# Zehong-Ma/MagCache

Measured on AMD Instinct MI355X. Metric: denoising steps/sec (MagCache on), Wan2.1-T2V-1.3B 480p 81f, higher is better.
Workload: dtype bf16

## Files before the change

include/magcache_hip.h:

```cpp
#ifndef MAGCACHE_HIP_H
#define MAGCACHE_HIP_H

#include <stddef.h>
#include <stdint.h>

#ifdef __cplusplus
extern "C" {
#endif

typedef struct mc_engine mc_engine;
typedef void* mc_stream;

typedef enum {
  MC_OK = 0,
  MC_EINVAL = 1,
  MC_ENOMEM = 2,
  MC_EHIP = 3,
  MC_ESTATE = 4
} mc_status;

typedef enum { MC_F32 = 0, MC_BF16 = 1 } mc_dtype;

typedef enum {
  MC_MODE_FULL = 0,
  MC_MODE_SKIP = 1,
  MC_MODE_CALIB = 2
} mc_mode;

typedef struct {
  int dim, ffn_dim, num_heads, num_layers;
  int in_dim, out_dim, freq_dim, text_dim, text_len;
  int latent_f, latent_h, latent_w;
  float eps;
  int sp_rank, sp_size;
  int n_branches;
  int calibration;
  int clip_dim;
  int vace_layers;
  int vace_stride;
  int vace_in_dim;
  int fp8_linear;
  int no_context_cache;
  int no_token_timesteps;
  int sp_phases;
} mc_config;

const char* mc_last_error(void);
const char* mc_version(void);
mc_status mc_set_option(const char* key, int value);

mc_status mc_create(const mc_config* cfg, mc_engine** out);
mc_status mc_create_sized(const mc_config* cfg, size_t cfg_bytes, mc_engine** out);
void mc_destroy(mc_engine* e);
size_t mc_workspace_bytes(const mc_engine* e);
mc_status mc_set_workspace(mc_engine* e, void* ws_dev, size_t bytes);
mc_status mc_buffer_info(const mc_engine* e, const char* name, size_t* offset, size_t* bytes);

mc_status mc_set_weight(mc_engine* e, const char* name, const void* src_dev, mc_dtype dtype, const int64_t* shape,
                        int ndim, mc_stream stream);
int mc_weights_missing(const mc_engine* e, char* buf, size_t buflen);

mc_status mc_forward(mc_engine* e, const float* latent_dev, const float* t_dev, double t_host,
                     const void* context_dev, mc_dtype ctx_dtype, int ctx_len, int branch, mc_mode mode,
                     float* out_dev, mc_stream stream);

mc_status mc_set_context(mc_engine* e, int slot, const void* context_dev, mc_dtype ctx_dtype, int ctx_len,
                         mc_stream stream);
mc_status mc_use_context(mc_engine* e, int slot);

mc_status mc_set_clip_fea(mc_engine* e, const void* clip_dev, mc_dtype dtype, int n_tokens, mc_stream stream);

mc_status mc_set_vace_context(mc_engine* e, const float* vace_dev, float context_scale, mc_stream stream);

mc_status mc_set_token_timesteps(mc_engine* e, const float* t_tokens_dev, mc_stream stream);

typedef enum {
  MC_PROF_ATTN_SELF = 0,
  MC_PROF_ATTN_CROSS = 1,
  MC_PROF_GEMM_QKV = 2,
  MC_PROF_GEMM_O = 3,
  MC_PROF_GEMM_CROSS_Q = 4,
  MC_PROF_GEMM_CROSS_O = 5,
  MC_PROF_GEMM_FFN1 = 6,
  MC_PROF_GEMM_FFN2 = 7,
  MC_PROF_LN_MODULATE = 8,
  MC_PROF_RMSNORM_ROPE = 9,
  MC_PROF_EMBED = 10,
  MC_PROF_HEAD = 11,
  MC_PROF_OTHER = 12,
  MC_PROF_SP_WAIT = 13,
  MC_PROF_NCLASS = 14
} mc_prof_class;
mc_status mc_profile_enable(mc_engine* e, int level);
mc_status mc_profile_read(mc_engine* e, double* attn_ms_total, int* attn_launches);
mc_status mc_profile_read_classes(mc_engine* e, double ms_total[MC_PROF_NCLASS], int launches[MC_PROF_NCLASS]);

mc_status mc_embed(mc_engine* e, const float* latent_dev, const float* t_dev, double t_host,
                   const void* context_dev, mc_dtype ctx_dtype, int ctx_len, mc_stream stream);
mc_status mc_block_pre_attn(mc_engine* e, int layer, mc_stream stream);
mc_status mc_block_pre_kv(mc_engine* e, int layer, mc_stream stream);
mc_status mc_block_pre_q(mc_engine* e, int layer, mc_stream stream);
mc_status mc_sp_set_chunks(mc_engine* e, int chunks);
mc_status mc_sp_round_info(const mc_engine* e, int round, int* n_rounds, int* chunk_rows, int* valid);
mc_status mc_block_attn_local(mc_engine* e, int layer, mc_stream stream);
mc_status mc_block_attn_round(mc_engine* e, int layer, int round, mc_stream stream);
mc_status mc_block_post_attn(mc_engine* e, int layer, int branch, mc_mode mode, mc_stream stream);
typedef int (*mc_sp_gather_fn)(void* user, int layer, int phase, mc_stream stream);
mc_status mc_blocks_sp(mc_engine* e, int layer_begin, int layer_end, int branch, mc_mode mode, int overlap,
                       mc_sp_gather_fn gather, void* user, mc_stream stream);
mc_status mc_sp_geometry(const mc_engine* e, int* num_layers, int* seq_len, int* rows_per_rank, int* head_stride, int* dim,
                         int* sp_size);
void* mc_workspace_base(const mc_engine* e);

#define MC_SP_ID_BYTES 128
typedef struct mc_sp_comm mc_sp_comm;
int mc_sp_rccl_available(void);
mc_status mc_sp_comm_id(void* id_out);
mc_status mc_sp_comm_create(const void* id, int nranks, int rank, mc_sp_comm** out);
void mc_sp_comm_destroy(mc_sp_comm* c);
const char* mc_sp_comm_info(const mc_sp_comm* c);
mc_status mc_blocks_sp_rccl(mc_engine* e, mc_sp_comm* c, int layer_begin, int layer_end, int branch, mc_mode mode,
                            int overlap, mc_stream stream);
mc_status mc_forward_sp_rccl(mc_engine* e, mc_sp_comm* c, const float* latent_dev, const float* t_dev, double t_host,
                             const void* context_dev, mc_dtype ctx_dtype, int ctx_len, int branch, mc_mode mode,
                             int overlap, float* tokens_full_dev, float* out_dev, mc_stream stream);
mc_status mc_vace_block_pre(mc_engine* e, int i, mc_stream stream);
mc_status mc_vace_block_post(mc_engine* e, int i, int branch, mc_mode mode, mc_stream stream);
mc_status mc_head(mc_engine* e, int branch, mc_mode mode, mc_stream stream);
mc_status mc_unpatchify(mc_engine* e, const float* tokens_dev, int tok0, int n_tok, float* out_dev,
                        mc_stream stream);

mc_status mc_calib_ready(const mc_engine* e, int branch, int* has_stats);
mc_status mc_calib_finalize(mc_engine* e, int branch, mc_stream stream);
mc_status mc_state_reset(mc_engine* e);
mc_status mc_import_residual(mc_engine* e, int branch, const float* src_dev, mc_stream stream);

typedef struct mc_rule mc_rule;
enum {
  MC_RULE_WAN21 = 0,
  MC_RULE_HUNYUAN = 1,
  MC_RULE_FLUX = 2,
  MC_RULE_WAN22_T2V = 3,
  MC_RULE_WAN22_I2V = 4,
  MC_RULE_WAN22_TI2V = 5,
  MC_RULE_FRAMEPACK = 6,
  MC_RULE_OMNIGEN2 = 7,
  MC_RULE_QWEN = 8,
  MC_RULE_EVAL_WAN = 9,
  MC_RULE_EVAL_OPENSORA = 10
};
mc_rule* mc_rule_create(int variant, int num_steps, double thresh, int K, double retention_ratio,
                        const double* mag_ratios, int n_ratios, int split_step);
void mc_rule_destroy(mc_rule* r);
int mc_rule_step(mc_rule* r, int* branch);
int mc_rule_cnt(const mc_rule* r);
void mc_rule_state(const mc_rule* r, double acc_err[2], int acc_steps[2], double acc_ratio[2]);
void mc_nearest_interp(const double* src, int src_len, double* dst, int target_length);

mc_status mc_op_gemm_bf16(const void* A_dev, long lda, const void* W_dev, long ldw, const float* bias_dev, int M,
                          int N, int K, int epi, void* Cb_dev, long ldc, float* X_dev, long ldx,
                          const float* gate_dev, const void* X0_dev, long ldx0, float* R_dev, long ldr,
                          void* X0out_dev, long ldx0out, int m_valid, mc_stream stream);
mc_status mc_op_gemm_bf16_resid_sel(const void* A_dev, long lda, const void* W_dev, long ldw, const float* bias_dev, int M,
                                    int N, int K, int capture, float* X_dev, long ldx, const float* gate_dev,
                                    const float* gate2_dev, const unsigned char* gate_sel_dev, const void* X0_dev, long ldx0,
                                    float* R_dev, long ldr, mc_stream stream);
mc_status mc_op_gemm_bf16_rowsplit(const void* A_dev, long lda, const void* W_dev, const void* W_b_dev, long ldw,
                                   const float* bias_dev, const float* bias_b_dev, int M, int N, int K, int m_split, int epi,
                                   void* Cb_dev, long ldc, float* X_dev, long ldx, const float* gate_dev, const float* gate_b_dev,
                                   mc_stream stream);
mc_status mc_op_gemm_bf16_gelu_split(const void* A_dev, long lda, const void* W_dev, long ldw, const float* bias_dev, int M,
                                     int N, int K, int n_split, void* Cb_dev, long ldc, void* Cb2_dev, long ldc2,
                                     mc_stream stream);
int mc_op_gemm_bf16_kernel(int M, int N, int K, int epi);
mc_status mc_op_set_splitk_workspace(void* ws_dev, size_t bytes);
int mc_op_gemm_bf16_splitk(int M, int N, int K, int epi);
size_t mc_op_gemm_splitk_need(int M, int N, int K, int epi);
mc_status mc_op_quantize_rows_fp8(const void* x_dev, mc_dtype dtype, long ldx, int M, int K, void* q_dev, long ldq,
                                  float* scale_dev, mc_stream stream);
mc_status mc_op_gemm_fp8(const void* A_q_dev, long lda, const float* a_scale_dev, const void* W_q_dev, long ldw,
                         const float* w_scale_dev, const float* bias_dev, int M, int N, int K, int epi, void* Cb_dev,
                         long ldc, float* X_dev, long ldx, const float* gate_dev, mc_stream stream);
mc_status mc_op_quantize_rows_mx(const void* x_dev, mc_dtype dtype, long ldx, int M, int K, void* q_dev, long ldq,
                                 void* scales_dev, long rows_pad, mc_stream stream);
mc_status mc_op_gemm_mxfp8(const void* A_q_dev, long lda, const void* a_scales_dev, long rows_pad_a, const void* W_q_dev,
                           long ldw, const void* w_scales_dev, long rows_pad_w, const float* bias_dev, int M, int N, int K,
                           int epi, void* Cb_dev, long ldc, float* X_dev, long ldx, const float* gate_dev,
                           mc_stream stream);
mc_status mc_op_attention(const void* Q_dev, long ldq, const void* K_dev, long ldk, long k_shard_stride,
                          const void* V_dev, long ldv, long v_shard_stride, void* O_dev, long ldo, int Lq_pad,
                          int n_heads, int shard_rows, int shard_valid, int n_shards, float scale,
                          mc_stream stream);
mc_status mc_op_attention_partial(const void* Q_dev, long ldq, const void* K_dev, long ldk, long k_shard_stride,
                                  const void* V_dev, long ldv, long v_shard_stride, void* O_dev, long ldo,
                                  int Lq_pad, int n_heads, int shard_rows, int shard_valid, int n_shards,
                                  float scale, int skip_shard, float* lse_out_dev, const float* lse_in_dev,
                                  mc_stream stream);
mc_status mc_op_attn_merge(const void* const* o_parts, const float* const* lse_parts, int n, void* out_bf16_dev, long ldo,
                           int rows, int rows_pad, int d, mc_stream stream);
mc_status mc_op_ln_modulate(const float* x_dev, long ldx, const void* x0_dev, long ldx0, const float* sc_dev,
                            const float* sh_dev, int mode, float eps, void* out_bf16_dev, long ldo,
                            float* out_f32_dev, long ldof, int M, int D, mc_stream stream);
mc_status mc_op_rmsnorm_rope(void* x_bf16_dev, long ldx, const float* w_dev, float eps, const float* cs_dev,
                             int cs_row0, int M, int D, mc_stream stream);
mc_status mc_op_skip_add(const void* x0_bf16_dev, long ldx0, const float* r_dev, long ldr, float* out_dev, long ldo,
                         int M, int D, mc_stream stream);
mc_status mc_op_residual_sub(const float* x_dev, long ldx, const void* x0_bf16_dev, long ldx0, float* r_dev,
                             long ldr, int M, int D, mc_stream stream);
mc_status mc_op_add_rows(float* x_dev, long ldx, const void* s_dev, mc_dtype s_dtype, float* r_dev, long ldr,
                         const void* x0_bf16_dev, long ldx0, int rows, int D, mc_stream stream);
mc_status mc_op_calib_stats(const float* r_dev, long ldr, const float* rp_dev, long ldrp, int M, int D,
                            double* partial_dev, int n_blocks, double* sums_dev, float* stats_dev,
                            mc_stream stream);
mc_status mc_op_cfg_euler(const float* cond_dev, const float* uncond_dev, float guide, float dt, float* x_dev,
                          float* eps_out_dev, size_t n, mc_stream stream);
mc_status mc_op_cfg_norm_euler(const float* cond_dev, const float* uncond_dev, long ld_pred, float guide, float dt,
                               float* x_dev, long ldx, int n_rows, int C, mc_stream stream);
mc_status mc_op_rmsnorm_rows_bf16(const float* x_dev, long ldx, const float* w_dev, float eps, void* out_bf16_dev, long ldo,
                                  int rows_valid, int rows, int D, mc_stream stream);
mc_status mc_op_lincomb(const float* const* xs_dev, const float* coef, int k, float* out_dev, size_t n,
                        mc_stream stream);
mc_status mc_op_cast_bf16(const float* src_dev, void* dst_bf16_dev, size_t n, mc_stream stream);
mc_status mc_op_rope_table(int F, int Hp, int Wp, int tok0, int n_tok, float* cs_host);

#ifdef __cplusplus
}
#endif
#endif
```

magcache_amd/_lib.py:

```python
import ctypes as C
import os

_HERE = os.path.dirname(os.path.abspath(__file__))
LIB_PATH = os.path.join(_HERE, "libmagcache_hip.so")
LIB_PATH = os.environ.get("MAGCACHE_HIP_LIB", LIB_PATH)

MC_OK, MC_EINVAL, MC_ENOMEM, MC_EHIP, MC_ESTATE = 0, 1, 2, 3, 4
MC_F32, MC_BF16 = 0, 1
MC_MODE_FULL, MC_MODE_SKIP, MC_MODE_CALIB = 0, 1, 2
PROF_CLASSES = ("attn_self", "attn_cross", "gemm_qkv", "gemm_o", "gemm_cross_q", "gemm_cross_o", "gemm_ffn1", "gemm_ffn2",
                "ln_modulate", "rmsnorm_rope", "embed", "head", "other", "sp_wait")
RULE_VARIANTS = {"wan21": 0, "hunyuan": 1, "flux": 2, "wan22_t2v": 3, "wan22_i2v": 4, "wan22_ti2v": 5, "framepack": 6,
                 "omnigen2": 7, "qwen": 8, "eval_wan": 9, "eval_opensora": 10}


class McConfig(C.Structure):
    _fields_ = [(n, C.c_int) for n in ("dim", "ffn_dim", "num_heads", "num_layers", "in_dim", "out_dim", "freq_dim",
                                       "text_dim", "text_len", "latent_f", "latent_h", "latent_w")] + \
               [("eps", C.c_float)] + \
               [(n, C.c_int) for n in ("sp_rank", "sp_size", "n_branches", "calibration", "clip_dim", "vace_layers",
                                         "vace_stride", "vace_in_dim", "fp8_linear", "no_context_cache",
                                         "no_token_timesteps", "sp_phases")]


class MagCacheHipError(RuntimeError):
    def __init__(self, status, msg):
        super().__init__(f"magcache_hip status {status}: {msg}")
        self.status = status


_vp, _i, _l, _f, _d, _sz = C.c_void_p, C.c_int, C.c_long, C.c_float, C.c_double, C.c_size_t
SP_GATHER_FN = C.CFUNCTYPE(C.c_int, C.c_void_p, C.c_int, C.c_int, C.c_void_p)

SIGNATURES = {
    "mc_last_error": (C.c_char_p, []),
    "mc_version": (C.c_char_p, []),
    "mc_set_option": (_i, [C.c_char_p, _i]),
    "mc_create": (_i, [C.POINTER(McConfig), C.POINTER(_vp)]),
    "mc_create_sized": (_i, [C.POINTER(McConfig), _sz, C.POINTER(_vp)]),
    "mc_destroy": (None, [_vp]),
    "mc_workspace_bytes": (_sz, [_vp]),
    "mc_set_workspace": (_i, [_vp, _vp, _sz]),
    "mc_buffer_info": (_i, [_vp, C.c_char_p, C.POINTER(_sz), C.POINTER(_sz)]),
    "mc_set_weight": (_i, [_vp, C.c_char_p, _vp, _i, C.POINTER(C.c_int64), _i, _vp]),
    "mc_weights_missing": (_i, [_vp, C.c_char_p, _sz]),
    "mc_forward": (_i, [_vp, _vp, _vp, _d, _vp, _i, _i, _i, _i, _vp, _vp]),
    "mc_set_clip_fea": (_i, [_vp, _vp, _i, _i, _vp]),
    "mc_set_vace_context": (_i, [_vp, _vp, _f, _vp]),
    "mc_set_token_timesteps": (_i, [_vp, _vp, _vp]),
    "mc_set_context": (_i, [_vp, _i, _vp, _i, _i, _vp]),
    "mc_use_context": (_i, [_vp, _i]),
    "mc_profile_enable": (_i, [_vp, _i]),
    "mc_profile_read": (_i, [_vp, C.POINTER(_d), C.POINTER(_i)]),
    "mc_profile_read_classes": (_i, [_vp, C.POINTER(_d), C.POINTER(_i)]),
    "mc_embed": (_i, [_vp, _vp, _vp, _d, _vp, _i, _i, _vp]),
    "mc_block_pre_attn": (_i, [_vp, _i, _vp]),
    "mc_block_pre_kv": (_i, [_vp, _i, _vp]),
    "mc_block_pre_q": (_i, [_vp, _i, _vp]),
    "mc_sp_set_chunks": (_i, [_vp, _i]),
    "mc_sp_round_info": (_i, [_vp, _i, C.POINTER(_i), C.POINTER(_i), C.POINTER(_i)]),
    "mc_sp_geometry": (_i, [_vp] + [C.POINTER(_i)] * 6),
    "mc_workspace_base": (_vp, [_vp]),
    "mc_block_attn_local": (_i, [_vp, _i, _vp]),
    "mc_block_attn_round": (_i, [_vp, _i, _i, _vp]),
    "mc_sp_rccl_available": (_i, []),
    "mc_sp_comm_id": (_i, [_vp]),
    "mc_sp_comm_create": (_i, [_vp, _i, _i, C.POINTER(_vp)]),
    "mc_sp_comm_destroy": (None, [_vp]),
    "mc_sp_comm_info": (C.c_char_p, [_vp]),
    "mc_blocks_sp_rccl": (_i, [_vp, _vp, _i, _i, _i, _i, _i, _vp]),
    "mc_forward_sp_rccl": (_i, [_vp, _vp, _vp, _vp, _d, _vp, _i, _i, _i, _i, _i, _vp, _vp, _vp]),
    "mc_block_post_attn": (_i, [_vp, _i, _i, _i, _vp]),
    "mc_blocks_sp": (_i, [_vp, _i, _i, _i, _i, _i, _vp, _vp, _vp]),
    "mc_vace_block_pre": (_i, [_vp, _i, _vp]),
    "mc_vace_block_post": (_i, [_vp, _i, _i, _i, _vp]),
    "mc_head": (_i, [_vp, _i, _i, _vp]),
    "mc_unpatchify": (_i, [_vp, _vp, _i, _i, _vp, _vp]),
    "mc_calib_ready": (_i, [_vp, _i, C.POINTER(_i)]),
    "mc_calib_finalize": (_i, [_vp, _i, _vp]),
    "mc_state_reset": (_i, [_vp]),
    "mc_import_residual": (_i, [_vp, _i, _vp, _vp]),
    "mc_rule_create": (_vp, [_i, _i, _d, _i, _d, C.POINTER(_d), _i, _i]),
    "mc_rule_destroy": (None, [_vp]),
    "mc_rule_step": (_i, [_vp, C.POINTER(_i)]),
    "mc_rule_cnt": (_i, [_vp]),
    "mc_rule_state": (None, [_vp, C.POINTER(_d), C.POINTER(_i), C.POINTER(_d)]),
    "mc_nearest_interp": (None, [C.POINTER(_d), _i, C.POINTER(_d), _i]),
    "mc_op_gemm_bf16": (_i, [_vp, _l, _vp, _l, _vp, _i, _i, _i, _i, _vp, _l, _vp, _l, _vp, _vp, _l, _vp, _l, _vp, _l,
                             _i, _vp]),
    "mc_op_gemm_bf16_resid_sel": (_i, [_vp, _l, _vp, _l, _vp, _i, _i, _i, _i, _vp, _l, _vp, _vp, _vp, _vp, _l, _vp, _l, _vp]),
    "mc_op_gemm_bf16_rowsplit": (_i, [_vp, _l, _vp, _vp, _l, _vp, _vp, _i, _i, _i, _i, _i, _vp, _l, _vp, _l, _vp, _vp, _vp]),
    "mc_op_gemm_bf16_gelu_split": (_i, [_vp, _l, _vp, _l, _vp, _i, _i, _i, _i, _vp, _l, _vp, _l, _vp]),
    "mc_op_gemm_bf16_kernel": (_i, [_i, _i, _i, _i]),
    "mc_op_gemm_bf16_splitk": (_i, [_i, _i, _i, _i]),
    "mc_op_gemm_splitk_need": (_sz, [_i, _i, _i, _i]),
    "mc_op_set_splitk_workspace": (_i, [_vp, _sz]),
    "mc_op_attention": (_i, [_vp, _l, _vp, _l, _l, _vp, _l, _l, _vp, _l, _i, _i, _i, _i, _i, _f, _vp]),
    "mc_op_quantize_rows_fp8": (_i, [_vp, _i, _l, _i, _i, _vp, _l, _vp, _vp]),
    "mc_op_gemm_fp8": (_i, [_vp, _l, _vp, _vp, _l, _vp, _vp, _i, _i, _i, _i, _vp, _l, _vp, _l, _vp, _vp]),
    "mc_op_quantize_rows_mx": (_i, [_vp, _i, _l, _i, _i, _vp, _l, _vp, _l, _vp]),
    "mc_op_gemm_mxfp8": (_i, [_vp, _l, _vp, _l, _vp, _l, _vp, _l, _vp, _i, _i, _i, _i, _vp, _l, _vp, _l, _vp, _vp]),
    "mc_op_attention_partial": (_i, [_vp, _l, _vp, _l, _l, _vp, _l, _l, _vp, _l, _i, _i, _i, _i, _i, _f, _i, _vp, _vp, _vp]),
    "mc_op_attn_merge": (_i, [_vp, _vp, _i, _vp, _l, _i, _i, _i, _vp]),
    "mc_op_ln_modulate": (_i, [_vp, _l, _vp, _l, _vp, _vp, _i, _f, _vp, _l, _vp, _l, _i, _i, _vp]),
    "mc_op_rmsnorm_rope": (_i, [_vp, _l, _vp, _f, _vp, _i, _i, _i, _vp]),
    "mc_op_skip_add": (_i, [_vp, _l, _vp, _l, _vp, _l, _i, _i, _vp]),
    "mc_op_residual_sub": (_i, [_vp, _l, _vp, _l, _vp, _l, _i, _i, _vp]),
    "mc_op_calib_stats": (_i, [_vp, _l, _vp, _l, _i, _i, _vp, _i, _vp, _vp, _vp]),
    "mc_op_cfg_euler": (_i, [_vp, _vp, _f, _f, _vp, _vp, _sz, _vp]),
    "mc_op_cast_bf16": (_i, [_vp, _vp, _sz, _vp]),
    "mc_op_cfg_norm_euler": (_i, [_vp, _vp, _l, _f, _f, _vp, _l, _i, _i, _vp]),
    "mc_op_rmsnorm_rows_bf16": (_i, [_vp, _l, _vp, _f, _vp, _l, _i, _i, _i, _vp]),
    "mc_op_lincomb": (_i, [_vp, _vp, _i, _vp, _sz, _vp]),
    "mc_op_add_rows": (_i, [_vp, _l, _vp, _i, _vp, _l, _vp, _l, _i, _i, _vp]),
    "mc_op_rope_table": (_i, [_i, _i, _i, _i, _i, _vp]),
    "mc_mmdit_create": (_i, [_vp, C.POINTER(_vp)]),
    "mc_mmdit_destroy": (None, [_vp]),
    "mc_mmdit_workspace_bytes": (_sz, [_vp]),
    "mc_mmdit_set_workspace": (_i, [_vp, _vp, _sz]),
    "mc_mmdit_buffer_info": (_i, [_vp, C.c_char_p, C.POINTER(_sz), C.POINTER(_sz)]),
    "mc_mmdit_geometry_bytes": (_i, [_vp, _i, _i, _i, _i, _i, C.POINTER(_sz)]),
    "mc_mmdit_set_geometry": (_i, [_vp, _i, _i, _i, _i, _i]),
    "mc_mmdit_set_weight": (_i, [_vp, C.c_char_p, _vp, _i, C.POINTER(C.c_int64), _i, _vp]),
    "mc_mmdit_weights_missing": (_i, [_vp, C.c_char_p, _sz]),
    "mc_mmdit_set_rope": (_i, [_vp, _vp, _vp, _i, _vp]),
    "mc_mmdit_set_controlnet": (_i, [_vp, _vp, _i, _vp, _i, _i, _i]),
    "mc_mmdit_controlnet_index": (_i, [_i, _i, _i, _i]),
    "mc_mmdit_forward": (_i, [_vp, _vp, _d, _d, _vp, _i, _vp, _i, _vp, _vp]),
    "mc_mmdit_forward2": (_i, [_vp, _vp, _d, _d, _vp, _i, _vp, _i, _i, _vp, _vp]),
    "mc_mmdit_begin": (_i, [_vp, _vp, _d, _d, _vp, _i, _vp, _i, _vp]),
    "mc_mmdit_block_pre": (_i, [_vp, _i, _vp]),
    "mc_mmdit_block_attn_local": (_i, [_vp, _i, _vp]),
    "mc_mmdit_block_post": (_i, [_vp, _i, _vp]),
    "mc_mmdit_end": (_i, [_vp, _vp, _vp]),
    "mc_mmdit_unpatchify": (_i, [_vp, _vp, _vp, _vp]),
    "mc_mmdit_calib_stats": (_i, [_vp, C.POINTER(C.c_float), _vp]),
    "mc_mmdit_state_reset": (_i, [_vp]),
}


class McMmditConfig(C.Structure):
    _fields_ = [(n, C.c_int) for n in ("family", "dim", "num_heads", "n_double", "n_single", "in_channels", "out_channels",
                                       "txt_dim", "txt_len", "vec_dim", "img_tokens", "latent_f", "latent_h", "latent_w",
                                       "refiner_depth", "calibration", "sp_rank", "sp_size")]


MC_FAMILY_FLUX, MC_FAMILY_HUNYUAN, MC_FAMILY_QWEN = 0, 1, 2

_lib = None


def load():
    global _lib
    if _lib is not None:
        return _lib
    if not os.path.exists(LIB_PATH):
        raise ImportError(f"{LIB_PATH} not found: the HIP engine is not built (python -m magcache_amd.build). "
                          "magcache_amd has no CPU fallback by design.")
    import torch
    lib = C.CDLL(LIB_PATH)
    for name, (res, args) in SIGNATURES.items():
        fn = getattr(lib, name)
        fn.restype = res
        fn.argtypes = args
    _lib = lib
    for kv in filter(None, os.environ.get("MAGCACHE_HIP_OPTIONS", "").split(",")):
        key, _, val = kv.partition("=")
        check(lib.mc_set_option(key.strip().encode(), int(val)))
    return lib


def check(status):
    if status != MC_OK:
        raise MagCacheHipError(status, load().mc_last_error().decode())
```

magcache_amd/csrc/engine.cpp:

```cpp
#include <cmath>
#include <cstddef>
#include <memory>

#include "host.h"

using mc::align_up;
using mc::bf16_t;
using mc::fail;
using mc::gp;
using mc::Linear;
using mc::RowRange;
using mc::whole;

namespace {

struct Layer {
  Linear qkv, o, cq, ckv, co, ffn1, ffn2;
  float *nq, *nk, *cnq, *cnk, *n3w, *n3b, *mod;
  Linear ckv_img;
  float* cnk_img = nullptr;
};

}

constexpr int kSpMaxParts = 9;

struct mc_engine {
  mc_config cfg;
  int d, ffn, H, NL, L, Lr, Lp, P, rank, tok0, Kp;
  int ctx_rows;
  std::vector<Layer> layers;
  bf16_t *w_patch, *w_text0, *w_text1;
  float *b_patch, *b_text0, *b_text1;
  float *w_time0, *b_time0, *w_time1, *b_time1, *w_tproj, *b_tproj;
  float *w_head, *b_head, *head_mod;
  bf16_t *w_img1 = nullptr, *w_img3 = nullptr;
  float *ln_img0_w = nullptr, *ln_img0_b = nullptr, *b_img1 = nullptr, *b_img3 = nullptr, *ln_img4_w = nullptr,
        *ln_img4_b = nullptr;
  int img_rows = 0;
  bool have_clip = false;
  bool sp = false;
  int sp_chunks = 1;
  int attn_layer = -2;
  int attn_launches = 0;
  bool attn_local_done = false;
  int attn_rounds_done = 0;
  hipStream_t side = nullptr;
  hipEvent_t ev_fork = nullptr, ev_join = nullptr;
  size_t splitk_bytes = 0;
  bool ctx_valid[2] = {false, false};
  int ctx_active = -1;
  const float* tok_t = nullptr;
  int HT = 64;
  int profile = 0;
  std::vector<hipEvent_t> prof_ev;
  std::vector<uint8_t> prof_cls;
  size_t prof_n = 0;
  std::vector<Layer> vlayers;
  std::vector<bf16_t*> w_after;
  std::vector<float*> b_after;
  bf16_t *w_vpatch = nullptr, *w_before = nullptr;
  float *b_vpatch = nullptr, *b_before = nullptr, *vscale = nullptr;
  int NV = 0, Kvp = 0;
  bool have_vace = false;
  float* cs_table = nullptr;
  mc::WeightStore weights;
  mc::Workspace work;
  int res_slot[2] = {0, 1};
  int res_scratch = 2;
  bool have_res[2] = {false, false};
  bool have_stats[2] = {false, false};
  bool embedded = false;

  template <class T>
  T* buf(const char* name) const { return work.get<T>(name); }
  float* residual(int idx) const {
    static const char* names[3] = {"residual0", "residual1", "residual2"};
    return buf<float>(names[idx]);
  }
};

namespace {

struct Prof {
  mc_engine* e;
  hipStream_t s;
  size_t idx = 0;
  bool on = false;
  Prof(mc_engine* e_, int cls, hipStream_t s_) : e(e_), s(s_) {
    if (!e->profile || (e->profile < 2 && cls != MC_PROF_ATTN_SELF) || e->prof_n + 2 > e->prof_ev.size()) return;
    idx = e->prof_n;
    if (hipEventRecord(e->prof_ev[idx], s) != hipSuccess) return;
    e->prof_cls[idx / 2] = (uint8_t)cls;
    e->prof_n += 2;
    on = true;
  }
  ~Prof() {
    if (on && hipEventRecord(e->prof_ev[idx + 1], s) != hipSuccess) e->prof_cls[idx / 2] = 0xff;
  }
  Prof(const Prof&) = delete;
  Prof& operator=(const Prof&) = delete;
};

void rope_table_host(int F, int Hp, int Wp, int tok0, int n_tok, float* cs) {
  const int d = 128, c = d / 2;
  const int n_hw = c / 3, n_t = c - 2 * n_hw;
  const double dim_t = (double)(d - 4 * (d / 6)), dim_hw = (double)(2 * (d / 6));
  for (int r = 0; r < n_tok; ++r) {
    const int tok = tok0 + r;
    float* row = cs + (size_t)r * 2 * c;
    if (tok >= F * Hp * Wp) {
      for (int i = 0; i < c; ++i) { row[2 * i] = 1.f; row[2 * i + 1] = 0.f; }
      continue;
    }
    const int f = tok / (Hp * Wp), rem = tok % (Hp * Wp), h = rem / Wp, w = rem % Wp;
    for (int i = 0; i < c; ++i) {
      double pos, fr;
      if (i < n_t) { pos = f; fr = 1.0 / std::pow(10000.0, (2.0 * i) / dim_t); }
      else if (i < n_t + n_hw) { pos = h; fr = 1.0 / std::pow(10000.0, (2.0 * (i - n_t)) / dim_hw); }
      else { pos = w; fr = 1.0 / std::pow(10000.0, (2.0 * (i - n_t - n_hw)) / dim_hw); }
      const double a = pos * fr;
      row[2 * i] = (float)std::cos(a);
      row[2 * i + 1] = (float)std::sin(a);
    }
  }
}

mc_status check_ready(const mc_engine* e) {
  if (!e) return fail(MC_EINVAL, "null engine");
  return mc::check_ready(e->work, e->weights, "mc_set_workspace");
}

}

namespace mc {
int g_fp8_fused_quant = 1;
int g_sp_attn_partials = 1;
}
static int g_n_cu = 0;

extern "C" {

mc_status mc_create_sized(const mc_config* cfg, size_t cfg_bytes, mc_engine** out) {
  if (!cfg || !out) return fail(MC_EINVAL, "null argument");
  if (cfg_bytes < offsetof(mc_config, fp8_linear) || cfg_bytes > sizeof(mc_config) || (cfg_bytes % sizeof(int)) != 0)
    return fail(MC_EINVAL, "mc_config of %zu bytes: this library knows %zu (0.1 layout) .. %zu", cfg_bytes,
                offsetof(mc_config, fp8_linear), sizeof(mc_config));
  mc_config full;
  memset(&full, 0, sizeof(full));
  memcpy(&full, cfg, cfg_bytes);
  return mc_create(&full, out);
}

mc_status mc_create(const mc_config* cfg, mc_engine** out) {
  if (!cfg || !out) return fail(MC_EINVAL, "null argument");
  const mc_config& c = *cfg;
  if (c.dim <= 0 || c.num_heads <= 0 || c.dim != c.num_heads * 128)
    return fail(MC_EINVAL, "dim (%d) must be num_heads (%d) * 128", c.dim, c.num_heads);
  if ((c.dim % 256) || (c.ffn_dim % 64) || (c.text_dim % 64) || (c.freq_dim % 4) || c.num_layers <= 0)
    return fail(MC_EINVAL, "unsupported geometry dim=%d ffn=%d text_dim=%d", c.dim, c.ffn_dim, c.text_dim);
  if ((c.latent_h & 1) || (c.latent_w & 1) || c.latent_f <= 0)
    return fail(MC_EINVAL, "latent grid %dx%dx%d not divisible by patch (1,2,2)", c.latent_f, c.latent_h, c.latent_w);
  if (c.sp_size < 1 || c.sp_rank < 0 || c.sp_rank >= c.sp_size) return fail(MC_EINVAL, "bad sp rank/size");
  if (c.n_branches != 1 && c.n_branches != 2) return fail(MC_EINVAL, "n_branches must be 1 or 2");
  if (c.out_dim * 4 > 256) return fail(MC_EINVAL, "out_dim*4 > 256 unsupported by the head kernel");
  if (c.clip_dim < 0 || (c.clip_dim % 256) != 0) return fail(MC_EINVAL, "clip_dim %d must be 0 or a multiple of 256", c.clip_dim);
  if (c.vace_layers < 0 || (c.vace_layers > 0 && (c.vace_stride <= 0 || c.vace_in_dim <= 0 ||
                                                   (c.vace_layers - 1) * c.vace_stride >= c.num_layers)))
    return fail(MC_EINVAL, "bad VACE geometry: %d blocks, stride %d, in_dim %d", c.vace_layers, c.vace_stride, c.vace_in_dim);
  if ((c.no_context_cache | c.no_token_timesteps) & ~1) return fail(MC_EINVAL, "no_context_cache / no_token_timesteps must be 0 or 1");
  if (c.fp8_linear < 0 || c.fp8_linear > 3)
    return fail(MC_EINVAL, "fp8_linear must be 0, 1 (per-row scales), 2 (MX block scales: QKV, FFN-1, FFN-2) or 3 (MX, the d x d Linears too)");
  if (c.fp8_linear && ((c.dim % 256) || (c.ffn_dim % 256) || c.dim < 512 || c.ffn_dim < 512))
    return fail(MC_EINVAL, "fp8_linear needs dim and ffn_dim to be multiples of 256 and >= 512");
  if (c.vace_layers > 0 && c.sp_size > 1 && (c.vace_layers - 1) * c.vace_stride == c.num_layers - 1)
    return fail(MC_EINVAL, "VACE with a hint on the last layer is single-GPU in this engine");

  std::unique_ptr<mc_engine, void (*)(mc_engine*)> own(new mc_engine(), mc_destroy);
  mc_engine* e = own.get();
  e->cfg = c;
  e->d = c.dim; e->ffn = c.ffn_dim; e->H = c.num_heads; e->NL = c.num_layers;
  e->L = c.latent_f * (c.latent_h / 2) * (c.latent_w / 2);
  e->P = c.sp_size; e->rank = c.sp_rank;
  e->sp = c.sp_size > 1 || c.sp_phases != 0;
  if (e->L % e->P) return fail(MC_EINVAL, "seq_len %d not divisible by sp_size %d", e->L, c.sp_size);
  e->Lr = e->L / e->P;
  e->Lp = (int)align_up(e->Lr, 256);
  e->tok0 = e->rank * e->Lr;
  e->Kp = (int)align_up((size_t)c.in_dim * 4, 64);
  e->HT = (int)align_up((size_t)c.out_dim * 4, 64);
  e->ctx_rows = (int)align_up(c.text_len, 64);
  const size_t d = e->d, ffn = e->ffn;
  mc::WeightStore& W = e->weights;

#define ALLOC(ptr, n) MC_TRY(W.alloc(&(ptr), (n)))
  const mc::Quant q_big = c.fp8_linear >= 2 ? mc::QUANT_MX : c.fp8_linear == 1 ? mc::QUANT_ROW : mc::QUANT_NONE;
  const mc::Quant q_dd = c.fp8_linear == 3 ? mc::QUANT_MX : mc::QUANT_NONE;
  e->layers.resize(e->NL);
  e->NV = c.vace_layers;
  e->vlayers.resize(e->NV);
  for (int i = 0; i < e->NL + e->NV; ++i) {
    const bool is_vace = i >= e->NL;
    Layer& l = is_vace ? e->vlayers[i - e->NL] : e->layers[i];
    const std::string p = (is_vace ? "vace_blocks." + std::to_string(i - e->NL) : "blocks." + std::to_string(i)) + ".";
    MC_TRY(W.add_linear(l.qkv, p + "self_attn.", {{"q", d}, {"k", d}, {"v", d}}, d, q_big));
    MC_TRY(W.add_linear(l.o, p + "self_attn.", {{"o", d}}, d, q_dd));
    MC_TRY(W.add_linear(l.cq, p + "cross_attn.", {{"q", d}}, d, q_dd));
    MC_TRY(W.add_linear(l.ckv, p + "cross_attn.", {{"k", d}, {"v", d}}, d));
    MC_TRY(W.add_linear(l.co, p + "cross_attn.", {{"o", d}}, d, q_dd));
    MC_TRY(W.add_linear(l.ffn1, p + "ffn.", {{"0", ffn}}, d, q_big));
    MC_TRY(W.add_linear(l.ffn2, p + "ffn.", {{"2", d}}, ffn, q_big));
    ALLOC(l.nq, d); ALLOC(l.nk, d); ALLOC(l.n3w, d); ALLOC(l.n3b, d); ALLOC(l.cnq, d); ALLOC(l.cnk, d); ALLOC(l.mod, 6 * d);
    W.add(p + "self_attn.norm_q.weight", l.nq, MC_F32, d);
    W.add(p + "self_attn.norm_k.weight", l.nk, MC_F32, d);
    W.add(p + "norm3.weight", l.n3w, MC_F32, d);
    W.add(p + "norm3.bias", l.n3b, MC_F32, d);
    W.add(p + "cross_attn.norm_q.weight", l.cnq, MC_F32, d);
    W.add(p + "cross_attn.norm_k.weight", l.cnk, MC_F32, d);
    W.add(p + "modulation", l.mod, MC_F32, 6 * d);
    if (c.clip_dim > 0) {
      MC_TRY(W.add_linear(l.ckv_img, p + "cross_attn.", {{"k_img", d}, {"v_img", d}}, d));
      ALLOC(l.cnk_img, d);
      W.add(p + "cross_attn.norm_k_img.weight", l.cnk_img, MC_F32, d);
    }
  }
  if (e->NV > 0) {
    e->Kvp = (int)align_up((size_t)c.vace_in_dim * 4, 64);
    const size_t kv = (size_t)c.vace_in_dim * 4;
    if (kv != (size_t)e->Kvp) { return fail(MC_EINVAL, "vace_in_dim*4 must be a multiple of 64"); }
    ALLOC(e->w_vpatch, d * kv); ALLOC(e->b_vpatch, d); ALLOC(e->w_before, d * d); ALLOC(e->b_before, d);
    ALLOC(e->vscale, d);
    W.add("vace_patch_embedding.weight", e->w_vpatch, MC_BF16, d * kv);
    W.add("vace_patch_embedding.bias", e->b_vpatch, MC_F32, d);
    W.add("vace_blocks.0.before_proj.weight", e->w_before, MC_BF16, d * d);
    W.add("vace_blocks.0.before_proj.bias", e->b_before, MC_F32, d);
    e->w_after.resize(e->NV); e->b_after.resize(e->NV);
    for (int i = 0; i < e->NV; ++i) {
      ALLOC(e->w_after[i], d * d); ALLOC(e->b_after[i], d);
      const std::string p = "vace_blocks." + std::to_string(i) + ".after_proj.";
      W.add(p + "weight", e->w_after[i], MC_BF16, d * d);
      W.add(p + "bias", e->b_after[i], MC_F32, d);
    }
  }
  if (c.clip_dim > 0) {
    const size_t cd = c.clip_dim;
    e->img_rows = (int)align_up(257, 64);
    ALLOC(e->ln_img0_w, cd); ALLOC(e->ln_img0_b, cd); ALLOC(e->w_img1, cd * cd); ALLOC(e->b_img1, cd);
    ALLOC(e->w_img3, d * cd); ALLOC(e->b_img3, d); ALLOC(e->ln_img4_w, d); ALLOC(e->ln_img4_b, d);
    W.add("img_emb.proj.0.weight", e->ln_img0_w, MC_F32, cd);
    W.add("img_emb.proj.0.bias", e->ln_img0_b, MC_F32, cd);
    W.add("img_emb.proj.1.weight", e->w_img1, MC_BF16, cd * cd);
    W.add("img_emb.proj.1.bias", e->b_img1, MC_F32, cd);
    W.add("img_emb.proj.3.weight", e->w_img3, MC_BF16, d * cd);
    W.add("img_emb.proj.3.bias", e->b_img3, MC_F32, d);
    W.add("img_emb.proj.4.weight", e->ln_img4_w, MC_F32, d);
    W.add("img_emb.proj.4.bias", e->ln_img4_b, MC_F32, d);
  }
  const size_t kin = (size_t)c.in_dim * 4;
  ALLOC(e->w_patch, d * e->Kp); ALLOC(e->b_patch, d);
  HIP_TRY(hipMemset(e->w_patch, 0, d * e->Kp * sizeof(bf16_t)));
  ALLOC(e->w_text0, d * c.text_dim); ALLOC(e->b_text0, d); ALLOC(e->w_text1, d * d); ALLOC(e->b_text1, d);
  ALLOC(e->w_time0, d * c.freq_dim); ALLOC(e->b_time0, d); ALLOC(e->w_time1, d * d); ALLOC(e->b_time1, d);
  ALLOC(e->w_tproj, 6 * d * d); ALLOC(e->b_tproj, 6 * d);
  ALLOC(e->w_head, (size_t)c.out_dim * 4 * d); ALLOC(e->b_head, (size_t)c.out_dim * 4); ALLOC(e->head_mod, 2 * d);
  mc::Slot& patch = W.add("patch_embedding.weight", e->w_patch, MC_BF16, d * kin);
  if (kin != (size_t)e->Kp) patch.pad = {d, kin, (size_t)e->Kp};
  W.add("patch_embedding.bias", e->b_patch, MC_F32, d);
  W.add("text_embedding.0.weight", e->w_text0, MC_BF16, d * c.text_dim);
  W.add("text_embedding.0.bias", e->b_text0, MC_F32, d);
  W.add("text_embedding.2.weight", e->w_text1, MC_BF16, d * d);
  W.add("text_embedding.2.bias", e->b_text1, MC_F32, d);
  W.add("time_embedding.0.weight", e->w_time0, MC_F32, d * c.freq_dim);
  W.add("time_embedding.0.bias", e->b_time0, MC_F32, d);
  W.add("time_embedding.2.weight", e->w_time1, MC_F32, d * d);
  W.add("time_embedding.2.bias", e->b_time1, MC_F32, d);
  W.add("time_projection.1.weight", e->w_tproj, MC_F32, 6 * d * d);
  W.add("time_projection.1.bias", e->b_tproj, MC_F32, 6 * d);
  W.add("head.head.weight", e->w_head, MC_F32, (size_t)c.out_dim * 4 * d);
  W.add("head.head.bias", e->b_head, MC_F32, (size_t)c.out_dim * 4);
  W.add("head.modulation", e->head_mod, MC_F32, 2 * d);

  ALLOC(e->cs_table, (size_t)e->Lp * 128);
  {
    std::vector<float> cs((size_t)e->Lp * 128);
    rope_table_host(c.latent_f, c.latent_h / 2, c.latent_w / 2, e->tok0, e->Lr, cs.data());
    for (size_t r = e->Lr; r < (size_t)e->Lp; ++r)
      for (int i = 0; i < 64; ++i) { cs[r * 128 + 2 * i] = 1.f; cs[r * 128 + 2 * i + 1] = 0.f; }
    HIP_TRY(hipMemcpy(e->cs_table, cs.data(), cs.size() * sizeof(float), hipMemcpyHostToDevice));
  }
#undef ALLOC

  mc::Workspace& ws = e->work;
  const size_t Lp = e->Lp;
  ws.add("x", Lp * d * 4);
  ws.add("x0", Lp * d * 2);
  ws.add("xn", Lp * d * 2);
  ws.add("qkv", Lp * 3 * d * 2);
  ws.add("ao", Lp * d * 2);
  ws.add("h", std::max(Lp * ffn * 2, Lp * d * 4));
  ws.add("tokens", Lp * e->Kp * 2);
  ws.add("ctx_in", (size_t)e->ctx_rows * c.text_dim * 2);
  ws.add("ctx_h", (size_t)e->ctx_rows * d * 2);
  ws.add("ctx", (size_t)e->ctx_rows * d * 2);
  ws.add("ckv", (size_t)e->ctx_rows * 2 * d * 2);
  ws.add("ctx_cache", (size_t)2 * e->ctx_rows * d * 2);
  if (!c.no_context_cache)
    ws.add("ckv_cache", (size_t)2 * (e->NL + e->NV) * e->ctx_rows * 2 * d * 2);
  const size_t tsets = c.no_token_timesteps ? 1 : 2;
  ws.add("temb", tsets * (c.freq_dim + 2 * d + 6 * d) * 4);
  ws.add("emod", tsets * (e->NL + e->NV) * 6 * d * 4);
  ws.add("tok_sel", c.no_token_timesteps ? 256 : (size_t)Lp + 256);
  ws.add("tok_t2", 64);
  if (c.fp8_linear) {
    ws.add("aq", Lp * std::max(d, ffn));
    ws.add("a_scale", Lp * 4);
    if (c.fp8_linear >= 2) ws.add("a_mx", (std::max(d, ffn) / 32) * Lp);
  }
  if (e->NV > 0) {
    ws.add("xc", Lp * d * 4);
    ws.add("c0", Lp * d * 2);
    ws.add("vtokens", Lp * (size_t)e->Kvp * 2);
  }
  ws.add("ehead", 2 * 2 * d * 4);
  ws.add("head_tokens", (size_t)Lp * e->HT * 4);
  ws.add("kv_local", e->sp ? Lp * 2 * d * 2 : 256);
  ws.add("kv_gather", e->sp ? (size_t)e->P * Lp * 2 * d * 2 : 256);
  ws.add("residual0", Lp * d * 4);
  ws.add("residual1", c.n_branches > 1 ? Lp * d * 4 : 256);
  ws.add("residual2", c.calibration ? Lp * d * 4 : 256);
  if (c.clip_dim > 0) {
    const size_t ir = e->img_rows, cd = c.clip_dim;
    ws.add("clip_in", ir * cd * 4);
    ws.add("clip_n", ir * cd * 2);
    ws.add("clip_h", ir * cd * 2);
    ws.add("clip_o", ir * d * 4);
    ws.add("clip_h2", ir * d * 2);
    ws.add("ctx_img", ir * d * 2);
    ws.add("ckv_img", ir * 2 * d * 2);
    ws.add("ao2", Lp * d * 2);
  }
  if (e->sp) ws.add("attn_lse", (size_t)e->H * Lp * 4);
  e->splitk_bytes = e->sp ? mc::gemm_splitk_ws_need((int)Lp, (int)d, (int)ffn, mc::EPI_RESID_GATE) : 0;
  ws.add("splitk", e->splitk_bytes ? e->splitk_bytes : 256);
  ws.add("ao_part", e->P > 1 ? (size_t)kSpMaxParts * Lp * d * 2 : 256);
  ws.add("lse_part", e->P > 1 ? (size_t)kSpMaxParts * e->H * Lp * 4 : 256);
  ws.add("calib_partial", (2048 * 4 + 2) * 8);
  ws.add("calib_sums", 4 * 8);
  ws.add("calib_stats", 2 * 3 * 4);
  *out = own.release();
  return MC_OK;
}

void mc_destroy(mc_engine* e) {
  if (!e) return;
  e->weights.free_all();
  for (hipEvent_t ev : e->prof_ev) (void)hipEventDestroy(ev);
  if (e->ev_fork) (void)hipEventDestroy(e->ev_fork);
  if (e->ev_join) (void)hipEventDestroy(e->ev_join);
  if (e->side) (void)hipStreamDestroy(e->side);
  delete e;
}

size_t mc_workspace_bytes(const mc_engine* e) { return e ? e->work.need : 0; }

mc_status mc_set_workspace(mc_engine* e, void* ws_dev, size_t bytes) {
  if (!e) return fail(MC_EINVAL, "null argument");
  MC_TRY(e->work.bind(ws_dev, bytes));
  e->have_res[0] = e->have_res[1] = false;
  HIP_TRY(hipMemset(e->buf<double>("calib_partial") + 2048 * 4, 0, 16));
  return MC_OK;
}

mc_status mc_buffer_info(const mc_engine* e, const char* name, size_t* offset, size_t* bytes) {
  if (!e || !name) return fail(MC_EINVAL, "null argument");
  std::string n(name);
  if (n == "residual_branch0" || n == "residual_branch1") {
    static const char* names[3] = {"residual0", "residual1", "residual2"};
    n = names[e->res_slot[n.back() - '0']];
  }
  return e->work.info(n, offset, bytes);
}

mc_status mc_set_weight(mc_engine* e, const char* name, const void* src_dev, mc_dtype dtype, const int64_t* shape,
                        int ndim, mc_stream stream) {
  if (e) {
    e->ctx_valid[0] = e->ctx_valid[1] = false;
    e->ctx_active = -1;
  }
  if (!e || !name || !src_dev || !shape) return fail(MC_EINVAL, "null argument");
  return e->weights.set(name, src_dev, dtype, shape, ndim, (hipStream_t)stream);
}

int mc_weights_missing(const mc_engine* e, char* buf, size_t buflen) { return e ? e->weights.missing(buf, buflen) : -1; }

mc_status mc_set_clip_fea(mc_engine* e, const void* clip_dev, mc_dtype dtype, int n_tokens, mc_stream stream_) {
  hipStream_t s = (hipStream_t)stream_;
  mc_status st = check_ready(e);
  if (st != MC_OK) return st;
  const mc_config& c = e->cfg;
  if (c.clip_dim <= 0) return fail(MC_EINVAL, "engine was created without clip_dim (t2v model)");
  if (!clip_dev || n_tokens != 257) return fail(MC_EINVAL, "clip_fea must be [257, %d]", c.clip_dim);
  const int cd = c.clip_dim, ir = e->img_rows, d = e->d;
  float* in = e->buf<float>("clip_in");
  HIP_TRY(hipMemsetAsync(in, 0, (size_t)ir * cd * 4, s));
  if (dtype == MC_F32) {
    HIP_TRY(hipMemcpyAsync(in, clip_dev, (size_t)n_tokens * cd * 4, hipMemcpyDeviceToDevice, s));
  } else {
    return fail(MC_EINVAL, "clip_fea must be given as fp32");
  }
  bf16_t* n0 = e->buf<bf16_t>("clip_n");
  HIP_TRY(mc::launch_ln_modulate(in, cd, nullptr, 0, e->ln_img0_w, e->ln_img0_b, 1, 1e-5f, n0, cd, nullptr, 0, ir, cd, s));
  {
    mc::GemmParams p = gp(n0, cd, e->w_img1, cd, e->b_img1, ir, cd, cd);
    p.Cb = e->buf<bf16_t>("clip_h"); p.ldc = cd;
    HIP_TRY(mc::launch_gemm_bf16(p, mc::EPI_GELU_ERF_BF16, s));
    mc::GemmParams q = gp(e->buf<bf16_t>("clip_h"), cd, e->w_img3, cd, e->b_img3, ir, d, cd);
    q.Cb = e->buf<bf16_t>("clip_h2"); q.ldc = d;
    HIP_TRY(mc::launch_gemm_bf16(q, mc::EPI_BF16, s));
  }
  HIP_TRY(hipMemsetAsync(e->buf<float>("clip_o"), 0, (size_t)ir * d * 4, s));
  HIP_TRY(mc::launch_ln_modulate(e->buf<float>("clip_o"), d, e->buf<bf16_t>("clip_h2"), d, e->ln_img4_w,
                                 e->ln_img4_b, 1, 1e-5f, e->buf<bf16_t>("ctx_img"), d, nullptr, 0, ir, d, s));
  e->have_clip = true;
  return MC_OK;
}

mc_status mc_set_vace_context(mc_engine* e, const float* vace_dev, float context_scale, mc_stream stream_) {
  hipStream_t s = (hipStream_t)stream_;
  mc_status st = check_ready(e);
  if (st != MC_OK) return st;
  if (e->NV <= 0) return fail(MC_EINVAL, "engine was created without VACE blocks");
  const mc_config& c = e->cfg;
  const int d = e->d;
  if (vace_dev) {
    bf16_t* vt = e->buf<bf16_t>("vtokens");
    HIP_TRY(mc::launch_patchify(vace_dev, c.vace_in_dim, c.latent_f, c.latent_h, c.latent_w, e->tok0, e->Lr, e->Lp, vt,
                                e->Kvp, s));
    mc::GemmParams p = gp(vt, e->Kvp, e->w_vpatch, e->Kvp, e->b_vpatch, e->Lp, d, e->Kvp);
    p.X = e->buf<float>("xc"); p.ldx = d;
    p.X0out = e->buf<bf16_t>("c0"); p.ldx0out = d;
    p.m_valid = e->Lr;
    HIP_TRY(mc::launch_gemm_bf16(p, mc::EPI_EMBED, s));
    e->have_vace = true;
  } else if (!e->have_vace) {
    return fail(MC_EINVAL, "null vace_context and none set before");
  }
  std::vector<float> sc(d, context_scale);
  HIP_TRY(hipMemcpyAsync(e->vscale, sc.data(), (size_t)d * 4, hipMemcpyHostToDevice, s));
  HIP_TRY(hipStreamSynchronize(s));
  return MC_OK;
}

static mc_status embed_context(mc_engine* e, const void* context_dev, mc_dtype ctx_dtype, int ctx_len, bf16_t* dst,
                               hipStream_t s) {
  const mc_config& c = e->cfg;
  const int d = e->d;
  if (ctx_len <= 0 || ctx_len > c.text_len)
    return fail(MC_EINVAL, "context length %d exceeds text_len %d", ctx_len, c.text_len);
  bf16_t* ctx_in = e->buf<bf16_t>("ctx_in");
  if (ctx_dtype == MC_F32) {
    HIP_TRY(mc::launch_cast_pad_bf16((const float*)context_dev, c.text_dim, ctx_len, e->ctx_rows, c.text_dim, ctx_in,
                                     c.text_dim, s));
  } else {
    HIP_TRY(hipMemsetAsync(ctx_in, 0, (size_t)e->ctx_rows * c.text_dim * 2, s));
    HIP_TRY(hipMemcpyAsync(ctx_in, context_dev, (size_t)ctx_len * c.text_dim * 2, hipMemcpyDeviceToDevice, s));
  }
  mc::GemmParams p = gp(ctx_in, c.text_dim, e->w_text0, c.text_dim, e->b_text0, e->ctx_rows, d, c.text_dim);
  p.Cb = e->buf<bf16_t>("ctx_h"); p.ldc = d;
  HIP_TRY(mc::launch_gemm_bf16(p, mc::EPI_GELU_BF16, s));
  mc::GemmParams q = gp(e->buf<bf16_t>("ctx_h"), d, e->w_text1, d, e->b_text1, e->ctx_rows, d, d);
  q.Cb = dst; q.ldc = d;
  HIP_TRY(mc::launch_gemm_bf16(q, mc::EPI_BF16, s));
  return MC_OK;
}

static mc_status context_kv(mc_engine* e, const Layer& l, const bf16_t* ctx, bf16_t* ckv, hipStream_t s) {
  const int d = e->d;
  mc::GemmParams q = gp(ctx, d, l.ckv.w, d, l.ckv.b, e->ctx_rows, 2 * d, d);
  q.Cb = ckv; q.ldc = 2 * d;
  HIP_TRY(mc::launch_gemm_bf16(q, mc::EPI_BF16, s));
  HIP_TRY(mc::launch_rmsnorm_rope(ckv, 2 * d, l.cnk, e->cfg.eps, nullptr, 0, e->ctx_rows, d, s));
  return MC_OK;
}

mc_status mc_embed(mc_engine* e, const float* latent_dev, const float* t_dev, double t_host,
                   const void* context_dev, mc_dtype ctx_dtype, int ctx_len, mc_stream stream_) {
  hipStream_t s = (hipStream_t)stream_;
  mc_status st = check_ready(e);
  if (st != MC_OK) return st;
  if (!latent_dev) return fail(MC_EINVAL, "null input");
  const mc_config& c = e->cfg;
  if (c.clip_dim > 0 && !e->have_clip)
    return fail(MC_ESTATE, "i2v model: mc_set_clip_fea must run before the forward (reference assert :226-227)");
  const int d = e->d;
  Prof pr(e, MC_PROF_EMBED, s);
  bf16_t* tokens = e->buf<bf16_t>("tokens");
  if (e->Kp != c.in_dim * 4) HIP_TRY(hipMemsetAsync(tokens, 0, (size_t)e->Lp * e->Kp * 2, s));
  HIP_TRY(mc::launch_patchify(latent_dev, c.in_dim, c.latent_f, c.latent_h, c.latent_w, e->tok0, e->Lr, e->Lp,
                              tokens, e->Kp, s));
  {
    mc::GemmParams p = gp(tokens, e->Kp, e->w_patch, e->Kp, e->b_patch, e->Lp, d, e->Kp);
    p.X = e->buf<float>("x"); p.ldx = d;
    p.X0out = e->buf<bf16_t>("x0"); p.ldx0out = d;
    p.m_valid = e->Lr;
    HIP_TRY(mc::launch_gemm_bf16(p, mc::EPI_EMBED, s));
  }
  const int n_sets = e->tok_t ? 2 : 1;
  float* t2 = e->buf<float>("tok_t2");
  if (e->tok_t)
    HIP_TRY(mc::launch_token_t_prepare(e->tok_t, e->L, e->tok0, e->Lr, e->Lp, t2, e->buf<uint8_t>("tok_sel"), s));
  const size_t temb_set = (size_t)c.freq_dim + 2 * d + 6 * d, emod_set = (size_t)(e->NL + e->NV) * 6 * d;
  for (int set = 0; set < n_sets; ++set) {
    float* temb = e->buf<float>("temb") + set * temb_set;
    float* sinus = temb;
    float* h1 = temb + c.freq_dim;
    float* ev = h1 + d;
    float* e0 = ev + d;
    HIP_TRY(mc::launch_sinusoid(e->tok_t ? t2 + set : t_dev, t_host, c.freq_dim, sinus, s));
    HIP_TRY(mc::launch_gemv_f32(e->w_time0, sinus, e->b_time0, h1, d, c.freq_dim, 0, 1, s));
    HIP_TRY(mc::launch_gemv_f32(e->w_time1, h1, e->b_time1, ev, d, d, 0, 0, s));
    HIP_TRY(mc::launch_gemv_f32(e->w_tproj, ev, e->b_tproj, e0, 6 * d, d, 1, 0, s));
    float* emod = e->buf<float>("emod") + set * emod_set;
    for (int l = 0; l < e->NL + e->NV; ++l)
      HIP_TRY(mc::launch_add_bcast(e0, 6 * d, (l < e->NL ? e->layers[l] : e->vlayers[l - e->NL]).mod,
                                   emod + (size_t)l * 6 * d, 6 * d, s));
    HIP_TRY(mc::launch_add_bcast(ev, d, e->head_mod, e->buf<float>("ehead") + set * 2 * d, 2 * d, s));
  }
  if (context_dev) {
    e->ctx_active = -1;
    mc_status cst = embed_context(e, context_dev, ctx_dtype, ctx_len, e->buf<bf16_t>("ctx"), s);
    if (cst != MC_OK) return cst;
  } else if (e->ctx_active < 0 || !e->ctx_valid[e->ctx_active]) {
    return fail(MC_ESTATE, "context_dev is NULL but no cached context is selected (mc_set_context)");
  }
  e->embedded = true;
  return MC_OK;
}

struct ActSrc {
  const bf16_t* rows = nullptr; long ld = 0;
  bool quantised = false;
  uint8_t *q = nullptr, *mx = nullptr;
};

static mc_status linear(mc_engine* e, const Linear& l, RowRange out, ActSrc a, mc::GemmParams p, int epi, hipStream_t s) {
  const int Lp = e->Lp, K = l.k_in;
  if (!l.q) {
    HIP_TRY(mc::launch_linear_bf16(l, out, a.rows, a.ld, Lp, p, epi, s));
    return MC_OK;
  }
  p.M = Lp; p.N = out.count; p.K = K; p.bias = l.b + out.first;
  uint8_t* aq = a.q ? a.q : e->buf<uint8_t>("aq");
  p.A = (const bf16_t*)aq; p.lda = K; p.W = (const bf16_t*)(l.q + (size_t)out.first * K); p.ldw = K;
  if (l.mx) {
    uint8_t* am = a.mx ? a.mx : e->buf<uint8_t>("a_mx");
    if (!a.quantised) HIP_TRY(mc::launch_quantize_rows_mx(a.rows, nullptr, a.ld, Lp, K, aq, K, am, (long)Lp, s));
    p.a_mx = am; p.mx_rows_a = (long)Lp; p.w_mx = l.mx + out.first; p.mx_rows_w = l.n_out;
    HIP_TRY(mc::launch_gemm_mxfp8(p, epi, s));
    return MC_OK;
  }
  float* as = e->buf<float>("a_scale");
  if (!a.quantised) HIP_TRY(mc::launch_quantize_rows_fp8(a.rows, nullptr, a.ld, Lp, K, aq, K, as, s));
  p.a_scale = as; p.w_scale = l.q_scale + out.first;
  HIP_TRY(mc::launch_gemm_fp8(p, epi, s));
  return MC_OK;
}

static mc_status ln_for_gemm(mc_engine* e, const Linear& l, const float* x, const float* sc, const float* sh, int mode,
                             const float* sc2, const float* sh2, const uint8_t* sel, hipStream_t s, ActSrc* a) {
  const int d = e->d, Lp = e->Lp;
  bf16_t* xn = e->buf<bf16_t>("xn");
  *a = ActSrc{xn, d, l.q && mc::g_fp8_fused_quant};
  if (a->quantised) {
    HIP_TRY(mc::launch_ln_modulate_fp8(x, d, sc, sh, mode, e->cfg.eps, e->buf<uint8_t>("aq"), d,
                                       l.mx ? nullptr : e->buf<float>("a_scale"), l.mx ? e->buf<uint8_t>("a_mx") : nullptr,
                                       (long)Lp, Lp, d, s, sc2, sh2, sel));
  } else {
    HIP_TRY(mc::launch_ln_modulate(x, d, nullptr, 0, sc, sh, mode, e->cfg.eps, xn, d, nullptr, 0, Lp, d, s, sc2, sh2, sel));
  }
  return MC_OK;
}

static const float* second_set(const mc_engine* e, const float* em) {
  return e->tok_t ? em + (size_t)(e->NL + e->NV) * 6 * e->d : nullptr;
}
static const uint8_t* tok_sel(const mc_engine* e) { return e->tok_t ? e->buf<uint8_t>("tok_sel") : nullptr; }

static int sp_chunk_rows(const mc_engine* e) { return e->Lp / e->sp_chunks; }
static int sp_round_valid(const mc_engine* e, int c) {
  const int lc = sp_chunk_rows(e);
  return std::max(0, std::min(lc, e->Lr - c * lc));
}
static int sp_rounds(const mc_engine* e) {
  const int lc = sp_chunk_rows(e);
  return (e->Lr + lc - 1) / lc;
}

static mc_status block_pre_kv(mc_engine* e, const Layer& l, const float* em, float* x, hipStream_t s) {
  const int d = e->d, Lp = e->Lp;
  const float* em2 = second_set(e, em);
  ActSrc a;
  {
    Prof pr(e, MC_PROF_LN_MODULATE, s);
    MC_TRY(ln_for_gemm(e, l.qkv, x, em + d, em, 0, em2 ? em2 + d : nullptr, em2, tok_sel(e), s, &a));
  }
  mc::GemmParams p = {};
  if (!e->sp) {
    bf16_t* qkv = e->buf<bf16_t>("qkv");
    p.Cb = qkv; p.ldc = 3 * d;
    {
      Prof pr(e, MC_PROF_GEMM_QKV, s);
      MC_TRY(linear(e, l.qkv, whole(l.qkv), a, p, mc::EPI_BF16, s));
    }
    Prof pr(e, MC_PROF_RMSNORM_ROPE, s);
    HIP_TRY(mc::launch_rmsnorm_rope(qkv, 3 * d, l.nq, e->cfg.eps, e->cs_table, 0, Lp, d, s));
    HIP_TRY(mc::launch_rmsnorm_rope(qkv + d, 3 * d, l.nk, e->cfg.eps, e->cs_table, 0, Lp, d, s));
  } else {
    bf16_t* kvl = e->buf<bf16_t>("kv_local");
    p.Cb = kvl; p.ldc = 2 * d;
    {
      Prof pr(e, MC_PROF_GEMM_QKV, s);
      MC_TRY(linear(e, l.qkv, RowRange{d, 2 * d}, a, p, mc::EPI_BF16, s));
    }
    Prof pr(e, MC_PROF_RMSNORM_ROPE, s);
    HIP_TRY(mc::launch_rmsnorm_rope(kvl, 2 * d, l.nk, e->cfg.eps, e->cs_table, 0, Lp, d, s));
  }
  e->attn_layer = -2;
  return MC_OK;
}

static mc_status block_pre_q(mc_engine* e, const Layer& l, hipStream_t s) {
  const int d = e->d, Lp = e->Lp;
  if (!e->sp) return MC_OK;
  bf16_t* qkv = e->buf<bf16_t>("qkv");
  {
    Prof pr(e, MC_PROF_GEMM_QKV, s);
    mc::GemmParams p = {};
    p.Cb = qkv; p.ldc = d;
    MC_TRY(linear(e, l.qkv, RowRange{0, d}, ActSrc{e->buf<bf16_t>("xn"), d, true}, p, mc::EPI_BF16, s));
  }
  Prof pr(e, MC_PROF_RMSNORM_ROPE, s);
  HIP_TRY(mc::launch_rmsnorm_rope(qkv, d, l.nq, e->cfg.eps, e->cs_table, 0, Lp, d, s));
  return MC_OK;
}

static mc_status block_pre(mc_engine* e, const Layer& l, const float* em, float* x, hipStream_t s) {
  mc_status st = block_pre_kv(e, l, em, x, s);
  return st != MC_OK ? st : block_pre_q(e, l, s);
}

static mc_status check_layer_call(mc_engine* e, int layer) {
  if (!e || !e->embedded) return fail(MC_ESTATE, "mc_embed must run first");
  if (layer < 0 || layer >= e->NL) return fail(MC_EINVAL, "layer %d out of range", layer);
  return MC_OK;
}

mc_status mc_block_pre_attn(mc_engine* e, int layer, mc_stream stream_) {
  if (mc_status st = check_layer_call(e, layer); st != MC_OK) return st;
  return block_pre(e, e->layers[layer], e->buf<float>("emod") + (size_t)layer * 6 * e->d, e->buf<float>("x"),
                   (hipStream_t)stream_);
}

mc_status mc_block_pre_kv(mc_engine* e, int layer, mc_stream stream_) {
  if (mc_status st = check_layer_call(e, layer); st != MC_OK) return st;
  if (!e->sp) return fail(MC_ESTATE, "mc_block_pre_kv needs a sequence-parallel engine (sp_size > 1 or sp_phases) (one GPU: mc_block_pre_attn / mc_forward)");
  return block_pre_kv(e, e->layers[layer], e->buf<float>("emod") + (size_t)layer * 6 * e->d, e->buf<float>("x"),
                      (hipStream_t)stream_);
}

mc_status mc_block_pre_q(mc_engine* e, int layer, mc_stream stream_) {
  if (mc_status st = check_layer_call(e, layer); st != MC_OK) return st;
  if (!e->sp) return fail(MC_ESTATE, "mc_block_pre_q needs a sequence-parallel engine (sp_size > 1 or sp_phases)");
  return block_pre_q(e, e->layers[layer], (hipStream_t)stream_);
}

static mc_status sp_attn_launch(mc_engine* e, int layer, int round, hipStream_t s) {
  const int d = e->d, Lp = e->Lp;
  if (e->attn_layer != layer) {
    e->attn_layer = layer; e->attn_launches = 0; e->attn_local_done = false; e->attn_rounds_done = 0;
  }
  const int n_rounds = sp_rounds(e);
  mc::AttnParams a;
  memset(&a, 0, sizeof(a));
  a.O = e->buf<bf16_t>("ao"); a.ldo = d; a.Lq_pad = Lp; a.n_heads = e->H; a.scale = 1.0f / std::sqrt(128.0f);
  a.Q = e->buf<bf16_t>("qkv"); a.ldq = d;
  bool more;
  if (round < 0) {
    if (e->attn_launches) return fail(MC_ESTATE, "the local-shard attention must be the first launch of a layer's chain");
    bf16_t* kvl = e->buf<bf16_t>("kv_local");
    a.K = kvl; a.ldk = 2 * d; a.V = kvl + d; a.ldv = 2 * d;
    a.shard_rows = Lp; a.shard_valid = e->Lr; a.n_shards = 1;
    more = true;
  } else {
    if (round != e->attn_rounds_done || round >= n_rounds)
      return fail(MC_ESTATE, "attention round %d out of order (rounds done %d of %d)", round, e->attn_rounds_done, n_rounds);
    const int lc = sp_chunk_rows(e);
    bf16_t* kvg = e->buf<bf16_t>("kv_gather") + (size_t)round * e->P * lc * 2 * d;
    a.K = kvg; a.ldk = 2 * d; a.k_shard_stride = (long)lc * 2 * d;
    a.V = kvg + d; a.ldv = 2 * d; a.v_shard_stride = (long)lc * 2 * d;
    a.shard_rows = lc; a.shard_valid = sp_round_valid(e, round); a.n_shards = e->P;
    if (e->attn_local_done) a.skip_shard_p1 = e->rank + 1;
    more = round + 1 < n_rounds;
    if (e->attn_local_done && e->P == 1) {
      e->attn_rounds_done++;
      return MC_OK;
    }
  }
  if (e->attn_launches) a.lse_in = e->buf<float>("attn_lse");
  if (more) a.lse_out = e->buf<float>("attn_lse");
  {
    Prof pr(e, MC_PROF_ATTN_SELF, s);
    HIP_TRY(mc::launch_attention(a, s));
  }
  e->attn_launches++;
  if (round < 0) e->attn_local_done = true; else e->attn_rounds_done++;
  return MC_OK;
}

static mc_status sp_attn_partial(mc_engine* e, int round, hipStream_t s) {
  const int d = e->d, Lp = e->Lp;
  const int slot = round < 0 ? 0 : 1 + round;
  mc::AttnParams a;
  memset(&a, 0, sizeof(a));
  a.O = e->buf<bf16_t>("ao_part") + (size_t)slot * Lp * d; a.ldo = d; a.Lq_pad = Lp; a.n_heads = e->H;
  a.scale = 1.0f / std::sqrt(128.0f);
  a.Q = e->buf<bf16_t>("qkv"); a.ldq = d;
  a.lse_out = e->buf<float>("lse_part") + (size_t)slot * e->H * Lp;
  if (round < 0) {
    bf16_t* kvl = e->buf<bf16_t>("kv_local");
    a.K = kvl; a.ldk = 2 * d; a.V = kvl + d; a.ldv = 2 * d;
    a.shard_rows = Lp; a.shard_valid = e->Lr; a.n_shards = 1;
  } else {
    const int lc = sp_chunk_rows(e);
    bf16_t* kvg = e->buf<bf16_t>("kv_gather") + (size_t)round * e->P * lc * 2 * d;
    a.K = kvg; a.ldk = 2 * d; a.k_shard_stride = (long)lc * 2 * d;
    a.V = kvg + d; a.ldv = 2 * d; a.v_shard_stride = (long)lc * 2 * d;
    a.shard_rows = lc; a.shard_valid = sp_round_valid(e, round); a.n_shards = e->P;
    a.skip_shard_p1 = e->rank + 1;
  }
  HIP_TRY(mc::launch_attention(a, s));
  return MC_OK;
}

static mc_status sp_side_stream(mc_engine* e) {
  if (e->side) return MC_OK;
  HIP_TRY(hipStreamCreateWithFlags(&e->side, hipStreamNonBlocking));
  HIP_TRY(hipEventCreateWithFlags(&e->ev_fork, hipEventDisableTiming));
  HIP_TRY(hipEventCreateWithFlags(&e->ev_join, hipEventDisableTiming));
  return MC_OK;
}

mc_status mc_block_attn_local(mc_engine* e, int layer, mc_stream stream_) {
  if (mc_status st = check_layer_call(e, layer); st != MC_OK) return st;
  if (!e->sp) return fail(MC_ESTATE, "mc_block_attn_local needs a sequence-parallel engine (sp_size > 1 or sp_phases)");
  return sp_attn_launch(e, layer, -1, (hipStream_t)stream_);
}

mc_status mc_block_attn_round(mc_engine* e, int layer, int round, mc_stream stream_) {
  if (mc_status st = check_layer_call(e, layer); st != MC_OK) return st;
  if (!e->sp) return fail(MC_ESTATE, "mc_block_attn_round needs a sequence-parallel engine (sp_size > 1 or sp_phases)");
  if (round < 0) return fail(MC_EINVAL, "round %d", round);
  return sp_attn_launch(e, layer, round, (hipStream_t)stream_);
}

mc_status mc_sp_set_chunks(mc_engine* e, int chunks) {
  if (!e) return fail(MC_EINVAL, "null engine");
  if (!e->sp) return fail(MC_ESTATE, "mc_sp_set_chunks needs a sequence-parallel engine (sp_size > 1 or sp_phases)");
  if (chunks < 1 || chunks > 64 || e->Lp % chunks || (e->Lp / chunks) % 64)
    return fail(MC_EINVAL, "sp chunks %d: rows per shard %d / chunks must be a multiple of 64", chunks, e->Lp);
  e->sp_chunks = chunks;
  e->attn_layer = -2;
  return MC_OK;
}

mc_status mc_sp_geometry(const mc_engine* e, int* num_layers, int* seq_len, int* rows_per_rank, int* head_stride, int* dim,
                         int* sp_size) {
  if (!e) return fail(MC_EINVAL, "null engine");
  if (num_layers) *num_layers = e->NL;
  if (seq_len) *seq_len = e->L;
  if (rows_per_rank) *rows_per_rank = e->Lr;
  if (head_stride) *head_stride = e->HT;
  if (dim) *dim = e->d;
  if (sp_size) *sp_size = e->P;
  return MC_OK;
}

void* mc_workspace_base(const mc_engine* e) { return e ? (void*)e->work.ws : nullptr; }

mc_status mc_sp_round_info(const mc_engine* e, int round, int* n_rounds, int* chunk_rows, int* valid) {
  if (!e) return fail(MC_EINVAL, "null engine");
  if (round < 0 || round >= e->sp_chunks) return fail(MC_EINVAL, "round %d of %d", round, e->sp_chunks);
  if (n_rounds) *n_rounds = e->sp ? sp_rounds(e) : 0;
  if (chunk_rows) *chunk_rows = sp_chunk_rows(e);
  if (valid) *valid = sp_round_valid(e, round);
  return MC_OK;
}

static mc_status block_post(mc_engine* e, const Layer& l, const float* em, float* x, int layer, bool capture, int branch,
                            mc_mode mode, hipStream_t s) {
  const int d = e->d, Lp = e->Lp, ffn = e->ffn;
  bf16_t* qkv = e->buf<bf16_t>("qkv");
  bf16_t* ao = e->buf<bf16_t>("ao");
  const float scale = 1.0f / std::sqrt(128.0f);
  const float* em2 = second_set(e, em);
  const uint8_t* sel = tok_sel(e);

  if (!e->sp) {
    mc::AttnParams a;
    memset(&a, 0, sizeof(a));
    a.O = ao; a.ldo = d; a.Lq_pad = Lp; a.n_heads = e->H; a.scale = scale;
    a.Q = qkv; a.ldq = 3 * d;
    a.K = qkv + d; a.ldk = 3 * d; a.k_shard_stride = 0;
    a.V = qkv + 2 * d; a.ldv = 3 * d; a.v_shard_stride = 0;
    a.shard_rows = Lp; a.shard_valid = e->Lr; a.n_shards = 1;
    Prof pr(e, MC_PROF_ATTN_SELF, s);
    HIP_TRY(mc::launch_attention(a, s));
  } else {
    if (e->attn_layer != layer) { e->attn_layer = layer; e->attn_launches = 0; e->attn_local_done = false; e->attn_rounds_done = 0; }
    while (e->attn_rounds_done < sp_rounds(e)) {
      mc_status st = sp_attn_launch(e, layer, e->attn_rounds_done, s);
      if (st != MC_OK) return st;
    }
    e->attn_layer = -2;
  }
  {
    Prof pr(e, MC_PROF_GEMM_O, s);
    mc::GemmParams p = {};
    p.X = x; p.ldx = d; p.gate = em + 2 * d;
    if (em2) { p.gate2 = em2 + 2 * d; p.gate_sel = sel; }
    MC_TRY(linear(e, l.o, whole(l.o), ActSrc{ao, d}, p, mc::EPI_RESID_GATE, s));
  }
  ActSrc xn;
  {
    Prof pr(e, MC_PROF_LN_MODULATE, s);
    MC_TRY(ln_for_gemm(e, l.cq, x, l.n3w, l.n3b, 1, nullptr, nullptr, nullptr, s, &xn));
  }
  bf16_t* cq = qkv;
  bf16_t* ckv = e->buf<bf16_t>("ckv");
  {
    mc::GemmParams p = {};
    p.Cb = cq; p.ldc = d;
    {
      Prof pr(e, MC_PROF_GEMM_CROSS_Q, s);
      MC_TRY(linear(e, l.cq, whole(l.cq), xn, p, mc::EPI_BF16, s));
    }
    {
      Prof pr(e, MC_PROF_RMSNORM_ROPE, s);
      HIP_TRY(mc::launch_rmsnorm_rope(cq, d, l.cnq, e->cfg.eps, nullptr, 0, Lp, d, s));
    }
    if (e->ctx_active >= 0) {
      const size_t li = (size_t)(&l - (layer >= 0 ? e->layers.data() : e->vlayers.data())) + (layer >= 0 ? 0 : e->NL);
      ckv = e->buf<bf16_t>("ckv_cache") + ((size_t)e->ctx_active * (e->NL + e->NV) + li) * e->ctx_rows * 2 * d;
    } else {
      Prof pr(e, MC_PROF_OTHER, s);
      mc_status kst = context_kv(e, l, e->buf<bf16_t>("ctx"), ckv, s);
      if (kst != MC_OK) return kst;
    }
    mc::AttnParams a;
    memset(&a, 0, sizeof(a));
    a.Q = cq; a.ldq = d; a.K = ckv; a.ldk = 2 * d; a.V = ckv + d; a.ldv = 2 * d;
    a.O = ao; a.ldo = d; a.Lq_pad = Lp; a.n_heads = e->H; a.scale = scale;
    a.shard_rows = e->ctx_rows; a.shard_valid = e->cfg.text_len; a.n_shards = 1;
    {
      Prof pr(e, MC_PROF_ATTN_CROSS, s);
      HIP_TRY(mc::launch_attention(a, s));
    }
    if (e->cfg.clip_dim > 0) {
      Prof pr(e, MC_PROF_OTHER, s);
      bf16_t* ckvi = e->buf<bf16_t>("ckv_img");
      bf16_t* ao2 = e->buf<bf16_t>("ao2");
      mc::GemmParams qi = gp(e->buf<bf16_t>("ctx_img"), d, l.ckv_img.w, d, l.ckv_img.b, e->img_rows, 2 * d, d);
      qi.Cb = ckvi; qi.ldc = 2 * d;
      HIP_TRY(mc::launch_gemm_bf16(qi, mc::EPI_BF16, s));
      HIP_TRY(mc::launch_rmsnorm_rope(ckvi, 2 * d, l.cnk_img, e->cfg.eps, nullptr, 0, e->img_rows, d, s));
      mc::AttnParams ai = a;
      ai.K = ckvi; ai.V = ckvi + d; ai.O = ao2;
      ai.shard_rows = e->img_rows; ai.shard_valid = 257;
      HIP_TRY(mc::launch_attention(ai, s));
      HIP_TRY(mc::launch_add_bf16(ao, ao2, (size_t)Lp * d, s));
    }
    Prof pr(e, MC_PROF_GEMM_CROSS_O, s);
    mc::GemmParams o = {};
    o.X = x; o.ldx = d; o.gate = nullptr;
    MC_TRY(linear(e, l.co, whole(l.co), ActSrc{ao, d}, o, mc::EPI_RESID_GATE, s));
  }
  {
    Prof pr(e, MC_PROF_LN_MODULATE, s);
    MC_TRY(ln_for_gemm(e, l.ffn1, x, em + 4 * d, em + 3 * d, 0, em2 ? em2 + 4 * d : nullptr, em2 ? em2 + 3 * d : nullptr, sel,
                       s, &xn));
  }
  bf16_t* h = e->buf<bf16_t>("h");
  {
    mc::GemmParams p = {};
    p.Cb = h; p.ldc = ffn;
    const bool h_fp8 = l.ffn1.mx && l.ffn2.mx && mc::g_fp8_fused_quant;
    ActSrc hidden{h, ffn};
    if (h_fp8) {
      hidden.quantised = true; hidden.q = (uint8_t*)h; hidden.mx = hidden.q + (size_t)Lp * ffn;
      p.Cq = hidden.q; p.ldcq = ffn; p.c_mx = hidden.mx; p.mx_rows_c = Lp;
    }
    {
      Prof pr(e, MC_PROF_GEMM_FFN1, s);
      MC_TRY(linear(e, l.ffn1, whole(l.ffn1), xn, p, h_fp8 ? mc::EPI_GELU_MXFP8 : mc::EPI_GELU_BF16, s));
    }
    mc::GemmParams q = {};
    q.X = x; q.ldx = d; q.gate = em + 5 * d;
    if (e->splitk_bytes) { q.splitk_ws = e->buf<float>("splitk"); q.splitk_ws_bytes = e->splitk_bytes; }
    if (em2) { q.gate2 = em2 + 5 * d; q.gate_sel = sel; }
    auto ffn2 = [&](int epi) -> mc_status {
      Prof pr(e, MC_PROF_GEMM_FFN2, s);
      return linear(e, l.ffn2, whole(l.ffn2), hidden, q, epi, s);
    };
    if (capture) {
      const int dst = (mode == MC_MODE_CALIB) ? e->res_scratch : e->res_slot[branch];
      q.X0 = e->buf<bf16_t>("x0"); q.ldx0 = d;
      q.R = e->residual(dst); q.ldr = d;
      {
        mc_status st = ffn2(mc::EPI_RESID_CAPTURE);
        if (st != MC_OK) return st;
      }
      if (mode == MC_MODE_CALIB) {
        if (!e->cfg.calibration) return fail(MC_ESTATE, "engine was created without calibration=1");
        if (e->have_res[branch]) {
          Prof pr(e, MC_PROF_OTHER, s);
          HIP_TRY(mc::launch_calib_stats(e->residual(dst), d, e->residual(e->res_slot[branch]), d, e->Lr, d,
                                         e->buf<double>("calib_partial"), 2048, e->buf<double>("calib_sums"),
                                         e->buf<float>("calib_stats") + 3 * branch, s));
          e->have_stats[branch] = true;
        } else {
          e->have_stats[branch] = false;
        }
        std::swap(e->res_slot[branch], e->res_scratch);
      }
      e->have_res[branch] = true;
    } else {
      mc_status st = ffn2(mc::EPI_RESID_GATE);
      if (st != MC_OK) return st;
    }
  }
  return MC_OK;
}

static bool hint_on_last_layer(const mc_engine* e) {
  return e->NV > 0 && (e->NV - 1) * e->cfg.vace_stride == e->NL - 1;
}

mc_status mc_block_post_attn(mc_engine* e, int layer, int branch, mc_mode mode, mc_stream stream_) {
  if (!e || !e->embedded) return fail(MC_ESTATE, "mc_embed must run first");
  if (layer < 0 || layer >= e->NL) return fail(MC_EINVAL, "layer %d out of range", layer);
  if (branch < 0 || branch >= e->cfg.n_branches) return fail(MC_EINVAL, "branch %d out of range", branch);
  return block_post(e, e->layers[layer], e->buf<float>("emod") + (size_t)layer * 6 * e->d, e->buf<float>("x"), layer,
                    layer == e->NL - 1 && !hint_on_last_layer(e), branch, mode, (hipStream_t)stream_);
}

static mc_status vace_pre_kv(mc_engine* e, int i, hipStream_t s) {
  const int d = e->d, Lp = e->Lp;
  float* xc = e->buf<float>("xc");
  if (i == 0) {
    HIP_TRY(hipMemsetAsync(xc, 0, (size_t)Lp * d * 4, s));
    HIP_TRY(mc::launch_skip_add(e->buf<bf16_t>("x0"), d, xc, d, xc, d, Lp, d, s));
    mc::GemmParams p = gp(e->buf<bf16_t>("c0"), d, e->w_before, d, e->b_before, Lp, d, d);
    p.X = xc; p.ldx = d; p.gate = nullptr;
    HIP_TRY(mc::launch_gemm_bf16(p, mc::EPI_RESID_GATE, s));
  }
  return block_pre_kv(e, e->vlayers[i], e->buf<float>("emod") + (size_t)(e->NL + i) * 6 * d, xc, s);
}

static mc_status vace_pre(mc_engine* e, int i, hipStream_t s) {
  mc_status st = vace_pre_kv(e, i, s);
  return st != MC_OK ? st : block_pre_q(e, e->vlayers[i], s);
}

static mc_status vace_post(mc_engine* e, int i, int branch, mc_mode mode, hipStream_t s) {
  const int d = e->d, Lp = e->Lp;
  float* xc = e->buf<float>("xc");
  mc_status st = block_post(e, e->vlayers[i], e->buf<float>("emod") + (size_t)(e->NL + i) * 6 * d, xc, -1, false, branch,
                            mode, s);
  if (st != MC_OK) return st;
  bf16_t* xn = e->buf<bf16_t>("xn");
  HIP_TRY(mc::launch_cast_bf16(xc, xn, (size_t)Lp * d, s));
  mc::GemmParams h = gp(xn, d, e->w_after[i], d, e->b_after[i], Lp, d, d);
  h.X = e->buf<float>("x"); h.ldx = d; h.gate = e->vscale;
  HIP_TRY(mc::launch_gemm_bf16(h, mc::EPI_RESID_GATE, s));
  return MC_OK;
}

static mc_status vace_block(mc_engine* e, int i, int branch, mc_mode mode, hipStream_t s) {
  mc_status st = vace_pre(e, i, s);
  return st != MC_OK ? st : vace_post(e, i, branch, mode, s);
}

mc_status mc_vace_block_pre(mc_engine* e, int i, mc_stream stream) {
  if (!e || !e->embedded) return fail(MC_ESTATE, "mc_embed must run first");
  if (i < 0 || i >= e->NV) return fail(MC_EINVAL, "VACE block %d out of range", i);
  if (!e->have_vace) return fail(MC_ESTATE, "mc_set_vace_context must run first");
  return vace_pre(e, i, (hipStream_t)stream);
}

mc_status mc_vace_block_post(mc_engine* e, int i, int branch, mc_mode mode, mc_stream stream) {
  if (!e || !e->embedded) return fail(MC_ESTATE, "mc_embed must run first");
  if (i < 0 || i >= e->NV) return fail(MC_EINVAL, "VACE block %d out of range", i);
  if (branch < 0 || branch >= e->cfg.n_branches) return fail(MC_EINVAL, "branch %d out of range", branch);
  return vace_post(e, i, branch, mode, (hipStream_t)stream);
}

mc_status mc_blocks_sp(mc_engine* e, int layer_begin, int layer_end, int branch, mc_mode mode, int overlap,
                       mc_sp_gather_fn gather, void* user, mc_stream stream) {
  if (!e || !e->embedded) return fail(MC_ESTATE, "mc_embed must run first");
  if (!gather) return fail(MC_EINVAL, "null gather callback");
  if (!e->sp) return fail(MC_ESTATE, "mc_blocks_sp needs a sequence-parallel engine (sp_size > 1 or sp_phases) (one GPU: mc_forward)");
  if (layer_begin < 0 || layer_end > e->NL || layer_begin > layer_end)
    return fail(MC_EINVAL, "layers [%d, %d) out of range (num_layers %d)", layer_begin, layer_end, e->NL);
  if (mode == MC_MODE_SKIP) return fail(MC_EINVAL, "a skipped forward runs no blocks (mc_embed -> mc_head)");
  hipStream_t s = (hipStream_t)stream;
  const int R = sp_rounds(e);
  auto coll = [&](int layer, int phase) -> mc_status {
    const int rc = gather(user, layer, phase, stream);
    return rc == 0 ? MC_OK : fail(MC_ESTATE, "gather callback failed (layer %d, phase %d, code %d)", layer, phase, rc);
  };
  auto wait_round = [&](int layer, int c, hipStream_t on) -> mc_status {
    Prof pr(e, MC_PROF_SP_WAIT, on);
    const int rc = gather(user, layer, 2 * c + 1, (mc_stream)on);
    return rc == 0 ? MC_OK : fail(MC_ESTATE, "gather callback failed (layer %d, phase %d, code %d)", layer, 2 * c + 1, rc);
  };
  if (!g_n_cu) {
    int dev = 0, n = 0;
    if (hipGetDevice(&dev) == hipSuccess && hipDeviceGetAttribute(&n, hipDeviceAttributeMultiprocessorCount, dev) == hipSuccess && n > 0)
      g_n_cu = n;
    else
      g_n_cu = 256;
  }
  const long wg = (long)(e->Lp / 256) * e->H, waves = (wg + g_n_cu - 1) / g_n_cu;
  const bool underfilled = wg * 10 < waves * g_n_cu * 9;
  const bool partials = (mc::g_sp_attn_partials == 2 || (mc::g_sp_attn_partials == 1 && underfilled)) && e->P > 1 && 1 + R <= kSpMaxParts;
  if (partials)
    if (mc_status st = sp_side_stream(e); st != MC_OK) return st;
  auto attend = [&](int l, const Layer& ly, int chain) -> mc_status {
    mc_status st;
    for (int c = 0; c < R; ++c)
      if ((st = coll(l, 2 * c)) != MC_OK) return st;
    if (!overlap)
      for (int c = 0; c < R; ++c)
        if ((st = wait_round(l, c, s)) != MC_OK) return st;
    if ((st = block_pre_q(e, ly, s)) != MC_OK) return st;
    if (!partials) {
      if ((st = sp_attn_launch(e, chain, -1, s)) != MC_OK) return st;
      for (int c = 0; c < R; ++c) {
        if (overlap && (st = wait_round(l, c, s)) != MC_OK) return st;
        if ((st = sp_attn_launch(e, chain, c, s)) != MC_OK) return st;
      }
      return MC_OK;
    }
    Prof chain_pr(e, MC_PROF_ATTN_SELF, s);
    HIP_TRY(hipEventRecord(e->ev_fork, s));
    HIP_TRY(hipStreamWaitEvent(e->side, e->ev_fork, 0));
    if ((st = sp_attn_partial(e, -1, s)) != MC_OK) return st;
    for (int c = 0; c < R; ++c) {
      hipStream_t on = (c & 1) ? s : e->side;
      if (overlap && (st = wait_round(l, c, on)) != MC_OK) return st;
      if ((st = sp_attn_partial(e, c, on)) != MC_OK) return st;
    }
    HIP_TRY(hipEventRecord(e->ev_join, e->side));
    HIP_TRY(hipStreamWaitEvent(s, e->ev_join, 0));
    const bf16_t* op[kSpMaxParts];
    const float* lp[kSpMaxParts];
    for (int i = 0; i <= R; ++i) {
      op[i] = e->buf<bf16_t>("ao_part") + (size_t)i * e->Lp * e->d;
      lp[i] = e->buf<float>("lse_part") + (size_t)i * e->H * e->Lp;
    }
    HIP_TRY(mc::launch_attn_merge(op, lp, 1 + R, e->buf<bf16_t>("ao"), e->d, e->Lp, e->Lp, e->d, s));
    e->attn_layer = chain; e->attn_launches = 1 + R; e->attn_local_done = true; e->attn_rounds_done = R;
    return MC_OK;
  };
  const int d = e->d;
  for (int l = layer_begin; l < layer_end; ++l) {
    mc_status st = block_pre_kv(e, e->layers[l], e->buf<float>("emod") + (size_t)l * 6 * d, e->buf<float>("x"), s);
    if (st != MC_OK) return st;
    if ((st = attend(l, e->layers[l], l)) != MC_OK) return st;
    if ((st = mc_block_post_attn(e, l, branch, mode, stream)) != MC_OK) return st;
    if (e->NV > 0 && l % e->cfg.vace_stride == 0 && l / e->cfg.vace_stride < e->NV) {
      const int i = l / e->cfg.vace_stride;
      if (!e->have_vace) return fail(MC_ESTATE, "mc_set_vace_context must run first");
      if ((st = vace_pre_kv(e, i, s)) != MC_OK) return st;
      if ((st = attend(l, e->vlayers[i], -1)) != MC_OK) return st;
      if ((st = mc_vace_block_post(e, i, branch, mode, stream)) != MC_OK) return st;
    }
  }
  return MC_OK;
}

static mc_status capture_unfused(mc_engine* e, int branch, mc_mode mode, hipStream_t s) {
  const int d = e->d;
  const int dst = (mode == MC_MODE_CALIB) ? e->res_scratch : e->res_slot[branch];
  HIP_TRY(mc::launch_residual_sub(e->buf<float>("x"), d, e->buf<bf16_t>("x0"), d, e->residual(dst), d, e->Lp, d, s));
  if (mode == MC_MODE_CALIB) {
    if (!e->cfg.calibration) return fail(MC_ESTATE, "engine was created without calibration=1");
    if (e->have_res[branch]) {
      HIP_TRY(mc::launch_calib_stats(e->residual(dst), d, e->residual(e->res_slot[branch]), d, e->Lr, d,
                                     e->buf<double>("calib_partial"), 2048, e->buf<double>("calib_sums"),
                                     e->buf<float>("calib_stats") + 3 * branch, s));
      e->have_stats[branch] = true;
    } else {
      e->have_stats[branch] = false;
    }
    std::swap(e->res_slot[branch], e->res_scratch);
  }
  e->have_res[branch] = true;
  return MC_OK;
}

mc_status mc_head(mc_engine* e, int branch, mc_mode mode, mc_stream stream_) {
  hipStream_t s = (hipStream_t)stream_;
  if (!e || !e->embedded) return fail(MC_ESTATE, "mc_embed must run first");
  if (branch < 0 || branch >= e->cfg.n_branches) return fail(MC_EINVAL, "branch %d out of range", branch);
  const int d = e->d;
  const float* eh = e->buf<float>("ehead");
  const float* eh2 = e->tok_t ? eh + 2 * d : nullptr;
  const uint8_t* sel = tok_sel(e);
  float* hn = e->buf<float>("h");
  Prof pr(e, MC_PROF_HEAD, s);
  if (mode == MC_MODE_SKIP) {
    if (!e->have_res[branch]) return fail(MC_ESTATE, "skip requested but residual_cache[%d] is empty", branch);
    HIP_TRY(mc::launch_ln_modulate(e->residual(e->res_slot[branch]), d, e->buf<bf16_t>("x0"), d, eh + d, eh, 0,
                                   e->cfg.eps, nullptr, 0, hn, d, e->Lr, d, s, eh2 ? eh2 + d : nullptr, eh2, sel));
  } else {
    HIP_TRY(mc::launch_ln_modulate(e->buf<float>("x"), d, nullptr, 0, eh + d, eh, 0, e->cfg.eps, nullptr, 0, hn, d,
                                   e->Lr, d, s, eh2 ? eh2 + d : nullptr, eh2, sel));
  }
  HIP_TRY(mc::launch_head_linear(hn, d, e->w_head, e->b_head, e->buf<float>("head_tokens"), e->HT, e->Lr,
                                 e->cfg.out_dim * 4, d, s));
  return MC_OK;
}

mc_status mc_unpatchify(mc_engine* e, const float* tokens_dev, int tok0, int n_tok, float* out_dev,
                        mc_stream stream_) {
  if (!e || !tokens_dev || !out_dev) return fail(MC_EINVAL, "null argument");
  if (tok0 < 0 || n_tok <= 0 || tok0 + n_tok > e->L) return fail(MC_EINVAL, "token range out of bounds");
  const mc_config& c = e->cfg;
  Prof pr(e, MC_PROF_HEAD, (hipStream_t)stream_);
  HIP_TRY(mc::launch_unpatchify(tokens_dev, e->HT, c.out_dim, c.latent_f, c.latent_h, c.latent_w, tok0, n_tok, out_dev,
                                (hipStream_t)stream_));
  return MC_OK;
}

mc_status mc_forward(mc_engine* e, const float* latent_dev, const float* t_dev, double t_host,
                     const void* context_dev, mc_dtype ctx_dtype, int ctx_len, int branch, mc_mode mode,
                     float* out_dev, mc_stream stream) {
  if (!e) return fail(MC_EINVAL, "null engine");
  if (e->sp) return fail(MC_ESTATE, "mc_forward is single-GPU; drive a sharded engine through the phase calls");
  if (!out_dev) return fail(MC_EINVAL, "null output");
  if (e->NV > 0 && mode != MC_MODE_SKIP && !e->have_vace)
    return fail(MC_ESTATE, "VACE model: mc_set_vace_context must run before a non-skipped forward");
  mc_status st = mc_embed(e, latent_dev, t_dev, t_host, context_dev, ctx_dtype, ctx_len, stream);
  if (st != MC_OK) return st;
  if (mode != MC_MODE_SKIP) {
    for (int l = 0; l < e->NL; ++l) {
      st = mc_block_pre_attn(e, l, stream);
      if (st != MC_OK) return st;
      st = mc_block_post_attn(e, l, branch, mode, stream);
      if (st != MC_OK) return st;
      if (e->NV > 0 && l % e->cfg.vace_stride == 0 && l / e->cfg.vace_stride < e->NV) {
        st = vace_block(e, l / e->cfg.vace_stride, branch, mode, (hipStream_t)stream);
        if (st != MC_OK) return st;
      }
    }
    if (hint_on_last_layer(e)) {
      st = capture_unfused(e, branch, mode, (hipStream_t)stream);
      if (st != MC_OK) return st;
    }
  }
  st = mc_head(e, branch, mode, stream);
  if (st != MC_OK) return st;
  return mc_unpatchify(e, e->buf<float>("head_tokens"), 0, e->L, out_dev, stream);
}

mc_status mc_calib_ready(const mc_engine* e, int branch, int* has_stats) {
  if (!e || !has_stats || branch < 0 || branch > 1) return fail(MC_EINVAL, "bad argument");
  *has_stats = e->have_stats[branch] ? 1 : 0;
  return MC_OK;
}

mc_status mc_calib_finalize(mc_engine* e, int branch, mc_stream stream) {
  if (!e || !e->work.ws) return fail(MC_ESTATE, "no workspace");
  if (branch < 0 || branch > 1) return fail(MC_EINVAL, "branch %d out of range", branch);
  HIP_TRY(mc::launch_calib_finalize(e->buf<double>("calib_sums"), e->buf<float>("calib_stats") + 3 * branch,
                                    (hipStream_t)stream));
  return MC_OK;
}

mc_status mc_import_residual(mc_engine* e, int branch, const float* src_dev, mc_stream stream) {
  if (!e || !e->work.ws || !src_dev) return fail(MC_EINVAL, "null argument / no workspace");
  if (branch < 0 || branch >= e->cfg.n_branches) return fail(MC_EINVAL, "branch %d out of range", branch);
  float* dst = e->residual(e->res_slot[branch]);
  if (dst != src_dev)
    HIP_TRY(hipMemcpyAsync(dst, src_dev, (size_t)e->Lr * e->d * sizeof(float), hipMemcpyDeviceToDevice,
                           (hipStream_t)stream));
  e->have_res[branch] = true;
  return MC_OK;
}

mc_status mc_set_context(mc_engine* e, int slot, const void* context_dev, mc_dtype ctx_dtype, int ctx_len,
                         mc_stream stream_) {
  hipStream_t s = (hipStream_t)stream_;
  mc_status st = check_ready(e);
  if (st != MC_OK) return st;
  if (slot < 0 || slot > 1) return fail(MC_EINVAL, "context slot %d out of range (0, 1)", slot);
  if (e->cfg.no_context_cache) return fail(MC_ESTATE, "the engine was created with no_context_cache: pass the context to every forward");
  if (!context_dev) return fail(MC_EINVAL, "null context");
  const int d = e->d;
  bf16_t* ctx = e->buf<bf16_t>("ctx_cache") + (size_t)slot * e->ctx_rows * d;
  e->ctx_valid[slot] = false;
  st = embed_context(e, context_dev, ctx_dtype, ctx_len, ctx, s);
  if (st != MC_OK) return st;
  bf16_t* base = e->buf<bf16_t>("ckv_cache") + (size_t)slot * (e->NL + e->NV) * e->ctx_rows * 2 * d;
  for (int l = 0; l < e->NL + e->NV; ++l) {
    st = context_kv(e, l < e->NL ? e->layers[l] : e->vlayers[l - e->NL], ctx, base + (size_t)l * e->ctx_rows * 2 * d, s);
    if (st != MC_OK) return st;
  }
  e->ctx_valid[slot] = true;
  e->ctx_active = slot;
  return MC_OK;
}

mc_status mc_use_context(mc_engine* e, int slot) {
  if (!e) return fail(MC_EINVAL, "null engine");
  if (slot < -1 || slot > 1) return fail(MC_EINVAL, "context slot %d out of range (-1, 0, 1)", slot);
  if (slot >= 0 && e->cfg.no_context_cache) return fail(MC_ESTATE, "the engine was created with no_context_cache");
  if (slot >= 0 && !e->ctx_valid[slot]) return fail(MC_ESTATE, "context slot %d was never set (mc_set_context)", slot);
  e->ctx_active = slot;
  return MC_OK;
}

mc_status mc_set_token_timesteps(mc_engine* e, const float* t_tokens_dev, mc_stream) {
  if (!e) return fail(MC_EINVAL, "null engine");
  if (t_tokens_dev && e->NV > 0) return fail(MC_EINVAL, "per-token timesteps are not defined for the VACE model");
  if (t_tokens_dev && e->cfg.no_token_timesteps) return fail(MC_ESTATE, "the engine was created with no_token_timesteps");
  e->tok_t = t_tokens_dev;
  return MC_OK;
}

mc_status mc_profile_enable(mc_engine* e, int on) {
  if (!e) return fail(MC_EINVAL, "null engine");
  if (on < 0 || on > 2) return fail(MC_EINVAL, "profile level %d (0 off, 1 self-attention, 2 every class)", on);
  if (on && e->prof_ev.empty()) {
    e->prof_ev.resize(2 * 8192);
    e->prof_cls.assign(8192, 0);
    for (auto& ev : e->prof_ev) HIP_TRY(hipEventCreate(&ev));
  }
  e->profile = on;
  e->prof_n = 0;
  return MC_OK;
}

mc_status mc_profile_read_classes(mc_engine* e, double ms_total[MC_PROF_NCLASS], int launches[MC_PROF_NCLASS]) {
  if (!e || !ms_total || !launches) return fail(MC_EINVAL, "null argument");
  for (int c = 0; c < MC_PROF_NCLASS; ++c) { ms_total[c] = 0.0; launches[c] = 0; }
  const size_t n = e->prof_n;
  e->prof_n = 0;
  for (size_t i = 0; i + 1 < n; i += 2) {
    const int c = e->prof_cls[i / 2];
    if (c >= MC_PROF_NCLASS) continue;
    HIP_TRY(hipEventSynchronize(e->prof_ev[i + 1]));
    float ms = 0.f;
    HIP_TRY(hipEventElapsedTime(&ms, e->prof_ev[i], e->prof_ev[i + 1]));
    ms_total[c] += ms;
    launches[c] += 1;
  }
  return MC_OK;
}

mc_status mc_profile_read(mc_engine* e, double* attn_ms_total, int* attn_launches) {
  if (!e || !attn_ms_total || !attn_launches) return fail(MC_EINVAL, "null argument");
  double ms[MC_PROF_NCLASS];
  int n[MC_PROF_NCLASS];
  mc_status st = mc_profile_read_classes(e, ms, n);
  if (st != MC_OK) return st;
  *attn_ms_total = ms[MC_PROF_ATTN_SELF];
  *attn_launches = n[MC_PROF_ATTN_SELF];
  return MC_OK;
}

mc_status mc_state_reset(mc_engine* e) {
  if (!e) return fail(MC_EINVAL, "null engine");
  e->have_res[0] = e->have_res[1] = false;
  e->have_stats[0] = e->have_stats[1] = false;
  return MC_OK;
}

mc_status mc_op_rope_table(int F, int Hp, int Wp, int tok0, int n_tok, float* cs_host) {
  if (!cs_host || n_tok <= 0) return fail(MC_EINVAL, "bad argument");
  rope_table_host(F, Hp, Wp, tok0, n_tok, cs_host);
  return MC_OK;
}

}
```

magcache_amd/csrc/ops_capi.cpp:

```cpp
#include <string>

#include "host.h"

using mc::bf16_t;
using mc::fail;
using mc::gp;

extern "C" {

const char* mc_last_error(void) { return mc::last_error(); }
const char* mc_version(void) { return "magcache_hip 0.5 (gfx950)"; }

static float* g_op_splitk_ws = nullptr;
static size_t g_op_splitk_bytes = 0;

mc_status mc_op_gemm_bf16(const void* A, long lda, const void* W, long ldw, const float* bias, int M, int N, int K,
                          int epi, void* Cb, long ldc, float* X, long ldx, const float* gate, const void* X0,
                          long ldx0, float* R, long ldr, void* X0out, long ldx0out, int m_valid, mc_stream s) {
  mc::GemmParams p = gp((const bf16_t*)A, lda, (const bf16_t*)W, ldw, bias, M, N, K);
  p.Cb = (bf16_t*)Cb; p.ldc = ldc; p.X = X; p.ldx = ldx; p.gate = gate;
  p.X0 = (const bf16_t*)X0; p.ldx0 = ldx0; p.R = R; p.ldr = ldr;
  p.X0out = (bf16_t*)X0out; p.ldx0out = ldx0out; p.m_valid = m_valid;
  p.splitk_ws = g_op_splitk_ws; p.splitk_ws_bytes = g_op_splitk_bytes;
  hipError_t err = mc::launch_gemm_bf16(p, epi, (hipStream_t)s);
  if (err == hipErrorInvalidValue) return fail(MC_EINVAL, "gemm: unsupported shape M=%d N=%d K=%d epi=%d", M, N, K, epi);
  HIP_TRY(err);
  return MC_OK;
}

mc_status mc_op_gemm_bf16_resid_sel(const void* A, long lda, const void* W, long ldw, const float* bias, int M, int N, int K,
                                    int capture, float* X, long ldx, const float* gate, const float* gate2,
                                    const unsigned char* gate_sel, const void* X0, long ldx0, float* R, long ldr, mc_stream s) {
  mc::GemmParams p = gp((const bf16_t*)A, lda, (const bf16_t*)W, ldw, bias, M, N, K);
  p.X = X; p.ldx = ldx; p.gate = gate; p.gate2 = gate2; p.gate_sel = gate_sel;
  p.X0 = (const bf16_t*)X0; p.ldx0 = ldx0; p.R = R; p.ldr = ldr;
  if (!gate || !gate2 || !gate_sel) return fail(MC_EINVAL, "gemm (per-token gates): gate, gate2 and gate_sel are required");
  hipError_t err = mc::launch_gemm_bf16(p, capture ? mc::EPI_RESID_CAPTURE : mc::EPI_RESID_GATE, (hipStream_t)s);
  if (err == hipErrorInvalidValue) return fail(MC_EINVAL, "gemm (per-token gates): unsupported shape M=%d N=%d K=%d", M, N, K);
  HIP_TRY(err);
  return MC_OK;
}

mc_status mc_op_gemm_bf16_rowsplit(const void* A, long lda, const void* W, const void* W_b, long ldw, const float* bias,
                                   const float* bias_b, int M, int N, int K, int m_split, int epi, void* Cb, long ldc, float* X,
                                   long ldx, const float* gate, const float* gate_b, mc_stream s) {
  mc::GemmParams p = gp((const bf16_t*)A, lda, (const bf16_t*)W, ldw, bias, M, N, K);
  p.Cb = (bf16_t*)Cb; p.ldc = ldc; p.X = X; p.ldx = ldx; p.gate = gate;
  p.m_split = m_split; p.W_b = (const bf16_t*)W_b; p.bias_b = bias_b; p.gate_b = gate_b;
  p.splitk_ws = g_op_splitk_ws; p.splitk_ws_bytes = g_op_splitk_bytes;
  if (epi != mc::EPI_BF16 && epi != mc::EPI_GELU_BF16 && epi != mc::EPI_RESID_GATE)
    return fail(MC_EINVAL, "gemm (row split): epi %d (0 bf16, 1 gelu, 2 gated residual)", epi);
  hipError_t err = mc::launch_gemm_bf16(p, epi, (hipStream_t)s);
  if (err == hipErrorInvalidValue)
    return fail(MC_EINVAL, "gemm (row split): unsupported shape M=%d N=%d K=%d m_split=%d epi=%d", M, N, K, m_split, epi);
  HIP_TRY(err);
  return MC_OK;
}

mc_status mc_op_gemm_bf16_gelu_split(const void* A, long lda, const void* W, long ldw, const float* bias, int M, int N, int K,
                                     int n_split, void* Cb, long ldc, void* Cb2, long ldc2, mc_stream s) {
  mc::GemmParams p = gp((const bf16_t*)A, lda, (const bf16_t*)W, ldw, bias, M, N, K);
  p.Cb = (bf16_t*)Cb; p.ldc = ldc; p.n_split = n_split; p.Cb2 = (bf16_t*)Cb2; p.ldc2 = ldc2;
  hipError_t err = mc::launch_gemm_bf16(p, mc::EPI_BF16_GELU_SPLIT, (hipStream_t)s);
  if (err == hipErrorInvalidValue)
    return fail(MC_EINVAL, "gemm (bf16 | gelu split): unsupported shape M=%d N=%d K=%d n_split=%d", M, N, K, n_split);
  HIP_TRY(err);
  return MC_OK;
}

int mc_op_gemm_bf16_kernel(int M, int N, int K, int epi) {
  mc::GemmParams p = gp(nullptr, K, nullptr, K, nullptr, M, N, K);
  p.ldc = N; p.ldx = N;
  if (M <= 0 || N <= 0 || K <= 0 || (K % 64) != 0 || (N % 4) != 0) return 0;
  static char dummy[16];
  if (epi == mc::EPI_RESID_CAPTURE) { p.X0 = (const bf16_t*)dummy; p.ldx0 = N; p.R = (float*)dummy; p.ldr = N; }
  if (epi == mc::EPI_BF16_GELU_SPLIT) { p.n_split = N > 256 ? (N / 2) / 256 * 256 : 0; p.Cb2 = (bf16_t*)dummy; p.ldc2 = N; }
  return mc::gemm_bf16_kernel_for(p, epi);
}

int mc_op_gemm_bf16_splitk(int M, int N, int K, int epi) {
  mc::GemmParams p = gp(nullptr, K, nullptr, K, nullptr, M, N, K);
  p.ldc = N; p.ldx = N;
  p.splitk_ws = g_op_splitk_ws; p.splitk_ws_bytes = g_op_splitk_bytes;
  if (M <= 0 || N <= 0 || K <= 0 || (mc::g_gemm_kernel != 0 && mc::g_gemm_kernel != 4)) return 1;
  return mc::gemm_splitk_slices(p, epi);
}

size_t mc_op_gemm_splitk_need(int M, int N, int K, int epi) { return mc::gemm_splitk_ws_need(M, N, K, epi); }

mc_status mc_op_set_splitk_workspace(void* ws_dev, size_t bytes) {
  g_op_splitk_ws = (float*)ws_dev;
  g_op_splitk_bytes = ws_dev ? bytes : 0;
  return MC_OK;
}

mc_status mc_op_attention(const void* Q, long ldq, const void* K, long ldk, long kss, const void* V, long ldv,
                          long vss, void* O, long ldo, int Lq_pad, int n_heads, int shard_rows, int shard_valid,
                          int n_shards, float scale, mc_stream s) {
  mc::AttnParams a;
  memset(&a, 0, sizeof(a));
  a.Q = (const bf16_t*)Q; a.ldq = ldq; a.K = (const bf16_t*)K; a.ldk = ldk; a.k_shard_stride = kss;
  a.V = (const bf16_t*)V; a.ldv = ldv; a.v_shard_stride = vss; a.O = (bf16_t*)O; a.ldo = ldo;
  a.Lq_pad = Lq_pad; a.n_heads = n_heads; a.shard_rows = shard_rows; a.shard_valid = shard_valid;
  a.n_shards = n_shards; a.scale = scale;
  hipError_t err = mc::launch_attention(a, (hipStream_t)s);
  if (err == hipErrorInvalidValue) return fail(MC_EINVAL, "attention: unsupported shape");
  HIP_TRY(err);
  return MC_OK;
}

mc_status mc_op_quantize_rows_fp8(const void* x, mc_dtype dtype, long ldx, int M, int K, void* q, long ldq, float* scale,
                                  mc_stream s) {
  hipError_t err = mc::launch_quantize_rows_fp8(dtype == MC_BF16 ? (const bf16_t*)x : nullptr,
                                                dtype == MC_F32 ? (const float*)x : nullptr, ldx, M, K, (uint8_t*)q, ldq,
                                                scale, (hipStream_t)s);
  if (err == hipErrorInvalidValue) return fail(MC_EINVAL, "quantize_rows_fp8: K, ldx, ldq must be multiples of 4");
  HIP_TRY(err);
  return MC_OK;
}

mc_status mc_op_gemm_fp8(const void* A, long lda, const float* a_scale, const void* W, long ldw, const float* w_scale,
                         const float* bias, int M, int N, int K, int epi, void* Cb, long ldc, float* X, long ldx,
                         const float* gate, mc_stream s) {
  mc::GemmParams p = gp((const bf16_t*)A, lda, (const bf16_t*)W, ldw, bias, M, N, K);
  p.a_scale = a_scale; p.w_scale = w_scale;
  p.Cb = (bf16_t*)Cb; p.ldc = ldc; p.X = X; p.ldx = ldx; p.gate = gate;
  hipError_t err = mc::launch_gemm_fp8(p, epi, (hipStream_t)s);
  if (err == hipErrorInvalidValue)
    return fail(MC_EINVAL, "gemm_fp8: needs N %% 256 == 0, K %% 256 == 0, K >= 512, lda/ldw %% 16 == 0, both scale vectors");
  HIP_TRY(err);
  return MC_OK;
}

mc_status mc_op_quantize_rows_mx(const void* x, mc_dtype dtype, long ldx, int M, int K, void* q, long ldq, void* scales,
                                 long rows_pad, mc_stream s) {
  hipError_t err = mc::launch_quantize_rows_mx(dtype == MC_BF16 ? (const bf16_t*)x : nullptr,
                                               dtype == MC_F32 ? (const float*)x : nullptr, ldx, M, K, (uint8_t*)q, ldq,
                                               (uint8_t*)scales, rows_pad, (hipStream_t)s);
  if (err == hipErrorInvalidValue)
    return fail(MC_EINVAL, "quantize_rows_mx: K %% 32 == 0, ldx %% 8 == 0, ldq %% 16 == 0, rows_pad >= M");
  HIP_TRY(err);
  return MC_OK;
}

mc_status mc_op_gemm_mxfp8(const void* A, long lda, const void* a_scales, long rows_pad_a, const void* W, long ldw,
                           const void* w_scales, long rows_pad_w, const float* bias, int M, int N, int K, int epi, void* Cb,
                           long ldc, float* X, long ldx, const float* gate, mc_stream s) {
  mc::GemmParams p = gp((const bf16_t*)A, lda, (const bf16_t*)W, ldw, bias, M, N, K);
  p.a_mx = (const uint8_t*)a_scales; p.mx_rows_a = rows_pad_a; p.w_mx = (const uint8_t*)w_scales; p.mx_rows_w = rows_pad_w;
  p.Cb = (bf16_t*)Cb; p.ldc = ldc; p.X = X; p.ldx = ldx; p.gate = gate;
  hipError_t err = mc::launch_gemm_mxfp8(p, epi, (hipStream_t)s);
  if (err == hipErrorInvalidValue)
    return fail(MC_EINVAL, "gemm_mxfp8: needs N %% 256 == 0, K %% 256 == 0, K >= 512, lda/ldw %% 16 == 0, block scales with "
                           "rows_pad_a >= M rounded up to 256, rows_pad_w >= N, both multiples of 4");
  HIP_TRY(err);
  return MC_OK;
}

mc_status mc_op_attention_partial(const void* Q, long ldq, const void* K, long ldk, long kss, const void* V, long ldv,
                                  long vss, void* O, long ldo, int Lq_pad, int n_heads, int shard_rows,
                                  int shard_valid, int n_shards, float scale, int skip_shard, float* lse_out,
                                  const float* lse_in, mc_stream s) {
  mc::AttnParams a;
  memset(&a, 0, sizeof(a));
  a.Q = (const bf16_t*)Q; a.ldq = ldq; a.K = (const bf16_t*)K; a.ldk = ldk; a.k_shard_stride = kss;
  a.V = (const bf16_t*)V; a.ldv = ldv; a.v_shard_stride = vss; a.O = (bf16_t*)O; a.ldo = ldo;
  a.Lq_pad = Lq_pad; a.n_heads = n_heads; a.shard_rows = shard_rows; a.shard_valid = shard_valid;
  a.n_shards = n_shards; a.scale = scale;
  a.skip_shard_p1 = skip_shard >= 0 ? skip_shard + 1 : 0; a.lse_out = lse_out; a.lse_in = lse_in;
  hipError_t err = mc::launch_attention(a, (hipStream_t)s);
  if (err == hipErrorInvalidValue) return fail(MC_EINVAL, "attention: unsupported shape / shard selection");
  HIP_TRY(err);
  return MC_OK;
}

mc_status mc_op_attn_merge(const void* const* o_parts, const float* const* lse_parts, int n, void* out, long ldo, int rows,
                           int rows_pad, int d, mc_stream s) {
  if (!o_parts || !lse_parts || !out) return fail(MC_EINVAL, "attn_merge: null argument");
  hipError_t err = mc::launch_attn_merge((const bf16_t* const*)o_parts, lse_parts, n, (bf16_t*)out, ldo, rows, rows_pad, d,
                                         (hipStream_t)s);
  if (err == hipErrorInvalidValue) return fail(MC_EINVAL, "attn_merge: 1..9 parts, d a multiple of 128, 16-byte rows");
  HIP_TRY(err);
  return MC_OK;
}

mc_status mc_op_ln_modulate(const float* x, long ldx, const void* x0, long ldx0, const float* sc, const float* sh,
                            int mode, float eps, void* out, long ldo, float* out_f32, long ldof, int M, int D,
                            mc_stream s) {
  hipError_t err = mc::launch_ln_modulate(x, ldx, (const bf16_t*)x0, ldx0, sc, sh, mode, eps, (bf16_t*)out, ldo,
                                          out_f32, ldof, M, D, (hipStream_t)s);
  if (err == hipErrorInvalidValue) return fail(MC_EINVAL, "ln_modulate: unsupported D=%d", D);
  HIP_TRY(err);
  return MC_OK;
}

mc_status mc_op_rmsnorm_rope(void* x, long ldx, const float* w, float eps, const float* cs, int cs_row0, int M, int D,
                             mc_stream s) {
  hipError_t err = mc::launch_rmsnorm_rope((bf16_t*)x, ldx, w, eps, cs, cs_row0, M, D, (hipStream_t)s);
  if (err == hipErrorInvalidValue) return fail(MC_EINVAL, "rmsnorm_rope: unsupported D=%d", D);
  HIP_TRY(err);
  return MC_OK;
}

mc_status mc_op_skip_add(const void* x0, long ldx0, const float* r, long ldr, float* out, long ldo, int M, int D,
                         mc_stream s) {
  hipError_t err = mc::launch_skip_add((const bf16_t*)x0, ldx0, r, ldr, out, ldo, M, D, (hipStream_t)s);
  if (err == hipErrorInvalidValue) return fail(MC_EINVAL, "skip_add: unsupported shape");
  HIP_TRY(err);
  return MC_OK;
}

mc_status mc_op_residual_sub(const float* x, long ldx, const void* x0, long ldx0, float* r, long ldr, int M, int D,
                             mc_stream s) {
  hipError_t err = mc::launch_residual_sub(x, ldx, (const bf16_t*)x0, ldx0, r, ldr, M, D, (hipStream_t)s);
  if (err == hipErrorInvalidValue) return fail(MC_EINVAL, "residual_sub: unsupported shape");
  HIP_TRY(err);
  return MC_OK;
}

mc_status mc_op_calib_stats(const float* r, long ldr, const float* rp, long ldrp, int M, int D, double* partial,
                            int n_blocks, double* sums, float* stats, mc_stream s) {
  hipError_t err = mc::launch_calib_stats(r, ldr, rp, ldrp, M, D, partial, n_blocks, sums, stats, (hipStream_t)s);
  if (err == hipErrorInvalidValue) return fail(MC_EINVAL, "calib_stats: unsupported shape");
  HIP_TRY(err);
  return MC_OK;
}

mc_status mc_op_cfg_euler(const float* cond, const float* uncond, float guide, float dt, float* x, float* eps_out,
                          size_t n, mc_stream s) {
  HIP_TRY(mc::launch_cfg_euler(cond, uncond, guide, dt, x, eps_out, n, (hipStream_t)s));
  return MC_OK;
}

mc_status mc_op_cfg_norm_euler(const float* cond, const float* uncond, long ld_pred, float guide, float dt, float* x, long ldx,
                               int n_rows, int C, mc_stream s) {
  if (!cond || !uncond || !x) return fail(MC_EINVAL, "null argument");
  hipError_t err = mc::launch_cfg_norm_euler(cond, uncond, ld_pred, guide, dt, x, ldx, n_rows, C, (hipStream_t)s);
  if (err == hipErrorInvalidValue) return fail(MC_EINVAL, "cfg_norm_euler: 0 < C <= 256, ld_pred / ldx >= C, n_rows >= 0");
  HIP_TRY(err);
  return MC_OK;
}

mc_status mc_op_rmsnorm_rows_bf16(const float* x, long ldx, const float* w, float eps, void* out, long ldo, int rows_valid,
                                  int rows, int D, mc_stream s) {
  if (!x || !w || !out) return fail(MC_EINVAL, "null argument");
  hipError_t err = mc::launch_rmsnorm_rows_bf16(x, ldx, w, eps, (bf16_t*)out, ldo, rows_valid, rows, D, (hipStream_t)s);
  if (err == hipErrorInvalidValue) return fail(MC_EINVAL, "rmsnorm_rows_bf16: D, ldx, ldo multiples of 4, 0 <= rows_valid <= rows");
  HIP_TRY(err);
  return MC_OK;
}

mc_status mc_op_lincomb(const float* const* xs_dev, const float* coef, int k, float* out_dev, size_t n, mc_stream s) {
  if (!xs_dev || !coef) return fail(MC_EINVAL, "null argument");
  hipError_t err = mc::launch_lincomb(xs_dev, coef, k, out_dev, n, (hipStream_t)s);
  if (err == hipErrorInvalidValue) return fail(MC_EINVAL, "lincomb: 1..6 operands, non-empty output");
  HIP_TRY(err);
  return MC_OK;
}

mc_status mc_op_add_rows(float* x, long ldx, const void* s, mc_dtype s_dtype, float* r, long ldr, const void* x0, long ldx0,
                         int rows, int D, mc_stream stream) {
  if (s_dtype != MC_F32 && s_dtype != MC_BF16) return fail(MC_EINVAL, "add_rows: the sample is fp32 or bf16");
  hipError_t err = mc::launch_add_rows(x, ldx, s, s_dtype == MC_BF16, r, ldr, (const bf16_t*)x0, ldx0, rows, D, (hipStream_t)stream);
  if (err == hipErrorInvalidValue)
    return fail(MC_EINVAL, "add_rows: D a multiple of 8, 16-byte aligned pointers, ldx / ldr >= D multiples of 4, ldx0 of 8, x0 needs r");
  HIP_TRY(err);
  return MC_OK;
}

mc_status mc_op_cast_bf16(const float* src, void* dst, size_t n, mc_stream s) {
  HIP_TRY(mc::launch_cast_bf16(src, (bf16_t*)dst, n, (hipStream_t)s));
  return MC_OK;
}

mc_status mc_set_option(const char* key, int value) {
  if (!key) return fail(MC_EINVAL, "null key");
  const std::string k(key);
  if (k == "gemm_kernel") {
    if ((value < 0 || value > 2) && value != 4)
      return fail(MC_EINVAL, "gemm_kernel must be 0 (by shape), 1 (128x128), 2 (256x256, 8 waves) or 4 (256x256, 4 waves, generated stream)");
    if (value == 2 && !mc::gemm_bf16_big_linked())
      return fail(MC_EINVAL, "gemm_kernel 2: the 8-wave reference kernel is not in this library (round 6: it lives in the "
                             "test-only libmagcache_hip_ref.so, magcache_amd.build.build_ref())");
    mc::g_gemm_kernel = value;
  } else if (k == "sp_attn_partials") {
    if (value < 0 || value > 2)
      return fail(MC_EINVAL, "sp_attn_partials must be 0 (chain on one stream), 1 (independent launches on two streams + merge where a launch "
                             "does not fill the chip in whole waves) or 2 (always)");
    mc::g_sp_attn_partials = value;
  } else if (k == "gemm_splitk") {
    if (value < 0 || value > 16) return fail(MC_EINVAL, "gemm_splitk must be 0 (never), 1 (by shape) or 2..16 (that many K slices wherever valid)");
    mc::g_gemm_splitk = value;
  } else if (k == "gemm_v2_max_grid") {
    if (value < 0 || value > 4096) return fail(MC_EINVAL, "gemm_v2_max_grid must be 0 (= the CUs) or a workgroup count");
    mc::g_gemm_v2_max_grid = value;
  } else if (k == "gemm_defer") {
    if (value != 0 && value != 1) return fail(MC_EINVAL, "gemm_defer must be 0 (residual epilogues in place) or 1 (deferred into the next tile's main loop)");
    mc::g_gemm_defer = value;
  } else if (k == "fp8_fused_quant") {
    if (value != 0 && value != 1) return fail(MC_EINVAL, "fp8_fused_quant must be 0 (separate quantise passes) or 1 (fused into the producers)");
    mc::g_fp8_fused_quant = value;
  } else if (k == "attn_kernel") {
    if (value != 0 && value != 3 && value != 5)
      return fail(MC_EINVAL, "attn_kernel must be 0 (default), 3 (8 waves x 32 rows) or 5 (4 waves x 64 rows, hand-scheduled)");
    mc::g_attn_kernel = value;
  } else if (k == "mmdit_two_streams") {
    if (value < -1 || value > 6) return fail(MC_EINVAL, "mmdit_two_streams must be -1 (by shape), 0, 1 or a diagnostic mode 2..6");
    mc::g_mmdit_two_streams = value;
  } else {
    return fail(MC_EINVAL, "unknown option '%s'", key);
  }
  return MC_OK;
}

}
```

magcache_amd/engine.py:

```python
import ctypes as C

import torch

from . import _lib
from ._lib import MC_BF16, MC_F32, MC_MODE_CALIB, MC_MODE_FULL, MC_MODE_SKIP, McConfig, check

WAN_T2V_1_3B = dict(dim=1536, ffn_dim=8960, freq_dim=256, num_heads=12, num_layers=30, text_len=512, in_dim=16,
                    out_dim=16, text_dim=4096, eps=1e-6)
WAN_T2V_14B = dict(dim=5120, ffn_dim=13824, freq_dim=256, num_heads=40, num_layers=40, text_len=512, in_dim=16,
                   out_dim=16, text_dim=4096, eps=1e-6)
WAN_I2V_14B = dict(WAN_T2V_14B, model_type="i2v", in_dim=36, clip_dim=1280)
N_CLIP_TOKENS = 257
WAN_VACE_1_3B = dict(WAN_T2V_1_3B, model_type="vace", vace_layers=list(range(0, 30, 2)), vace_in_dim=96)
WAN_VACE_14B = dict(WAN_T2V_14B, model_type="vace", vace_layers=list(range(0, 40, 5)), vace_in_dim=96)


def vace_geometry(cfg):
    if "vace_in_dim" not in cfg and "vace_layers" not in cfg:
        return 0, 0
    layers = cfg.get("vace_layers") or list(range(0, cfg["num_layers"], 2))
    stride = layers[1] - layers[0] if len(layers) > 1 else cfg["num_layers"]
    assert layers[0] == 0 and all(b - a == stride for a, b in zip(layers, layers[1:])), \
        f"vace_layers {layers}: the engine takes an arithmetic progression starting at 0 (upstream's configs are)"
    return len(layers), stride


def _stream():
    return C.c_void_p(torch.cuda.current_stream().cuda_stream)


def _ptr(t):
    return C.c_void_p(t.data_ptr()) if t is not None else C.c_void_p(0)


def weight_names(cfg):
    d, ffn = cfg["dim"], cfg["ffn_dim"]
    out = [("patch_embedding.weight", (d, cfg["in_dim"], 1, 2, 2)), ("patch_embedding.bias", (d,)),
           ("text_embedding.0.weight", (d, cfg["text_dim"])), ("text_embedding.0.bias", (d,)),
           ("text_embedding.2.weight", (d, d)), ("text_embedding.2.bias", (d,)),
           ("time_embedding.0.weight", (d, cfg["freq_dim"])), ("time_embedding.0.bias", (d,)),
           ("time_embedding.2.weight", (d, d)), ("time_embedding.2.bias", (d,)),
           ("time_projection.1.weight", (6 * d, d)), ("time_projection.1.bias", (6 * d,)),
           ("head.head.weight", (4 * cfg["out_dim"], d)), ("head.head.bias", (4 * cfg["out_dim"],)),
           ("head.modulation", (1, 2, d))]
    cd = cfg.get("clip_dim", 0)
    if cd:
        out += [("img_emb.proj.0.weight", (cd,)), ("img_emb.proj.0.bias", (cd,)),
                ("img_emb.proj.1.weight", (cd, cd)), ("img_emb.proj.1.bias", (cd,)),
                ("img_emb.proj.3.weight", (d, cd)), ("img_emb.proj.3.bias", (d,)),
                ("img_emb.proj.4.weight", (d,)), ("img_emb.proj.4.bias", (d,))]
    nv, _ = vace_geometry(cfg)
    if nv:
        out += [("vace_patch_embedding.weight", (d, cfg["vace_in_dim"], 1, 2, 2)), ("vace_patch_embedding.bias", (d,)),
                ("vace_blocks.0.before_proj.weight", (d, d)), ("vace_blocks.0.before_proj.bias", (d,))]
        out += [(f"vace_blocks.{i}.after_proj.{w}", (d, d) if w == "weight" else (d,)) for i in range(nv) for w in ("weight", "bias")]
    for p in [f"blocks.{i}." for i in range(cfg["num_layers"])] + [f"vace_blocks.{i}." for i in range(nv)]:
        for a in ("self_attn", "cross_attn"):
            for w in ("q", "k", "v", "o"):
                out += [(p + f"{a}.{w}.weight", (d, d)), (p + f"{a}.{w}.bias", (d,))]
            out += [(p + f"{a}.norm_q.weight", (d,)), (p + f"{a}.norm_k.weight", (d,))]
        if cd:
            out += [(p + "cross_attn.k_img.weight", (d, d)), (p + "cross_attn.k_img.bias", (d,)),
                    (p + "cross_attn.v_img.weight", (d, d)), (p + "cross_attn.v_img.bias", (d,)),
                    (p + "cross_attn.norm_k_img.weight", (d,))]
        out += [(p + "norm3.weight", (d,)), (p + "norm3.bias", (d,)),
                (p + "ffn.0.weight", (ffn, d)), (p + "ffn.0.bias", (ffn,)),
                (p + "ffn.2.weight", (d, ffn)), (p + "ffn.2.bias", (d,)),
                (p + "modulation", (1, 6, d))]
    return out


def synthetic_weights(cfg, seed=0, std=0.02, device="cuda"):
    g = torch.Generator(device=device).manual_seed(seed)
    for name, shape in weight_names(cfg):
        kind = name.replace("img_emb.proj.0.", "img_emb.norm0.").replace("img_emb.proj.4.", "img_emb.norm4.")
        if name.endswith("modulation"):
            t = torch.randn(shape, generator=g, device=device) / cfg["dim"] ** 0.5
        elif "norm" in kind and name.endswith("weight"):
            t = 1.0 + 0.1 * torch.randn(shape, generator=g, device=device)
        elif "norm" in kind and name.endswith("bias"):
            t = 0.1 * torch.randn(shape, generator=g, device=device)
        else:
            t = std * torch.randn(shape, generator=g, device=device)
        yield name, t


class Engine:

    def __init__(self, cfg, latent_grid, device="cuda:0", sp_rank=0, sp_size=1, n_branches=2, calibration=False,
                 sp_phases=False):
        if not torch.cuda.is_available():
            raise RuntimeError("magcache_amd.Engine needs a ROCm device; there is no CPU fallback")
        self.lib = _lib.load()
        self.cfg = dict(cfg)
        self.device = torch.device(device)
        torch.cuda.set_device(self.device)
        F_, H_, W_ = latent_grid
        self.grid = (F_, H_, W_)
        self.seq_len = F_ * (H_ // 2) * (W_ // 2)
        c = McConfig(dim=cfg["dim"], ffn_dim=cfg["ffn_dim"], num_heads=cfg["num_heads"], num_layers=cfg["num_layers"],
                     in_dim=cfg["in_dim"], out_dim=cfg["out_dim"], freq_dim=cfg["freq_dim"], text_dim=cfg["text_dim"],
                     text_len=cfg["text_len"], latent_f=F_, latent_h=H_, latent_w=W_, eps=cfg.get("eps", 1e-6),
                     sp_rank=sp_rank, sp_size=sp_size, n_branches=n_branches, calibration=int(calibration),
                     clip_dim=cfg.get("clip_dim", 0), vace_layers=vace_geometry(cfg)[0], vace_stride=vace_geometry(cfg)[1],
                     vace_in_dim=cfg.get("vace_in_dim", 0) if vace_geometry(cfg)[0] else 0,
                     fp8_linear=int(cfg.get("fp8_linear", 0) or 0),
                     no_context_cache=int(bool(cfg.get("no_context_cache", 0))),
                     no_token_timesteps=int(bool(cfg.get("no_token_timesteps", 0))), sp_phases=int(bool(sp_phases)))
        self.context_cache = not cfg.get("no_context_cache", 0)
        self.sp_rank, self.sp_size, self.n_branches = sp_rank, sp_size, n_branches
        self.sharded = sp_size > 1 or bool(sp_phases)
        self.vace_layers, self.vace_stride = vace_geometry(cfg)
        h = C.c_void_p()
        check(self.lib.mc_create_sized(C.byref(c), C.sizeof(c), C.byref(h)))
        self.h = h
        nbytes = self.lib.mc_workspace_bytes(self.h)
        self.workspace = torch.empty(nbytes + 256, dtype=torch.uint8, device=self.device)
        off = (-self.workspace.data_ptr()) % 256
        self.ws = self.workspace[off:off + nbytes]
        self.ws.zero_()
        check(self.lib.mc_set_workspace(self.h, _ptr(self.ws), nbytes))
        self.tokens_per_rank = self.seq_len // sp_size
        self.head_stride = (4 * cfg["out_dim"] + 63) // 64 * 64
        self._tok_t = None

    def __del__(self):
        try:
            if getattr(self, "h", None):
                torch.cuda.synchronize(self.device)
                for comm in getattr(self, "_rccl", []):
                    self.lib.mc_sp_comm_destroy(comm)
                self._rccl = []
                self.lib.mc_destroy(self.h)
                self.h = None
        except Exception:
            pass

    def set_weight(self, name, tensor):
        t = tensor.detach()
        if t.dtype not in (torch.float32, torch.bfloat16):
            t = t.float()
        t = t.to(self.device).contiguous()
        shape = (C.c_int64 * t.dim())(*t.shape)
        dt = MC_F32 if t.dtype == torch.float32 else MC_BF16
        st = self.lib.mc_set_weight(self.h, name.encode(), _ptr(t), dt, shape, t.dim(), _stream())
        if st != 0 and dt == MC_BF16 and b"must be given as fp32" in self.lib.mc_last_error():
            t = t.float()
            st = self.lib.mc_set_weight(self.h, name.encode(), _ptr(t), MC_F32, shape, t.dim(), _stream())
        check(st)
        torch.cuda.current_stream().synchronize()

    def load_weights(self, named_tensors):
        items = named_tensors.items() if hasattr(named_tensors, "items") else named_tensors
        for name, t in items:
            self.set_weight(name, t)
        buf = C.create_string_buffer(4096)
        n = self.lib.mc_weights_missing(self.h, buf, 4096)
        if n:
            raise KeyError(f"{n} weights missing, e.g.: {buf.value.decode().split()[:5]}")

    def buffer(self, name, dtype=torch.uint8):
        off, nb = C.c_size_t(), C.c_size_t()
        check(self.lib.mc_buffer_info(self.h, name.encode(), C.byref(off), C.byref(nb)))
        return self.ws[off.value:off.value + nb.value].view(dtype)

    def residual(self, branch):
        d = self.cfg["dim"]
        return self.buffer(f"residual_branch{branch}", torch.float32).view(-1, d)[:self.tokens_per_rank]

    def set_clip_fea(self, clip_fea):
        c = clip_fea.detach().to(self.device, torch.float32).reshape(-1, clip_fea.shape[-1]).contiguous()
        check(self.lib.mc_set_clip_fea(self.h, _ptr(c), MC_F32, c.shape[0], _stream()))
        torch.cuda.current_stream().synchronize()

    def set_token_timesteps(self, t_tokens):
        if t_tokens is None:
            if self._tok_t is not None:
                check(self.lib.mc_set_token_timesteps(self.h, C.c_void_p(0), _stream()))
                self._tok_t = None
            return
        t = t_tokens.detach().reshape(-1).to(self.device, torch.float32).contiguous()
        assert t.numel() >= self.seq_len, f"per-token timesteps: {t.numel()} < seq_len {self.seq_len}"
        check(self.lib.mc_set_token_timesteps(self.h, _ptr(t), _stream()))
        self._tok_t = t

    def token_timestep_record(self):
        r = self.buffer("tok_t2", torch.float32)[:3].cpu()
        return float(r[0]), float(r[1]), int(r[2])

    def profile(self, on=True):
        check(self.lib.mc_profile_enable(self.h, int(on)))

    def profile_read(self):
        ms, n = C.c_double(), C.c_int()
        check(self.lib.mc_profile_read(self.h, C.byref(ms), C.byref(n)))
        return ms.value, n.value

    def profile_read_classes(self):
        from ._lib import PROF_CLASSES
        ms, n = (C.c_double * len(PROF_CLASSES))(), (C.c_int * len(PROF_CLASSES))()
        check(self.lib.mc_profile_read_classes(self.h, ms, n))
        return {name: (ms[i], n[i]) for i, name in enumerate(PROF_CLASSES)}

    def set_vace_context(self, vace_context, scale=1.0):
        v = None if vace_context is None else vace_context.detach().to(self.device, torch.float32).contiguous()
        check(self.lib.mc_set_vace_context(self.h, _ptr(v), float(scale), _stream()))

    def _ctx(self, context):
        if context.dtype == torch.bfloat16:
            return context.contiguous(), MC_BF16
        return context.float().contiguous(), MC_F32

    def set_context(self, slot, context):
        ctx, cdt = self._ctx(context.to(self.device))
        check(self.lib.mc_set_context(self.h, int(slot), _ptr(ctx), cdt, ctx.shape[0], _stream()))
        self._keep_ctx = ctx

    def use_context(self, slot):
        check(self.lib.mc_use_context(self.h, int(slot)))

    def _ctx_args(self, context):
        if context is None:
            return None, MC_F32, 0
        ctx, cdt = self._ctx(context)
        return ctx, cdt, ctx.shape[0]

    def forward(self, latent, t, context, branch=0, mode=MC_MODE_FULL, out=None):
        assert not self.sharded, "use magcache_amd.parallel.SequenceParallelForward for a sharded engine"
        latent = latent.float().contiguous()
        ctx, cdt, clen = self._ctx_args(context)
        if out is None:
            out = torch.empty((self.cfg["out_dim"],) + self.grid, dtype=torch.float32, device=self.device)
        t_dev, t_host = self._t(t)
        check(self.lib.mc_forward(self.h, _ptr(latent), _ptr(t_dev), t_host, _ptr(ctx), cdt, clen, branch,
                                  mode, _ptr(out), _stream()))
        self._keep = (latent, ctx, t_dev)
        return out

    def _t(self, t):
        if torch.is_tensor(t):
            if t.is_cuda:
                return t.reshape(-1)[:1].to(torch.float32), 0.0
            return None, float(t.reshape(-1)[0])
        return None, float(t)

    def embed(self, latent, t, context):
        latent = latent.float().contiguous()
        ctx, cdt, clen = self._ctx_args(context)
        t_dev, t_host = self._t(t)
        check(self.lib.mc_embed(self.h, _ptr(latent), _ptr(t_dev), t_host, _ptr(ctx), cdt, clen, _stream()))
        self._keep = (latent, ctx, t_dev)

    def block_pre_attn(self, layer):
        check(self.lib.mc_block_pre_attn(self.h, layer, _stream()))

    def block_pre_kv(self, layer):
        check(self.lib.mc_block_pre_kv(self.h, layer, _stream()))

    def block_pre_q(self, layer):
        check(self.lib.mc_block_pre_q(self.h, layer, _stream()))

    def block_attn_local(self, layer):
        check(self.lib.mc_block_attn_local(self.h, layer, _stream()))

    def block_attn_round(self, layer, rnd):
        check(self.lib.mc_block_attn_round(self.h, layer, rnd, _stream()))

    def sp_set_chunks(self, chunks):
        check(self.lib.mc_sp_set_chunks(self.h, int(chunks)))

    def sp_round_info(self, rnd=0):
        n, rows, valid = C.c_int(), C.c_int(), C.c_int()
        check(self.lib.mc_sp_round_info(self.h, rnd, C.byref(n), C.byref(rows), C.byref(valid)))
        return n.value, rows.value, valid.value

    def rccl_attach(self, group=None):
        import torch.distributed as dist
        rank, n = dist.get_rank(group), dist.get_world_size(group)
        assert n == self.sp_size and rank == self.sp_rank, (n, rank, self.sp_size, self.sp_rank)
        have = torch.tensor([float(self.lib.mc_sp_rccl_available())], device=self.device)
        mine = have.item() > 0.5
        dist.all_reduce(have, op=dist.ReduceOp.MIN, group=group)
        if have.item() < 0.5:
            raise RuntimeError("librccl could not be bound on " + ("this rank: " + self.lib.mc_last_error().decode() if not mine
                                                                  else "another rank of the group"))
        box = [None]
        if rank == 0:
            buf = C.create_string_buffer(128)
            if self.lib.mc_sp_comm_id(buf) == 0:
                box[0] = buf.raw
        src = dist.get_global_rank(group, 0) if group is not None else 0
        dist.broadcast_object_list(box, src=src, group=group)
        if box[0] is None:
            raise RuntimeError("ncclGetUniqueId failed on the group's first rank")
        comm = C.c_void_p()
        check(self.lib.mc_sp_comm_create(C.c_char_p(box[0]), n, rank, C.byref(comm)))
        self._rccl = getattr(self, "_rccl", [])
        self._rccl.append(comm)
        return comm

    def rccl_detach(self, comm):
        torch.cuda.synchronize(self.device)
        self.lib.mc_sp_comm_destroy(comm)
        self._rccl = [c for c in getattr(self, "_rccl", []) if c is not comm]

    def rccl_info(self, comm):
        return self.lib.mc_sp_comm_info(comm).decode()

    def forward_sp_rccl(self, comm, latent, t, context, branch, mode, overlap, tokens_full, out):
        latent = latent.float().contiguous()
        ctx, cdt, clen = self._ctx_args(context)
        t_dev, t_host = self._t(t)
        check(self.lib.mc_forward_sp_rccl(self.h, comm, _ptr(latent), _ptr(t_dev), t_host, _ptr(ctx), cdt, clen, branch, mode,
                                          int(bool(overlap)), _ptr(tokens_full), _ptr(out), _stream()))
        self._keep = (latent, ctx, t_dev)

    def block_post_attn(self, layer, branch, mode):
        check(self.lib.mc_block_post_attn(self.h, layer, branch, mode, _stream()))

    def blocks_sp(self, layer_begin, layer_end, branch, mode, overlap, gather):
        from ._lib import SP_GATHER_FN
        err = []

        def cb(_user, layer, phase, stream_):
            try:
                gather(layer, phase, stream_)
                return 0
            except BaseException as ex:
                err.append(ex)
                return 1
        fn = SP_GATHER_FN(cb)
        st = self.lib.mc_blocks_sp(self.h, layer_begin, layer_end, branch, mode, int(bool(overlap)), fn, None, _stream())
        if err:
            raise err[0]
        check(st)

    def vace_block_pre(self, i):
        check(self.lib.mc_vace_block_pre(self.h, i, _stream()))

    def vace_block_post(self, i, branch, mode):
        check(self.lib.mc_vace_block_post(self.h, i, branch, mode, _stream()))

    def head(self, branch, mode):
        check(self.lib.mc_head(self.h, branch, mode, _stream()))

    def unpatchify(self, tokens, tok0, n_tok, out):
        check(self.lib.mc_unpatchify(self.h, _ptr(tokens), tok0, n_tok, _ptr(out), _stream()))

    def calib_has_stats(self, branch):
        has = C.c_int()
        check(self.lib.mc_calib_ready(self.h, branch, C.byref(has)))
        return bool(has.value)

    def calib_finalize(self, branch):
        check(self.lib.mc_calib_finalize(self.h, branch, _stream()))

    def calib_stats(self, branch):
        has = C.c_int()
        check(self.lib.mc_calib_ready(self.h, branch, C.byref(has)))
        if not has.value:
            return None
        s = self.buffer("calib_stats", torch.float32)[3 * branch:3 * branch + 3].cpu()
        return float(s[0]), float(s[1]), float(s[2])

    def import_residual(self, branch, tensor):
        t = tensor.float().contiguous()
        assert tuple(t.shape) == (self.tokens_per_rank, self.cfg["dim"]), tuple(t.shape)
        check(self.lib.mc_import_residual(self.h, branch, _ptr(t), _stream()))
        self._keep_res = t

    def reset(self):
        check(self.lib.mc_state_reset(self.h))


__all__ = ["Engine", "WAN_T2V_1_3B", "WAN_T2V_14B", "weight_names", "synthetic_weights", "MC_MODE_FULL",
           "MC_MODE_SKIP", "MC_MODE_CALIB"]
```

magcache_amd/model.py:

```python
import json
import os

import numpy as np
import torch

from .engine import MC_MODE_CALIB, MC_MODE_FULL, MC_MODE_SKIP, Engine
from .mag_ratios import TABLES


def nearest_interp(src_array, target_length):
    src_array = np.asarray(src_array)
    if target_length == 1:
        return np.array([src_array[-1]])
    pos = np.arange(target_length) * ((len(src_array) - 1) / (target_length - 1))
    return src_array[np.round(pos).astype(int)]


def resample_cfg_table(mag_ratios, sample_steps):
    mag_ratios = np.asarray(mag_ratios, dtype=np.float64)
    if len(mag_ratios) == sample_steps * 2:
        return mag_ratios
    pair = [nearest_interp(mag_ratios[i::2], sample_steps) for i in (0, 1)]
    return np.stack(pair, axis=1).reshape(-1)


def select_table(ckpt_dir, task="t2v"):
    s = str(ckpt_dir)
    if "vace" in task:
        return TABLES["wan2.1_vace_14B" if "14B" in s else "wan2.1_vace_1.3B"]
    if "i2v" in task:
        return TABLES["wan2.1_i2v_720P" if "720P" in s else "wan2.1_i2v_480P"]
    if "T2V-14B" in s:
        return TABLES["wan2.1_t2v_14B"]
    if "T2V-1.3B" in s:
        return TABLES["wan2.1_t2v_1.3B"]
    raise ValueError(f"no mag_ratios table for ckpt_dir={ckpt_dir!r}; run --magcache_calibration first")


def _version_of(t):
    try:
        return t._version
    except RuntimeError:
        return None


def _fingerprint(t):
    v = t.detach().contiguous()
    words = v.view(torch.int16 if v.element_size() == 2 else (torch.int32 if v.element_size() == 4 else torch.uint8))
    w = words.reshape(-1).to(torch.int64)
    idx = torch.arange(w.numel(), dtype=torch.int64, device=w.device) * 2654435761 + 1
    return torch.stack([w.sum(), (w * idx).sum()])


def _compare_conditioning():
    return os.environ.get("MAGCACHE_COMPARE_CONDITIONING") == "1"


def _tensor_key(t):
    return (t, _version_of(t), _fingerprint(t) if _compare_conditioning() else None)


def _same_tensor(key, t):
    k, ver, fp = key
    now = _version_of(t)
    if ver is None or now is None:
        return False
    same = k is t and ver == now or (k.data_ptr() == t.data_ptr() and k.shape == t.shape and k.dtype == t.dtype and
                                     k.device == t.device and ver == _version_of(k) == now)
    if same and _compare_conditioning():
        same = fp is not None and bool(torch.equal(fp, _fingerprint(t)))
    return same


class WanModelHIP:

    model_type = "t2v"
    patch_size = (1, 2, 2)

    def __init__(self, cfg, latent_grid, device="cuda:0", calibration=True, engine=None, sp_rank=0, sp_size=1,
                 sp_group=None, sp_phases=False):
        self.cfg = dict(cfg)
        for k in ("dim", "ffn_dim", "freq_dim", "text_len", "text_dim", "in_dim", "out_dim", "num_heads",
                  "num_layers"):
            setattr(self, k, cfg[k])
        self.latent_grid = tuple(latent_grid)
        if cfg.get("model_type", "t2v") != "t2v":
            self.model_type = cfg["model_type"]
        self._clip_key = None
        self._vace_key = None
        self._ctx_keys = [None, None]
        self._ctx_lru = 0
        self.engine = engine or Engine(cfg, latent_grid, device=device, n_branches=2, calibration=calibration,
                                       sp_rank=sp_rank, sp_size=sp_size, sp_phases=sp_phases)
        self.device = self.engine.device
        self.sp_group = sp_group

    def load_state_dict(self, state_dict):
        self.engine.load_weights(state_dict)
        self._ctx_keys = [None, None]
        return self

    def _cached_context(self, ctx):
        for slot, key in enumerate(self._ctx_keys):
            if key is not None and _same_tensor(key, ctx):
                try:
                    self.engine.use_context(slot)
                except Exception:
                    self._ctx_keys[slot] = None
                    break
                self._ctx_lru = 1 - slot
                return
        slot = self._ctx_lru
        self.engine.set_context(slot, ctx)
        self._ctx_keys[slot] = _tensor_key(ctx)
        self._ctx_lru = 1 - slot

    def _check_inputs(self, x, context, seq_len, clip_fea, y):
        if self.model_type == "i2v":
            assert clip_fea is not None and y is not None
        assert len(x) == 1 and len(context) == 1, "the engine evaluates one sample per call, as the Wan sampler does"
        u = x[0]
        c_in = u.shape[0] + (y[0].shape[0] if y is not None else 0)
        assert tuple(u.shape[1:]) == self.latent_grid and c_in == self.in_dim, \
            f"latent {tuple(u.shape)} (+y) does not match the engine grid {(self.in_dim,) + self.latent_grid}"
        if y is not None:
            assert len(y) == 1 and tuple(y[0].shape[1:]) == self.latent_grid
        assert self.engine.seq_len <= seq_len
        assert context[0].shape[0] <= self.text_len and context[0].shape[1] == self.text_dim

    def _run(self, x, t, context, branch, mode, clip_fea=None, y=None, vace=None):
        lat = x[0].to(self.device)
        if y is not None:
            lat = torch.cat([lat, y[0].to(self.device)], dim=0)
        if vace is not None:
            vc, scale = vace[0][0], float(vace[1])
            k = self._vace_key
            if k is None or not _same_tensor(k[0], vc):
                self.engine.set_vace_context(vc, scale)
                self._vace_key = (_tensor_key(vc), scale)
            elif k[1] != scale:
                self.engine.set_vace_context(None, scale)
                self._vace_key = (k[0], scale)
        if clip_fea is not None:
            if self._clip_key is None or not _same_tensor(self._clip_key, clip_fea):
                self.engine.set_clip_fea(clip_fea)
                self._clip_key = _tensor_key(clip_fea)
        if torch.is_tensor(t) and t.numel() > 1:
            assert t.shape[0] == 1 or t.dim() == 1, "one sample per call"
            tv = t.reshape(-1)
            assert tv.numel() >= self.engine.seq_len, f"t has {tv.numel()} entries, the sequence {self.engine.seq_len}"
            tv = tv[:self.engine.seq_len]
            k = getattr(self, "_tok_t_key", None)
            trusted = getattr(t, "_mc_two_valued", False) or os.environ.get("MAGCACHE_VALIDATE_TOKEN_T") == "0"
            if not trusted and (k is None or not _same_tensor(k, t)):
                n = int(torch.unique(tv).numel())
                if n > 2:
                    raise ValueError(f"per-token timesteps with {n} distinct values: the engine supports at most two "
                                     "per forward (Wan2.2 TI2V: conditioning frame + the step's t)")
                self._tok_t_key = _tensor_key(t)
            self.check_token_timesteps(block=False)
            self.engine.set_token_timesteps(tv)
            self._tok_trusted = trusted
            t = tv[-1:]
        elif hasattr(self.engine, "set_token_timesteps"):
            self.engine.set_token_timesteps(None)
        t = t if not torch.is_tensor(t) else t.to(self.device)
        if hasattr(self.engine, "set_context") and getattr(self.engine, "context_cache", True):
            self._cached_context(context[0])
            ctx = None
        else:
            ctx = context[0].to(self.device)
        if getattr(self.engine, "sharded", self.engine.sp_size > 1):
            if getattr(self, "_sp", None) is None:
                from .parallel import SequenceParallelForward
                self._sp = SequenceParallelForward(self.engine, group=self.sp_group)
            out = self._sp.forward(lat, t, ctx, branch, mode)
        else:
            out = self.engine.forward(lat, t, ctx, branch=branch, mode=mode)
        if getattr(self, "_tok_trusted", False):
            self._tok_trusted = False
            if getattr(self, "_tok_ring", None) is None:
                self._tok_ring = [[torch.zeros(3, dtype=torch.float32).pin_memory(), torch.cuda.Event(), False]
                                  for _ in range(16)]
                self._tok_next = 0
            slot = self._tok_ring[self._tok_next]
            if slot[2]:
                slot[1].synchronize()
                self._tok_examine(slot)
            slot[0].copy_(self.engine.buffer("tok_t2", torch.float32)[:3], non_blocking=True)
            slot[1].record()
            slot[2] = True
            self._tok_next = (self._tok_next + 1) % len(self._tok_ring)
        return [out.float()]

    @staticmethod
    def _tok_examine(slot):
        slot[2] = False
        tmax, tmin, neither = (float(v) for v in slot[0])
        if neither > 0:
            raise ValueError(f"per-token timesteps: {int(neither)} tokens carried neither t = {tmax:g} nor t = {tmin:g} in a "
                             "forward whose tensor was tagged two-valued (the engine supports at most two distinct values)")

    def check_token_timesteps(self, block=True):
        err = None
        for slot in getattr(self, "_tok_ring", None) or []:
            if not slot[2]:
                continue
            if block:
                slot[1].synchronize()
            elif not slot[1].query():
                continue
            try:
                self._tok_examine(slot)
            except ValueError as ex:
                err = err or ex
        if err is not None:
            raise err

    def __call__(self, *args, **kwargs):
        return type(self).forward(self, *args, **kwargs)


def _i2v_inputs(clip_fea, y):
    return {} if clip_fea is None and y is None else dict(clip_fea=clip_fea, y=y)


def plain_forward(self, x, t, context, seq_len, clip_fea=None, y=None):
    self._check_inputs(x, context, seq_len, clip_fea, y)
    return self._run(x, t, context, 0, MC_MODE_FULL, **_i2v_inputs(clip_fea, y))


WanModelHIP.forward = plain_forward


def _advance(self):
    self.cnt += 1
    if self.cnt >= self.num_steps:
        self.cnt = 0
        self.accumulated_ratio = [1.0, 1.0]
        self.accumulated_err = [0.0, 0.0]
        self.accumulated_steps = [0, 0]


def _decide(self):
    p = self.cnt % 2
    skip_forward = False
    if self.cnt >= int(self.num_steps * self.retention_ratio):
        self.accumulated_ratio[p] = self.accumulated_ratio[p] * self.mag_ratios[self.cnt]
        self.accumulated_steps[p] += 1
        self.accumulated_err[p] += np.abs(1 - self.accumulated_ratio[p])
        if self.accumulated_err[p] < self.magcache_thresh and self.accumulated_steps[p] <= self.K:
            skip_forward = True
        else:
            self.accumulated_err[p] = 0
            self.accumulated_steps[p] = 0
            self.accumulated_ratio[p] = 1.0
    if skip_forward and self.residual_cache[p] is None:
        raise RuntimeError("MagCache asked to skip before any residual was cached (retention_ratio too small?)")
    return p, skip_forward


def _cached_forward(self, x, t, context, **run_kw):
    p, skip_forward = _decide(self)
    out = self._run(x, t, context, p, MC_MODE_SKIP if skip_forward else MC_MODE_FULL, **run_kw)
    self.residual_cache[p] = self.engine.residual(p)
    _advance(self)
    return out


def _calibration_forward(self, x, t, context, **run_kw):
    p = self.cnt % 2
    out = self._run(x, t, context, p, MC_MODE_CALIB, **run_kw)
    if self.cnt >= 2:
        norm_ratio, norm_std, cos_dis = self.engine.calib_stats(p)
        self.norm_ratio.append(round(norm_ratio, 5))
        self.norm_std.append(round(norm_std, 5))
        self.cos_dis.append(round(cos_dis, 5))
        print(f"time: {self.cnt}, norm_ratio: {norm_ratio}, norm_std: {norm_std}, cos_dis: {cos_dis}")
    self.residual_cache[p] = self.engine.residual(p)
    self.cnt += 1
    if self.cnt >= self.num_steps:
        self.cnt = 0
        self.accumulated_ratio = [1.0, 1.0]
        self.accumulated_err = [0.0, 0.0]
        self.accumulated_steps = [0, 0]
        print("norm ratio")
        print(self.norm_ratio)
        print("norm std")
        print(self.norm_std)
        print("cos_dis")
        print(self.cos_dis)
        for fn, v in (("wan2_1_mag_ratio", self.norm_ratio), ("wan2_1_mag_std", self.norm_std),
                      ("wan2_1_cos_dis", self.cos_dis)):
            with open(fn + ".json", "w") as f:
                json.dump(v, f)
    return out


def magcache_forward(self, x, t, context, seq_len, clip_fea=None, y=None):
    self._check_inputs(x, context, seq_len, clip_fea, y)
    return _cached_forward(self, x, t, context, **_i2v_inputs(clip_fea, y))


def magcache_calibration(self, x, t, context, seq_len, clip_fea=None, y=None):
    self._check_inputs(x, context, seq_len, clip_fea, y)
    return _calibration_forward(self, x, t, context, **_i2v_inputs(clip_fea, y))


def _vace_checks(self, x, vace_context, context, seq_len):
    type(self)._check_inputs(self, x, context, seq_len, None, None)
    assert len(vace_context) == 1 and tuple(vace_context[0].shape[1:]) == self.latent_grid \
        and vace_context[0].shape[0] == self.cfg["vace_in_dim"], f"vace_context {tuple(vace_context[0].shape)}"


def magcache_vace_forward(self, x, t, vace_context, context, seq_len, vace_context_scale=1.0, clip_fea=None, y=None):
    _vace_checks(self, x, vace_context, context, seq_len)
    return _cached_forward(self, x, t, context, vace=(vace_context, vace_context_scale))


def magcache_vace_calibration(self, x, t, vace_context, context, seq_len, vace_context_scale=1.0, clip_fea=None, y=None):
    _vace_checks(self, x, vace_context, context, seq_len)
    return _calibration_forward(self, x, t, context, vace=(vace_context, vace_context_scale))


def vace_plain_forward(self, x, t, vace_context, context, seq_len, vace_context_scale=1.0, clip_fea=None, y=None):
    _vace_checks(self, x, vace_context, context, seq_len)
    return self._run(x, t, context, 0, MC_MODE_FULL, vace=(vace_context, vace_context_scale))


def call_branch(model, step, branch, x, t, context, seq_len, **kw):
    cls = type(model)
    has_state = getattr(cls, "forward", None) in (magcache_forward, magcache_calibration, magcache_vace_forward,
                                                  magcache_vace_calibration)
    if has_state:
        model.cnt = 2 * step + branch
    out = model(x, t=t, context=context, seq_len=seq_len, **kw)
    if has_state and branch == 0:
        _advance(model)
    return out


def init_magcache(model, sample_steps, magcache_thresh=0.12, magcache_K=2, retention_ratio=0.2, mag_ratios=None,
                  ckpt_dir="Wan2.1-T2V-1.3B"):
    cls = model.__class__
    cls.forward = magcache_forward
    cls.cnt = 0
    cls.num_steps = sample_steps * 2
    cls.magcache_thresh = magcache_thresh
    cls.K = magcache_K
    cls.accumulated_err = [0.0, 0.0]
    cls.accumulated_steps = [0, 0]
    cls.accumulated_ratio = [1.0, 1.0]
    cls.retention_ratio = retention_ratio
    cls.residual_cache = [None, None]
    table = select_table(ckpt_dir) if mag_ratios is None else np.asarray(mag_ratios, dtype=np.float64)
    cls.mag_ratios = resample_cfg_table(table, sample_steps)
    model.engine.reset()
    return model


def init_magcache_calibration(model, sample_steps):
    cls = model.__class__
    cls.forward = magcache_calibration
    cls.cnt = 0
    cls.num_steps = sample_steps * 2
    cls.norm_ratio, cls.norm_std, cls.cos_dis = [], [], []
    cls.residual_cache = [None, None]
    cls.accumulated_err, cls.accumulated_steps, cls.accumulated_ratio = [0.0, 0.0], [0, 0], [1.0, 1.0]
    model.engine.reset()
    return model


def disable_magcache(model):
    model.__class__.forward = plain_forward
    model.engine.reset()
    return model
```

magcache_amd/sampler.py:

```python
import math
import ctypes as C

import numpy as np
import torch

from . import _lib
from ._lib import check


def flow_timesteps(num_steps, shift=5.0, num_train_timesteps=1000, sigma_grid="reference"):
    if sigma_grid == "upstream":
        sig = np.linspace(1.0 - 1.0 / num_train_timesteps, 0.0, num_steps + 1)[:-1]
    else:
        assert sigma_grid == "reference", sigma_grid
        sig = np.linspace(1.0, 0.01, num_steps + 1)[:-1]
    sig = shift * sig / (1 + (shift - 1) * sig)
    sig = np.concatenate([sig, [0.0]]).astype(np.float32)
    return sig, (sig[:-1] * num_train_timesteps).astype(np.int64)


def cfg_euler_(latent, eps_cond, eps_uncond, guide_scale, dt, eps_out=None):
    lib = _lib.load()
    assert latent.is_contiguous() and eps_cond.is_contiguous() and eps_uncond.is_contiguous()
    check(lib.mc_op_cfg_euler(C.c_void_p(eps_cond.data_ptr()), C.c_void_p(eps_uncond.data_ptr()),
                              float(guide_scale), float(dt), C.c_void_p(latent.data_ptr()),
                              C.c_void_p(eps_out.data_ptr()) if eps_out is not None else C.c_void_p(0),
                              latent.numel(), C.c_void_p(torch.cuda.current_stream().cuda_stream)))
    return latent


def lincomb_hip(coefs, tensors, out=None):
    lib = _lib.load()
    k = len(tensors)
    out = torch.empty_like(tensors[0]) if out is None else out
    ptrs = (C.c_void_p * k)(*[t.data_ptr() for t in tensors])
    cf = (C.c_float * k)(*[float(c) for c in coefs])
    check(lib.mc_op_lincomb(ptrs, cf, k, C.c_void_p(out.data_ptr()), out.numel(),
                            C.c_void_p(torch.cuda.current_stream().cuda_stream)))
    return out


class FlowSolver:

    def __init__(self, sigmas, solver="unipc", order=2, lincomb=lincomb_hip):
        assert solver in ("euler", "unipc", "dpm++")
        self.sig = np.asarray(sigmas, dtype=np.float64)
        self.n = len(self.sig) - 1
        self.solver, self.order, self.lc = solver, order, lincomb
        with np.errstate(divide="ignore"):
            self.lam = np.log(1.0 - self.sig) - np.log(self.sig)
        self.x0_hist, self.idx_hist = [], []
        self.last_sample, self.lower_order_nums, self.this_order = None, 0, 1

    def _unipc_coeffs(self, i_s0, i_t, order, hist_idx, corrector):
        lam, sig = self.lam, self.sig
        h = lam[i_t] - lam[i_s0]
        rks = [(lam[j] - lam[i_s0]) / h for j in hist_idx[:order - 1]]
        rks.append(1.0)
        hh = -h
        h_phi_1 = math.expm1(hh)
        B_h = math.expm1(hh)
        h_phi_k = h_phi_1 / hh - 1.0
        fact = 1.0
        R, b = [], []
        for j in range(1, order + 1):
            R.append([rk ** (j - 1) for rk in rks])
            b.append(h_phi_k * fact / B_h)
            fact *= (j + 1)
            h_phi_k = h_phi_k / hh - 1.0 / fact
        R, b = np.array(R), np.array(b)
        if corrector:
            rhos = np.array([0.5]) if order == 1 else np.linalg.solve(R, b)
        else:
            rhos = np.array([0.5]) if order == 2 else (np.linalg.solve(R[:-1, :-1], b[:-1]) if order > 2 else np.array([]))
        alpha_t = 1.0 - sig[i_t]
        return sig[i_t] / sig[i_s0], -alpha_t * h_phi_1, -alpha_t * B_h, rks, rhos

    def _unipc_update(self, x, i_s0, i_t, order, model_t=None):
        m0 = self.x0_hist[-1]
        prev = list(zip(self.idx_hist[-2::-1], self.x0_hist[-2::-1]))[:order - 1]
        A, Bm, Cd, rks, rhos = self._unipc_coeffs(i_s0, i_t, order, [j for j, _ in prev], model_t is not None)
        coefs, tens = [A, Bm], [x, m0]
        for k, (_, mk) in enumerate(prev):
            w = Cd * rhos[k] / rks[k]
            coefs.append(w)
            tens.append(mk)
            coefs[1] -= w
        if model_t is not None:
            w = Cd * rhos[-1]
            coefs.append(w)
            tens.append(model_t)
            coefs[1] -= w
        return self.lc(coefs, tens)

    def step(self, i, x, v):
        sig = self.sig
        if self.solver == "euler":
            return self.lc([1.0, sig[i + 1] - sig[i]], [x, v])
        x0 = self.lc([1.0, -sig[i]], [x, v])
        if self.solver == "unipc":
            if i > 0 and self.last_sample is not None:
                x = self._unipc_update(self.last_sample, i - 1, i, self.this_order, model_t=x0)
            self.x0_hist.append(x0)
            self.idx_hist.append(i)
            self.x0_hist, self.idx_hist = self.x0_hist[-self.order:], self.idx_hist[-self.order:]
            this_order = min(self.order, self.n - i)
            self.this_order = min(this_order, self.lower_order_nums + 1)
            self.last_sample = x
            out = self._unipc_update(x, i, i + 1, self.this_order)
            if self.lower_order_nums < self.order:
                self.lower_order_nums += 1
            return out
        self.x0_hist.append(x0)
        self.idx_hist.append(i)
        self.x0_hist, self.idx_hist = self.x0_hist[-2:], self.idx_hist[-2:]
        lam = self.lam
        h = lam[i + 1] - lam[i]
        alpha_t = 1.0 - sig[i + 1]
        e = math.expm1(-h)
        if len(self.x0_hist) < 2 or i == self.n - 1:
            return self.lc([sig[i + 1] / sig[i], -alpha_t * e], [x, x0])
        r0 = (lam[i] - lam[self.idx_hist[0]]) / h
        w1 = -0.5 * alpha_t * e / r0
        return self.lc([sig[i + 1] / sig[i], -alpha_t * e + w1, -w1], [x, x0, self.x0_hist[0]])


def sample(model, noise, context, context_null, sampling_steps=50, shift=5.0, guide_scale=5.0, seq_len=None,
           callback=None, solver="euler", layout=None, lincomb=None, model_kwargs=None, sigma_grid="reference"):
    mk = model_kwargs or {}
    sig, ts = flow_timesteps(sampling_steps, shift, sigma_grid=sigma_grid)
    device = noise.device
    t_dev = torch.tensor(ts, dtype=torch.float32, device=device)
    latent = noise.clone().float().contiguous()
    seq_len = seq_len or model.engine.seq_len
    lc = lincomb or lincomb_hip
    fs = FlowSolver(sig, solver, lincomb=lc) if solver != "euler" else None
    cfg_par = layout is not None and layout.cfg_size == 2
    for i in range(sampling_steps):
        timestep = t_dev[i:i + 1]
        if cfg_par:
            from .model import call_branch
            mine = call_branch(model, i, layout.branch, [latent], timestep,
                               [context if layout.branch == 0 else context_null], seq_len, **mk)[0]
            eps_c, eps_u = layout.exchange(mine.contiguous())
        else:
            eps_c = model([latent], t=timestep, context=[context], seq_len=seq_len, **mk)[0]
            eps_u = model([latent], t=timestep, context=[context_null], seq_len=seq_len, **mk)[0]
        if fs is None and lincomb is None:
            cfg_euler_(latent, eps_c, eps_u, guide_scale, float(sig[i + 1] - sig[i]))
        elif fs is None:
            dt = float(sig[i + 1] - sig[i])
            latent = lc([1.0, dt * (1.0 - guide_scale), dt * guide_scale], [latent, eps_u, eps_c])
        else:
            v = lc([1.0 - guide_scale, guide_scale], [eps_u.contiguous(), eps_c.contiguous()])
            latent = fs.step(i, latent, v)
        if callback is not None:
            callback(i, latent)
    return latent


def qwen_image_sigmas(num_inference_steps, image_seq_len, base_image_seq_len=256, max_image_seq_len=8192, base_shift=0.5,
                      max_shift=0.9, shift_terminal=0.02, num_train_timesteps=1000):
    n = int(num_inference_steps)
    s = np.linspace(1.0, 1.0 / n, n).astype(np.float32)
    m = (max_shift - base_shift) / (max_image_seq_len - base_image_seq_len)
    mu = image_seq_len * m + (base_shift - m * base_image_seq_len)
    s = (math.exp(mu) / (math.exp(mu) + (1.0 / s.astype(np.float64) - 1.0) ** 1.0))
    if shift_terminal:
        one_minus = 1.0 - s
        s = 1.0 - one_minus / (one_minus[-1] / (1.0 - shift_terminal))
    s = s.astype(np.float32)
    return np.concatenate([s, [0.0]]).astype(np.float32), (s * num_train_timesteps).astype(np.float32)


def cfg_norm_euler_(latent, pred_cond, pred_uncond, true_cfg_scale, dt):
    lib = _lib.load()
    assert latent.dtype == pred_cond.dtype == pred_uncond.dtype == torch.float32
    assert latent.is_contiguous() and pred_cond.is_contiguous() and pred_uncond.is_contiguous()
    n, c = latent.shape[-2], latent.shape[-1]
    assert pred_cond.shape[-1] == c and pred_cond.shape[-2] >= n and pred_uncond.shape == pred_cond.shape
    check(lib.mc_op_cfg_norm_euler(C.c_void_p(pred_cond.data_ptr()), C.c_void_p(pred_uncond.data_ptr()), c,
                                   float(true_cfg_scale), float(dt), C.c_void_p(latent.data_ptr()), c, n, c,
                                   C.c_void_p(torch.cuda.current_stream().cuda_stream)))
    return latent


def sample_qwen_image(model, latents, prompt_embeds, negative_prompt_embeds, img_shapes, num_inference_steps=50,
                      true_cfg_scale=4.0, image_latents=None, sigmas=None, callback=None):
    x = latents.to(torch.float32).contiguous().clone()
    n = x.shape[1]
    if sigmas is None:
        sigmas, _ = qwen_image_sigmas(num_inference_steps, n)
    pe, ne = prompt_embeds, negative_prompt_embeds
    lens_c, lens_u = [int(pe.shape[1])], [int(ne.shape[1])]
    do_cfg = true_cfg_scale > 1 and ne is not None
    for i in range(num_inference_steps):
        t = torch.tensor([float(sigmas[i]) * 1000.0], device=x.device)
        inp = x if image_latents is None else torch.cat([x, image_latents.to(x)], dim=1)
        cond = model(hidden_states=inp, timestep=t / 1000, encoder_hidden_states=pe, img_shapes=img_shapes,
                     txt_seq_lens=lens_c, return_dict=False)[0]
        dt = float(sigmas[i + 1]) - float(sigmas[i])
        if do_cfg:
            unc = model(hidden_states=inp, timestep=t / 1000, encoder_hidden_states=ne, img_shapes=img_shapes,
                        txt_seq_lens=lens_u, return_dict=False)[0]
            cfg_norm_euler_(x[0], cond[0].contiguous(), unc[0].contiguous(), true_cfg_scale, dt)
        else:
            lincomb_hip([1.0, dt], [x[0], cond[0, :n].contiguous()], out=x[0])
        if callback is not None:
            callback(i, x)
    return x
```

Before: 5.509.

## Share block-0 self-attention between conditional and unconditional CFG forwards

Adds a pair mode where the first CFG branch saves the hidden state after block-0 self-attention and the cross-attention query. The second branch, given the same latent and timestep, reuses them and skips patch/time embedding and block-0 self-attention. This removes duplicated context-independent work in each step. In exchange it adds an extra device copy of the hidden state, extra workspace, and state-invalidation logic that must be dropped on any other API call.

```diff
diff --git a/include/magcache_hip.h b/include/magcache_hip.h
--- a/include/magcache_hip.h
+++ b/include/magcache_hip.h
@@ -63,6 +63,9 @@
 mc_status mc_forward(mc_engine* e, const float* latent_dev, const float* t_dev, double t_host,
                      const void* context_dev, mc_dtype ctx_dtype, int ctx_len, int branch, mc_mode mode,
                      float* out_dev, mc_stream stream);
+
+mc_status mc_pair_begin(mc_engine* e);
+mc_status mc_pair_end(mc_engine* e);
 
 mc_status mc_set_context(mc_engine* e, int slot, const void* context_dev, mc_dtype ctx_dtype, int ctx_len,
                          mc_stream stream);
diff --git a/magcache_amd/_lib.py b/magcache_amd/_lib.py
--- a/magcache_amd/_lib.py
+++ b/magcache_amd/_lib.py
@@ -45,6 +45,8 @@
     "mc_set_weight": (_i, [_vp, C.c_char_p, _vp, _i, C.POINTER(C.c_int64), _i, _vp]),
     "mc_weights_missing": (_i, [_vp, C.c_char_p, _sz]),
     "mc_forward": (_i, [_vp, _vp, _vp, _d, _vp, _i, _i, _i, _i, _vp, _vp]),
+    "mc_pair_begin": (_i, [_vp]),
+    "mc_pair_end": (_i, [_vp]),
     "mc_set_clip_fea": (_i, [_vp, _vp, _i, _i, _vp]),
     "mc_set_vace_context": (_i, [_vp, _vp, _f, _vp]),
     "mc_set_token_timesteps": (_i, [_vp, _vp, _vp]),
diff --git a/magcache_amd/csrc/engine.cpp b/magcache_amd/csrc/engine.cpp
--- a/magcache_amd/csrc/engine.cpp
+++ b/magcache_amd/csrc/engine.cpp
@@ -71,6 +71,12 @@
   bool have_res[2] = {false, false};
   bool have_stats[2] = {false, false};
   bool embedded = false;
+  enum { PAIR_NONE, PAIR_ARMED, PAIR_KEPT, PAIR_DEAD };
+  int pair = PAIR_NONE;
+  const float *pair_latent = nullptr, *pair_t_dev = nullptr;
+  double pair_t_host = 0.0;
+  bool pair_capable() const { return !sp && NV == 0 && cfg.clip_dim == 0 && cfg.fp8_linear == 0; }
+  void pair_drop() { if (pair != PAIR_NONE) pair = PAIR_DEAD; }
 
   template <class T>
   T* buf(const char* name) const { return work.get<T>(name); }
@@ -347,6 +353,8 @@
   ws.add("calib_partial", (2048 * 4 + 2) * 8);
   ws.add("calib_sums", 4 * 8);
   ws.add("calib_stats", 2 * 3 * 4);
+  ws.add("pair_x", e->pair_capable() ? Lp * d * 4 : 256);
+  ws.add("pair_cq", e->pair_capable() ? Lp * d * 2 : 256);
   *out = own.release();
   return MC_OK;
 }
@@ -367,6 +375,7 @@
   if (!e) return fail(MC_EINVAL, "null argument");
   MC_TRY(e->work.bind(ws_dev, bytes));
   e->have_res[0] = e->have_res[1] = false;
+  e->pair_drop();
   HIP_TRY(hipMemset(e->buf<double>("calib_partial") + 2048 * 4, 0, 16));
   return MC_OK;
 }
@@ -386,6 +395,7 @@
   if (e) {
     e->ctx_valid[0] = e->ctx_valid[1] = false;
     e->ctx_active = -1;
+    e->pair_drop();
   }
   if (!e || !name || !src_dev || !shape) return fail(MC_EINVAL, "null argument");
   return e->weights.set(name, src_dev, dtype, shape, ndim, (hipStream_t)stream);
@@ -397,6 +407,7 @@
   hipStream_t s = (hipStream_t)stream_;
   mc_status st = check_ready(e);
   if (st != MC_OK) return st;
+  e->pair_drop();
   const mc_config& c = e->cfg;
   if (c.clip_dim <= 0) return fail(MC_EINVAL, "engine was created without clip_dim (t2v model)");
   if (!clip_dev || n_tokens != 257) return fail(MC_EINVAL, "clip_fea must be [257, %d]", c.clip_dim);
@@ -429,6 +440,7 @@
   hipStream_t s = (hipStream_t)stream_;
   mc_status st = check_ready(e);
   if (st != MC_OK) return st;
+  e->pair_drop();
   if (e->NV <= 0) return fail(MC_EINVAL, "engine was created without VACE blocks");
   const mc_config& c = e->cfg;
   const int d = e->d;
@@ -483,24 +495,17 @@
   return MC_OK;
 }
 
-mc_status mc_embed(mc_engine* e, const float* latent_dev, const float* t_dev, double t_host,
-                   const void* context_dev, mc_dtype ctx_dtype, int ctx_len, mc_stream stream_) {
-  hipStream_t s = (hipStream_t)stream_;
-  mc_status st = check_ready(e);
-  if (st != MC_OK) return st;
-  if (!latent_dev) return fail(MC_EINVAL, "null input");
+static mc_status embed_latent_time(mc_engine* e, const float* latent_dev, const float* t_dev, double t_host, float* x,
+                                   hipStream_t s) {
   const mc_config& c = e->cfg;
-  if (c.clip_dim > 0 && !e->have_clip)
-    return fail(MC_ESTATE, "i2v model: mc_set_clip_fea must run before the forward (reference assert :226-227)");
   const int d = e->d;
-  Prof pr(e, MC_PROF_EMBED, s);
   bf16_t* tokens = e->buf<bf16_t>("tokens");
   if (e->Kp != c.in_dim * 4) HIP_TRY(hipMemsetAsync(tokens, 0, (size_t)e->Lp * e->Kp * 2, s));
   HIP_TRY(mc::launch_patchify(latent_dev, c.in_dim, c.latent_f, c.latent_h, c.latent_w, e->tok0, e->Lr, e->Lp,
                               tokens, e->Kp, s));
   {
     mc::GemmParams p = gp(tokens, e->Kp, e->w_patch, e->Kp, e->b_patch, e->Lp, d, e->Kp);
-    p.X = e->buf<float>("x"); p.ldx = d;
+    p.X = x; p.ldx = d;
     p.X0out = e->buf<bf16_t>("x0"); p.ldx0out = d;
     p.m_valid = e->Lr;
     HIP_TRY(mc::launch_gemm_bf16(p, mc::EPI_EMBED, s));
@@ -526,15 +531,38 @@
                                    emod + (size_t)l * 6 * d, 6 * d, s));
     HIP_TRY(mc::launch_add_bcast(ev, d, e->head_mod, e->buf<float>("ehead") + set * 2 * d, 2 * d, s));
   }
+  return MC_OK;
+}
+
+static mc_status embed_text(mc_engine* e, const void* context_dev, mc_dtype ctx_dtype, int ctx_len, hipStream_t s) {
   if (context_dev) {
     e->ctx_active = -1;
-    mc_status cst = embed_context(e, context_dev, ctx_dtype, ctx_len, e->buf<bf16_t>("ctx"), s);
-    if (cst != MC_OK) return cst;
-  } else if (e->ctx_active < 0 || !e->ctx_valid[e->ctx_active]) {
+    return embed_context(e, context_dev, ctx_dtype, ctx_len, e->buf<bf16_t>("ctx"), s);
+  }
+  if (e->ctx_active < 0 || !e->ctx_valid[e->ctx_active])
     return fail(MC_ESTATE, "context_dev is NULL but no cached context is selected (mc_set_context)");
-  }
+  return MC_OK;
+}
+
+static mc_status embed(mc_engine* e, const float* latent_dev, const float* t_dev, double t_host, const void* context_dev,
+                       mc_dtype ctx_dtype, int ctx_len, float* x, hipStream_t s) {
+  mc_status st = check_ready(e);
+  if (st != MC_OK) return st;
+  if (!latent_dev) return fail(MC_EINVAL, "null input");
+  if (e->cfg.clip_dim > 0 && !e->have_clip)
+    return fail(MC_ESTATE, "i2v model: mc_set_clip_fea must run before the forward (reference assert :226-227)");
+  Prof pr(e, MC_PROF_EMBED, s);
+  MC_TRY(embed_latent_time(e, latent_dev, t_dev, t_host, x, s));
+  MC_TRY(embed_text(e, context_dev, ctx_dtype, ctx_len, s));
   e->embedded = true;
   return MC_OK;
+}
+
+mc_status mc_embed(mc_engine* e, const float* latent_dev, const float* t_dev, double t_host,
+                   const void* context_dev, mc_dtype ctx_dtype, int ctx_len, mc_stream stream_) {
+  if (e) e->pair_drop();
+  return embed(e, latent_dev, t_dev, t_host, context_dev, ctx_dtype, ctx_len, e ? e->buf<float>("x") : nullptr,
+               (hipStream_t)stream_);
 }
 
 struct ActSrc {
@@ -657,6 +685,7 @@
 
 mc_status mc_block_pre_attn(mc_engine* e, int layer, mc_stream stream_) {
   if (mc_status st = check_layer_call(e, layer); st != MC_OK) return st;
+  e->pair_drop();
   return block_pre(e, e->layers[layer], e->buf<float>("emod") + (size_t)layer * 6 * e->d, e->buf<float>("x"),
                    (hipStream_t)stream_);
 }
@@ -664,6 +693,7 @@
 mc_status mc_block_pre_kv(mc_engine* e, int layer, mc_stream stream_) {
   if (mc_status st = check_layer_call(e, layer); st != MC_OK) return st;
   if (!e->sp) return fail(MC_ESTATE, "mc_block_pre_kv needs a sequence-parallel engine (sp_size > 1 or sp_phases) (one GPU: mc_block_pre_attn / mc_forward)");
+  e->pair_drop();
   return block_pre_kv(e, e->layers[layer], e->buf<float>("emod") + (size_t)layer * 6 * e->d, e->buf<float>("x"),
                       (hipStream_t)stream_);
 }
@@ -671,6 +701,7 @@
 mc_status mc_block_pre_q(mc_engine* e, int layer, mc_stream stream_) {
   if (mc_status st = check_layer_call(e, layer); st != MC_OK) return st;
   if (!e->sp) return fail(MC_ESTATE, "mc_block_pre_q needs a sequence-parallel engine (sp_size > 1 or sp_phases)");
+  e->pair_drop();
   return block_pre_q(e, e->layers[layer], (hipStream_t)stream_);
 }
 
@@ -770,6 +801,7 @@
     return fail(MC_EINVAL, "sp chunks %d: rows per shard %d / chunks must be a multiple of 64", chunks, e->Lp);
   e->sp_chunks = chunks;
   e->attn_layer = -2;
+  e->pair_drop();
   return MC_OK;
 }
 
@@ -796,9 +828,8 @@
   return MC_OK;
 }
 
-static mc_status block_post(mc_engine* e, const Layer& l, const float* em, float* x, int layer, bool capture, int branch,
-                            mc_mode mode, hipStream_t s) {
-  const int d = e->d, Lp = e->Lp, ffn = e->ffn;
+static mc_status block_post_self(mc_engine* e, const Layer& l, const float* em, float* x, int layer, bf16_t* cq, hipStream_t s) {
+  const int d = e->d, Lp = e->Lp;
   bf16_t* qkv = e->buf<bf16_t>("qkv");
   bf16_t* ao = e->buf<bf16_t>("ao");
   const float scale = 1.0f / std::sqrt(128.0f);
@@ -835,19 +866,26 @@
     Prof pr(e, MC_PROF_LN_MODULATE, s);
     MC_TRY(ln_for_gemm(e, l.cq, x, l.n3w, l.n3b, 1, nullptr, nullptr, nullptr, s, &xn));
   }
-  bf16_t* cq = qkv;
+  mc::GemmParams p = {};
+  p.Cb = cq; p.ldc = d;
+  {
+    Prof pr(e, MC_PROF_GEMM_CROSS_Q, s);
+    MC_TRY(linear(e, l.cq, whole(l.cq), xn, p, mc::EPI_BF16, s));
+  }
+  Prof pr(e, MC_PROF_RMSNORM_ROPE, s);
+  HIP_TRY(mc::launch_rmsnorm_rope(cq, d, l.cnq, e->cfg.eps, nullptr, 0, Lp, d, s));
+  return MC_OK;
+}
+
+static mc_status block_post_ctx(mc_engine* e, const Layer& l, const float* em, float* x, int layer, const bf16_t* cq,
+                                bool capture, int branch, mc_mode mode, hipStream_t s) {
+  const int d = e->d, Lp = e->Lp, ffn = e->ffn;
+  bf16_t* ao = e->buf<bf16_t>("ao");
+  const float scale = 1.0f / std::sqrt(128.0f);
+  const float* em2 = second_set(e, em);
+  const uint8_t* sel = tok_sel(e);
   bf16_t* ckv = e->buf<bf16_t>("ckv");
   {
-    mc::GemmParams p = {};
-    p.Cb = cq; p.ldc = d;
-    {
-      Prof pr(e, MC_PROF_GEMM_CROSS_Q, s);
-      MC_TRY(linear(e, l.cq, whole(l.cq), xn, p, mc::EPI_BF16, s));
-    }
-    {
-      Prof pr(e, MC_PROF_RMSNORM_ROPE, s);
-      HIP_TRY(mc::launch_rmsnorm_rope(cq, d, l.cnq, e->cfg.eps, nullptr, 0, Lp, d, s));
-    }
     if (e->ctx_active >= 0) {
       const size_t li = (size_t)(&l - (layer >= 0 ? e->layers.data() : e->vlayers.data())) + (layer >= 0 ? 0 : e->NL);
       ckv = e->buf<bf16_t>("ckv_cache") + ((size_t)e->ctx_active * (e->NL + e->NV) + li) * e->ctx_rows * 2 * d;
@@ -884,6 +922,7 @@
     o.X = x; o.ldx = d; o.gate = nullptr;
     MC_TRY(linear(e, l.co, whole(l.co), ActSrc{ao, d}, o, mc::EPI_RESID_GATE, s));
   }
+  ActSrc xn;
   {
     Prof pr(e, MC_PROF_LN_MODULATE, s);
     MC_TRY(ln_for_gemm(e, l.ffn1, x, em + 4 * d, em + 3 * d, 0, em2 ? em2 + 4 * d : nullptr, em2 ? em2 + 3 * d : nullptr, sel,
@@ -941,6 +980,12 @@
   return MC_OK;
 }
 
+static mc_status block_post(mc_engine* e, const Layer& l, const float* em, float* x, int layer, bf16_t* cq, bool capture,
+                            int branch, mc_mode mode, hipStream_t s) {
+  MC_TRY(block_post_self(e, l, em, x, layer, cq, s));
+  return block_post_ctx(e, l, em, x, layer, cq, capture, branch, mode, s);
+}
+
 static bool hint_on_last_layer(const mc_engine* e) {
   return e->NV > 0 && (e->NV - 1) * e->cfg.vace_stride == e->NL - 1;
 }
@@ -949,8 +994,9 @@
   if (!e || !e->embedded) return fail(MC_ESTATE, "mc_embed must run first");
   if (layer < 0 || layer >= e->NL) return fail(MC_EINVAL, "layer %d out of range", layer);
   if (branch < 0 || branch >= e->cfg.n_branches) return fail(MC_EINVAL, "branch %d out of range", branch);
+  e->pair_drop();
   return block_post(e, e->layers[layer], e->buf<float>("emod") + (size_t)layer * 6 * e->d, e->buf<float>("x"), layer,
-                    layer == e->NL - 1 && !hint_on_last_layer(e), branch, mode, (hipStream_t)stream_);
+                    e->buf<bf16_t>("qkv"), layer == e->NL - 1 && !hint_on_last_layer(e), branch, mode, (hipStream_t)stream_);
 }
 
 static mc_status vace_pre_kv(mc_engine* e, int i, hipStream_t s) {
@@ -974,8 +1020,8 @@
 static mc_status vace_post(mc_engine* e, int i, int branch, mc_mode mode, hipStream_t s) {
   const int d = e->d, Lp = e->Lp;
   float* xc = e->buf<float>("xc");
-  mc_status st = block_post(e, e->vlayers[i], e->buf<float>("emod") + (size_t)(e->NL + i) * 6 * d, xc, -1, false, branch,
-                            mode, s);
+  mc_status st = block_post(e, e->vlayers[i], e->buf<float>("emod") + (size_t)(e->NL + i) * 6 * d, xc, -1,
+                            e->buf<bf16_t>("qkv"), false, branch, mode, s);
   if (st != MC_OK) return st;
   bf16_t* xn = e->buf<bf16_t>("xn");
   HIP_TRY(mc::launch_cast_bf16(xc, xn, (size_t)Lp * d, s));
@@ -1109,8 +1155,7 @@
   return MC_OK;
 }
 
-mc_status mc_head(mc_engine* e, int branch, mc_mode mode, mc_stream stream_) {
-  hipStream_t s = (hipStream_t)stream_;
+static mc_status head(mc_engine* e, const float* x, int branch, mc_mode mode, hipStream_t s) {
   if (!e || !e->embedded) return fail(MC_ESTATE, "mc_embed must run first");
   if (branch < 0 || branch >= e->cfg.n_branches) return fail(MC_EINVAL, "branch %d out of range", branch);
   const int d = e->d;
@@ -1124,12 +1169,18 @@
     HIP_TRY(mc::launch_ln_modulate(e->residual(e->res_slot[branch]), d, e->buf<bf16_t>("x0"), d, eh + d, eh, 0,
                                    e->cfg.eps, nullptr, 0, hn, d, e->Lr, d, s, eh2 ? eh2 + d : nullptr, eh2, sel));
   } else {
-    HIP_TRY(mc::launch_ln_modulate(e->buf<float>("x"), d, nullptr, 0, eh + d, eh, 0, e->cfg.eps, nullptr, 0, hn, d,
+    HIP_TRY(mc::launch_ln_modulate(x, d, nullptr, 0, eh + d, eh, 0, e->cfg.eps, nullptr, 0, hn, d,
                                    e->Lr, d, s, eh2 ? eh2 + d : nullptr, eh2, sel));
   }
   HIP_TRY(mc::launch_head_linear(hn, d, e->w_head, e->b_head, e->buf<float>("head_tokens"), e->HT, e->Lr,
                                  e->cfg.out_dim * 4, d, s));
   return MC_OK;
+}
+
+mc_status mc_head(mc_engine* e, int branch, mc_mode mode, mc_stream stream) {
+  if (!e) return fail(MC_ESTATE, "mc_embed must run first");
+  e->pair_drop();
+  return head(e, e->buf<float>("x"), branch, mode, (hipStream_t)stream);
 }
 
 mc_status mc_unpatchify(mc_engine* e, const float* tokens_dev, int tok0, int n_tok, float* out_dev,
@@ -1143,6 +1194,18 @@
   return MC_OK;
 }
 
+mc_status mc_pair_begin(mc_engine* e) {
+  if (!e) return fail(MC_EINVAL, "null engine");
+  e->pair = e->pair_capable() ? mc_engine::PAIR_ARMED : mc_engine::PAIR_NONE;
+  return MC_OK;
+}
+
+mc_status mc_pair_end(mc_engine* e) {
+  if (!e) return fail(MC_EINVAL, "null engine");
+  e->pair = mc_engine::PAIR_NONE;
+  return MC_OK;
+}
+
 mc_status mc_forward(mc_engine* e, const float* latent_dev, const float* t_dev, double t_host,
                      const void* context_dev, mc_dtype ctx_dtype, int ctx_len, int branch, mc_mode mode,
                      float* out_dev, mc_stream stream) {
@@ -1151,25 +1214,55 @@
   if (!out_dev) return fail(MC_EINVAL, "null output");
   if (e->NV > 0 && mode != MC_MODE_SKIP && !e->have_vace)
     return fail(MC_ESTATE, "VACE model: mc_set_vace_context must run before a non-skipped forward");
-  mc_status st = mc_embed(e, latent_dev, t_dev, t_host, context_dev, ctx_dtype, ctx_len, stream);
-  if (st != MC_OK) return st;
-  if (mode != MC_MODE_SKIP) {
+  if (branch < 0 || branch >= e->cfg.n_branches) return fail(MC_EINVAL, "branch %d out of range", branch);
+  hipStream_t s = (hipStream_t)stream;
+  const int d = e->d;
+  const bool runs = mode != MC_MODE_SKIP;
+  const bool reuse = e->pair == mc_engine::PAIR_KEPT && runs && latent_dev == e->pair_latent && t_dev == e->pair_t_dev &&
+                     t_host == e->pair_t_host;
+  const bool keep = e->pair == mc_engine::PAIR_ARMED && runs;
+  e->pair = keep ? mc_engine::PAIR_KEPT : e->pair == mc_engine::PAIR_NONE ? mc_engine::PAIR_NONE : mc_engine::PAIR_DEAD;
+  if (keep) { e->pair_latent = latent_dev; e->pair_t_dev = t_dev; e->pair_t_host = t_host; }
+  float* x = e->buf<float>(keep ? "pair_x" : "x");
+  bf16_t* cq = e->buf<bf16_t>(keep || reuse ? "pair_cq" : "qkv");
+  mc_status st;
+  if (reuse) {
+    if ((st = check_ready(e)) != MC_OK) return st;
+    if (context_dev) {
+      Prof pr(e, MC_PROF_EMBED, s);
+      st = embed_text(e, context_dev, ctx_dtype, ctx_len, s);
+    } else {
+      st = embed_text(e, nullptr, ctx_dtype, 0, s);
+    }
+  } else {
+    st = embed(e, latent_dev, t_dev, t_host, context_dev, ctx_dtype, ctx_len, x, s);
+  }
+  if (st != MC_OK) { e->pair_drop(); return st; }
+  if (runs) {
     for (int l = 0; l < e->NL; ++l) {
-      st = mc_block_pre_attn(e, l, stream);
-      if (st != MC_OK) return st;
-      st = mc_block_post_attn(e, l, branch, mode, stream);
-      if (st != MC_OK) return st;
+      const Layer& ly = e->layers[l];
+      const float* em = e->buf<float>("emod") + (size_t)l * 6 * d;
+      const bool capture = l == e->NL - 1 && !hint_on_last_layer(e);
+      if (!(reuse && l == 0)) {
+        if ((st = block_pre(e, ly, em, x, s)) != MC_OK) break;
+        if ((st = block_post_self(e, ly, em, x, l, l == 0 ? cq : e->buf<bf16_t>("qkv"), s)) != MC_OK) break;
+      }
+      if (keep && l == 0) {
+        Prof pr(e, MC_PROF_OTHER, s);
+        if (hipMemcpyAsync(e->buf<float>("x"), x, (size_t)e->Lp * d * 4, hipMemcpyDeviceToDevice, s) != hipSuccess) {
+          st = fail(MC_EHIP, "hipMemcpyAsync of the kept stream failed");
+          break;
+        }
+      }
+      if ((st = block_post_ctx(e, ly, em, x, l, l == 0 ? cq : e->buf<bf16_t>("qkv"), capture, branch, mode, s)) != MC_OK) break;
       if (e->NV > 0 && l % e->cfg.vace_stride == 0 && l / e->cfg.vace_stride < e->NV) {
-        st = vace_block(e, l / e->cfg.vace_stride, branch, mode, (hipStream_t)stream);
-        if (st != MC_OK) return st;
+        if ((st = vace_block(e, l / e->cfg.vace_stride, branch, mode, s)) != MC_OK) break;
       }
     }
-    if (hint_on_last_layer(e)) {
-      st = capture_unfused(e, branch, mode, (hipStream_t)stream);
-      if (st != MC_OK) return st;
-    }
-  }
-  st = mc_head(e, branch, mode, stream);
+    if (st == MC_OK && hint_on_last_layer(e)) st = capture_unfused(e, branch, mode, s);
+    if (st != MC_OK) { e->pair_drop(); return st; }
+  }
+  st = head(e, x, branch, mode, s);
   if (st != MC_OK) return st;
   return mc_unpatchify(e, e->buf<float>("head_tokens"), 0, e->L, out_dev, stream);
 }
@@ -1236,6 +1329,7 @@
   if (t_tokens_dev && e->NV > 0) return fail(MC_EINVAL, "per-token timesteps are not defined for the VACE model");
   if (t_tokens_dev && e->cfg.no_token_timesteps) return fail(MC_ESTATE, "the engine was created with no_token_timesteps");
   e->tok_t = t_tokens_dev;
+  e->pair_drop();
   return MC_OK;
 }
 
diff --git a/magcache_amd/csrc/ops_capi.cpp b/magcache_amd/csrc/ops_capi.cpp
--- a/magcache_amd/csrc/ops_capi.cpp
+++ b/magcache_amd/csrc/ops_capi.cpp
@@ -9,7 +9,7 @@
 extern "C" {
 
 const char* mc_last_error(void) { return mc::last_error(); }
-const char* mc_version(void) { return "magcache_hip 0.5 (gfx950)"; }
+const char* mc_version(void) { return "magcache_hip 0.6 (gfx950)"; }
 
 static float* g_op_splitk_ws = nullptr;
 static size_t g_op_splitk_bytes = 0;
diff --git a/magcache_amd/engine.py b/magcache_amd/engine.py
--- a/magcache_amd/engine.py
+++ b/magcache_amd/engine.py
@@ -244,6 +244,12 @@
             return None, float(t.reshape(-1)[0])
         return None, float(t)
 
+    def pair_begin(self):
+        check(self.lib.mc_pair_begin(self.h))
+
+    def pair_end(self):
+        check(self.lib.mc_pair_end(self.h))
+
     def embed(self, latent, t, context):
         latent = latent.float().contiguous()
         ctx, cdt, clen = self._ctx_args(context)
diff --git a/magcache_amd/model.py b/magcache_amd/model.py
--- a/magcache_amd/model.py
+++ b/magcache_amd/model.py
@@ -193,6 +193,16 @@
             self._tok_next = (self._tok_next + 1) % len(self._tok_ring)
         return [out.float()]
 
+    def pair_begin(self):
+        begin = getattr(self.engine, "pair_begin", None)
+        if begin is not None:
+            begin()
+
+    def pair_end(self):
+        end = getattr(self.engine, "pair_end", None)
+        if end is not None:
+            end()
+
     @staticmethod
     def _tok_examine(slot):
         slot[2] = False
diff --git a/magcache_amd/sampler.py b/magcache_amd/sampler.py
--- a/magcache_amd/sampler.py
+++ b/magcache_amd/sampler.py
@@ -126,7 +126,8 @@
 
 
 def sample(model, noise, context, context_null, sampling_steps=50, shift=5.0, guide_scale=5.0, seq_len=None,
-           callback=None, solver="euler", layout=None, lincomb=None, model_kwargs=None, sigma_grid="reference"):
+           callback=None, solver="euler", layout=None, lincomb=None, model_kwargs=None, sigma_grid="reference",
+           cfg_pair=True):
     mk = model_kwargs or {}
     sig, ts = flow_timesteps(sampling_steps, shift, sigma_grid=sigma_grid)
     device = noise.device
@@ -144,8 +145,15 @@
                                [context if layout.branch == 0 else context_null], seq_len, **mk)[0]
             eps_c, eps_u = layout.exchange(mine.contiguous())
         else:
-            eps_c = model([latent], t=timestep, context=[context], seq_len=seq_len, **mk)[0]
-            eps_u = model([latent], t=timestep, context=[context_null], seq_len=seq_len, **mk)[0]
+            pair = cfg_pair and hasattr(model, "pair_begin")
+            if pair:
+                model.pair_begin()
+            try:
+                eps_c = model([latent], t=timestep, context=[context], seq_len=seq_len, **mk)[0]
+                eps_u = model([latent], t=timestep, context=[context_null], seq_len=seq_len, **mk)[0]
+            finally:
+                if pair:
+                    model.pair_end()
         if fs is None and lincomb is None:
             cfg_euler_(latent, eps_c, eps_u, guide_scale, float(sig[i + 1] - sig[i]))
         elif fs is None:
```

Measured after the change: 5.584, median of 6. 1.4% higher.
